# Crowsinc/LiveVisionKit

Hardware: AMD Instinct MI355X
Metric: stabilized frames/sec (one 4K YUV420 stream per GPU, steady state) (higher is better)
Workload: dtype f32

## Files before the change

include/lvk_hip.h:

```cpp
#ifndef LVK_HIP_H
#define LVK_HIP_H

#include <stdint.h>
#include <stddef.h>

#ifdef __cplusplus
extern "C" {
#endif

#define LVK_HIP_OK              0
#define LVK_HIP_ERR_ARG        -1
#define LVK_HIP_ERR_RUNTIME    -2
#define LVK_HIP_ERR_NO_DEVICE  -3

typedef struct lvk_hip_ctx lvk_hip_ctx;


int  lvk_hip_ctx_create(int device, lvk_hip_ctx** out);
int  lvk_hip_ctx_create_on_stream(int device, void* hip_stream, lvk_hip_ctx** out);
void lvk_hip_ctx_destroy(lvk_hip_ctx* ctx);
int  lvk_hip_sync(lvk_hip_ctx* ctx);
void* lvk_hip_stream(lvk_hip_ctx* ctx);
const char* lvk_hip_last_error(lvk_hip_ctx* ctx);
const char* lvk_hip_version(void);
// ... 6 lines not shown

int lvk_hip_malloc(lvk_hip_ctx* ctx, size_t bytes, void** d_ptr);
int lvk_hip_free(lvk_hip_ctx* ctx, void* d_ptr);
int lvk_hip_trim(lvk_hip_ctx* ctx);
int lvk_hip_upload(lvk_hip_ctx* ctx, void* d_dst, const void* h_src, size_t bytes);
int lvk_hip_download(lvk_hip_ctx* ctx, void* h_dst, const void* d_src, size_t bytes);

int  lvk_hip_host_malloc(lvk_hip_ctx* ctx, size_t bytes, void** h_ptr);
int  lvk_hip_host_free(lvk_hip_ctx* ctx, void* h_ptr);


int lvk_hip_remap_homography(lvk_hip_ctx* ctx,
                             const void* d_src, int src_step, int src_rows, int src_cols,
                             void* d_dst, int dst_step, int dst_rows, int dst_cols,
                             int off_x, int off_y, const float H[9], const uint8_t bg[3], int yuv);

int lvk_hip_remap_mesh(lvk_hip_ctx* ctx,
                       const void* d_src, int src_step, int src_rows, int src_cols,
                       void* d_dst, int dst_step,
                       const float* mesh, int mesh_rows, int mesh_cols, const uint8_t bg[3], int yuv);

int lvk_hip_remap_map(lvk_hip_ctx* ctx, const void* d_src, int src_step, int rows, int cols, void* d_dst, int dst_step,
                      const void* d_map, int map_step, const uint8_t bg[3], int yuv);

#define LVK_REMAP_EXACT 0
#define LVK_REMAP_1LSB  1
int lvk_hip_set_remap_precision(lvk_hip_ctx* ctx, int precision);
int lvk_hip_get_remap_precision(lvk_hip_ctx* ctx);

int lvk_hip_upscale(lvk_hip_ctx* ctx, const void* d_src, int src_step, int src_rows, int src_cols,
                    void* d_dst, int dst_step, int dst_rows, int dst_cols, int yuv);

int lvk_hip_sharpen(lvk_hip_ctx* ctx, const void* d_src, int src_step, int rows, int cols, void* d_dst, int dst_step, float sharpness);

typedef struct lvk_camera_params { double fx, fy, cx, cy, k1, k2, p1, p2, k3; } lvk_camera_params;
int lvk_hip_lens_map_create(lvk_hip_ctx* ctx, const lvk_camera_params* params, int rows, int cols, void** d_map, int view_xywh[4]);
int lvk_hip_lens_map_destroy(lvk_hip_ctx* ctx, void* d_map);
int lvk_hip_warpmesh_apply_lens(lvk_hip_ctx* ctx, const void* d_src, int src_step, int rows, int cols, void* d_dst, int dst_step,
                                const float* mesh, int mesh_rows, int mesh_cols, const uint8_t bg[3], int yuv, const lvk_camera_params* lens);
int lvk_hip_lens_undistort_points(lvk_hip_ctx* ctx, const lvk_camera_params* params, int rows, int cols, double sx, double sy,
                                  const float* pts, int n, float* out);

int lvk_hip_warpmesh_apply_yuv420(lvk_hip_ctx* ctx, const void* d_src, int src_step, int rows, int cols,
                                  void* o_y, int oy_step, void* o_u, int ou_step, void* o_v, int ov_step, int nv12,
                                  const float* mesh, int mesh_rows, int mesh_cols, const uint8_t bg[3]);

int lvk_hip_warpmesh_apply(lvk_hip_ctx* ctx,
                           const void* d_src, int src_step, int rows, int cols,
                           void* d_dst, int dst_step,
                           const float* mesh, int mesh_rows, int mesh_cols, const uint8_t bg[3], int yuv);

int lvk_hip_ingest_yuv420(lvk_hip_ctx* ctx, const void* d_y, int y_step, const void* d_u, int u_step, const void* d_v, int v_step, int nv12,
                          int rows, int cols, void* d_dst, int dst_step);
int lvk_hip_egress_yuv420(lvk_hip_ctx* ctx, const void* d_src, int src_step, int rows, int cols,
                          void* d_y, int y_step, void* d_u, int u_step, void* d_v, int v_step, int nv12);

#define LVK_VIDEO_FORMAT_I420 1
#define LVK_VIDEO_FORMAT_NV12 2
#define LVK_VIDEO_FORMAT_YVYU 3
#define LVK_VIDEO_FORMAT_YUY2 4
#define LVK_VIDEO_FORMAT_UYVY 5
#define LVK_VIDEO_FORMAT_RGBA 6
#define LVK_VIDEO_FORMAT_BGRA 7
#define LVK_VIDEO_FORMAT_BGRX 8
#define LVK_VIDEO_FORMAT_Y800 9
#define LVK_VIDEO_FORMAT_I444 10
#define LVK_VIDEO_FORMAT_BGR3 11
#define LVK_VIDEO_FORMAT_I422 12
#define LVK_VIDEO_FORMAT_I40A 13
#define LVK_VIDEO_FORMAT_I42A 14
#define LVK_VIDEO_FORMAT_YUVA 15
#define LVK_VIDEO_FORMAT_AYUV 16
int lvk_hip_ingest_obs(lvk_hip_ctx* ctx, int video_format, const void* const d_planes[3], const int steps[3], int rows, int cols, void* d_dst, int dst_step);
int lvk_hip_egress_obs(lvk_hip_ctx* ctx, int video_format, const void* d_src, int src_step, int rows, int cols, void* const d_planes[3], const int steps[3]);
int lvk_hip_obs_frame_format(int video_format);

typedef struct lvk_stab_settings
{
    int detection_width, detection_height;
    int detection_regions_x, detection_regions_y;
    int force_detection;
    float max_feature_density, min_feature_density, accumulation_rate;
    int track_local_motions;
    float temporal_smoothing, local_smoothing;
    int min_motion_samples;
    float acceptance_threshold, uniformity_threshold;
    int predictive_samples;
    float corrective_limit_x, corrective_limit_y;
    float smoothing_steps, response_rate;
    int motion_width, motion_height;
    float background[3];
    int crop_to_stable_region, stabilize_output;
    float min_scene_quality, min_tracking_quality;
} lvk_stab_settings;

typedef struct lvk_stab_stats
{
    float tracking_stability;
    float scene_quality, trust;
    float distribution;
    int n_detected, n_matched, n_tracked, frame_delay;
    double smoothing_factor;
    double homography[9];
} lvk_stab_stats;

#define LVK_FORMAT_BGR 0
#define LVK_FORMAT_BGRA 1
#define LVK_FORMAT_RGB 2
#define LVK_FORMAT_RGBA 3
#define LVK_FORMAT_YUV 4
#define LVK_FORMAT_GRAY 5

typedef struct lvk_hip_stab lvk_hip_stab;

void lvk_stab_default_settings(lvk_stab_settings* s);
int  lvk_hip_stab_create(lvk_hip_ctx* ctx, const lvk_stab_settings* settings, lvk_hip_stab** out);
void lvk_hip_stab_destroy(lvk_hip_stab* stab);
int  lvk_hip_stab_configure(lvk_hip_stab* stab, const lvk_stab_settings* settings);
int  lvk_hip_stab_restart(lvk_hip_stab* stab);
int  lvk_hip_stab_draw_trackers(lvk_hip_stab* stab);
int  lvk_hip_stab_draw_motion_mesh(lvk_hip_stab* stab);
int  lvk_hip_draw_grid(lvk_hip_ctx* ctx, void* d_dst, int dst_step, int rows, int cols, int grid_w, int grid_h, const uint8_t colour[3], int thickness);
int  lvk_hip_draw_crosses(lvk_hip_ctx* ctx, void* d_dst, int dst_step, int rows, int cols, const float* pts_xy, int n,
                          float scale_x, float scale_y, const uint8_t colour[3], int cross_size, int thickness);
int  lvk_hip_draw_points(lvk_hip_ctx* ctx, void* d_dst, int dst_step, int rows, int cols, const float* pts_xy, int n, float scale_x, float scale_y,
                         const uint8_t colour[3], int point_size);
int  lvk_hip_draw_rect(lvk_hip_ctx* ctx, void* d_dst, int dst_step, int rows, int cols, const int rect_xywh[4], const uint8_t colour[3], int thickness);
int  lvk_hip_draw_text(lvk_hip_ctx* ctx, void* d_dst, int dst_step, int rows, int cols, const char* text, int x, int y, const uint8_t colour[3],
                       int scale, int thickness);
int  lvk_hip_stab_set_lens(lvk_hip_stab* stab, const lvk_camera_params* params);
int  lvk_hip_stab_reset_context(lvk_hip_stab* stab);
int  lvk_hip_stab_ready(const lvk_hip_stab* stab);
int  lvk_hip_stab_frame_delay(const lvk_hip_stab* stab);
int  lvk_hip_stab_stable_region(const lvk_hip_stab* stab, int rows, int cols, int rect_xywh[4]);

typedef struct lvk_frame_info { int rows, cols, format; } lvk_frame_info;
int  lvk_hip_stab_next_output(const lvk_hip_stab* stab, int rows, int cols, int format, lvk_frame_info* out);
int  lvk_hip_stab_push(lvk_hip_stab* stab, const void* d_frame, int step, int rows, int cols, uint64_t timestamp, int format,
                       void* d_out, int out_step, int out_rows, int* produced, uint64_t* out_timestamp, const void** released,
                       lvk_frame_info* emitted);

int  lvk_hip_stab_push_yuv420(lvk_hip_stab* stab, const void* d_y, int y_step, const void* d_u, int u_step, const void* d_v, int v_step, int nv12,
                              int rows, int cols, uint64_t timestamp,
                              void* o_y, int oy_step, void* o_u, int ou_step, void* o_v, int ov_step, int o_rows,
                              int* produced, uint64_t* out_timestamp, lvk_frame_info* emitted);
int  lvk_hip_stab_push_obs(lvk_hip_stab* stab, int video_format, const void* const d_planes[3], const int steps[3], int rows, int cols, uint64_t timestamp,
                           void* const o_planes[3], const int o_steps[3], int o_rows, int* produced, uint64_t* out_timestamp, lvk_frame_info* emitted);

int  lvk_hip_stab_push_yuv420_host(lvk_hip_stab* stab, const void* h_y, int y_step, const void* h_u, int u_step, const void* h_v, int v_step, int nv12,
                                   int rows, int cols, uint64_t timestamp,
                                   void* oh_y, int oy_step, void* oh_u, int ou_step, void* oh_v, int ov_step, int o_rows,
                                   int* produced, uint64_t* out_timestamp, lvk_frame_info* emitted);
int  lvk_hip_stab_push_obs_host(lvk_hip_stab* stab, int video_format,
                                const void* const h_planes[3], const int steps[3], int rows, int cols, uint64_t timestamp,
                                void* const oh_planes[3], const int o_steps[3], int o_rows,
                                int* produced, uint64_t* out_timestamp, lvk_frame_info* emitted);
int  lvk_hip_stab_prefetch_yuv420_host(lvk_hip_stab* stab, const void* h_y, int y_step, const void* h_u, int u_step, const void* h_v, int v_step,
                                       int nv12, int rows, int cols);
int  lvk_hip_stab_prefetch_cancel(lvk_hip_stab* stab);
int  lvk_hip_stab_set_overlap(lvk_hip_stab* stab, int enable);
int  lvk_hip_stab_set_bulk_context(lvk_hip_stab* stab, lvk_hip_ctx* bulk);
void* lvk_hip_stab_output_stream(lvk_hip_stab* stab);
int  lvk_hip_stab_set_remap_precision(lvk_hip_stab* stab, int precision);
int  lvk_hip_stab_get_remap_precision(const lvk_hip_stab* stab);


typedef struct lvk_deblock_settings
{
    uint32_t detection_levels;
    uint32_t block_size;
    uint32_t filter_size;
    float filter_scaling;
} lvk_deblock_settings;

typedef struct lvk_hip_deblock lvk_hip_deblock;

void lvk_hip_deblock_default_settings(lvk_deblock_settings* s);
int  lvk_hip_deblock_create(lvk_hip_ctx* ctx, const lvk_deblock_settings* settings, lvk_hip_deblock** out);
int  lvk_hip_deblock_configure(lvk_hip_deblock* deb, const lvk_deblock_settings* settings);
void lvk_hip_deblock_destroy(lvk_hip_deblock* deb);
int  lvk_hip_deblock_apply(lvk_hip_deblock* deb, void* d_frame, int step, int rows, int cols, int format, int region_xywh[4]);
int  lvk_hip_deblock_draw_influence(const lvk_hip_deblock* deb, void* d_frame, int step, int rows, int cols, int format);
int  lvk_hip_deblock_filter_region(const lvk_hip_deblock* deb, int region_xywh[4]);

int  lvk_hip_cas(lvk_hip_ctx* ctx, const void* d_src, int src_step, int rows, int cols, int format, void* d_dst, int dst_step, float sharpness);

int  lvk_hip_reformat(lvk_hip_ctx* ctx, const void* d_src, int src_step, int rows, int cols, int src_format, void* d_dst, int dst_step,
                      int dst_format);

int  lvk_hip_fsr_easu(lvk_hip_ctx* ctx, const void* d_src, int src_step, int rows, int cols, int format, const int region_xywh[4], void* d_dst,
                      int dst_step, int out_rows, int out_cols);
int  lvk_hip_fsr_geometry(int rows, int cols, int out_rows, int out_cols, float multiplier, int maintain_aspect_ratio, const int crop_ltrb[4],
                          int region_xywh[4], int out_rows_cols[2], int* skip);
int  lvk_hip_text_size(const char* text, int scale, int thickness, int wh[2], int* baseline);



int  lvk_hip_stab_prefetch(lvk_hip_stab* stab, const void* d_frame, int step, int rows, int cols, int format);
int  lvk_hip_stab_prefetch_yuv420(lvk_hip_stab* stab, const void* d_y, int y_step, const void* d_u, int u_step, const void* d_v, int v_step,
                                  int nv12, int rows, int cols);
long long lvk_hip_stab_lookahead_frames(lvk_hip_stab* stab);

int lvk_hip_remap_homography_gray(lvk_hip_ctx* ctx, const void* d_src, int src_step, int src_rows, int src_cols,
                                  void* d_dst, int dst_step, int dst_rows, int dst_cols, int off_x, int off_y, const float H[9], uint8_t bg);
int lvk_hip_remap_mesh_gray(lvk_hip_ctx* ctx, const void* d_src, int src_step, int src_rows, int src_cols, void* d_dst, int dst_step,
                            const float* mesh, int mesh_rows, int mesh_cols, uint8_t bg);
int lvk_hip_remap_map_gray(lvk_hip_ctx* ctx, const void* d_src, int src_step, int rows, int cols, void* d_dst, int dst_step,
                           const void* d_map, int map_step, uint8_t bg);
int lvk_hip_warpmesh_apply_gray(lvk_hip_ctx* ctx, const void* d_src, int src_step, int rows, int cols, void* d_dst, int dst_step,
                                const float* mesh, int mesh_rows, int mesh_cols, uint8_t bg);
int lvk_hip_warpmesh_apply_lens_gray(lvk_hip_ctx* ctx, const void* d_src, int src_step, int rows, int cols, void* d_dst, int dst_step,
                                     const float* mesh, int mesh_rows, int mesh_cols, uint8_t bg, const lvk_camera_params* lens);
int  lvk_hip_stab_push_gray(lvk_hip_stab* stab, const void* d_frame, int step, int rows, int cols, uint64_t timestamp,
                            void* d_out, int out_step, int out_rows, int* produced, uint64_t* out_timestamp, const void** released,
                            lvk_frame_info* emitted);
int  lvk_hip_stab_push_gray_host(lvk_hip_stab* stab, const void* h_frame, int step, int rows, int cols, uint64_t timestamp,
                                 void* oh_out, int out_step, int out_rows, int* produced, uint64_t* out_timestamp, lvk_frame_info* emitted);

int lvk_hip_remap_homography_c4(lvk_hip_ctx* ctx, const void* d_src, int src_step, int src_rows, int src_cols,
                                void* d_dst, int dst_step, int dst_rows, int dst_cols, int off_x, int off_y, const float H[9], const uint8_t bg[4]);
int lvk_hip_remap_mesh_c4(lvk_hip_ctx* ctx, const void* d_src, int src_step, int src_rows, int src_cols, void* d_dst, int dst_step,
                          const float* mesh, int mesh_rows, int mesh_cols, const uint8_t bg[4]);
int lvk_hip_remap_map_c4(lvk_hip_ctx* ctx, const void* d_src, int src_step, int rows, int cols, void* d_dst, int dst_step,
                         const void* d_map, int map_step, const uint8_t bg[4]);
int lvk_hip_warpmesh_apply_c4(lvk_hip_ctx* ctx, const void* d_src, int src_step, int rows, int cols, void* d_dst, int dst_step,
                              const float* mesh, int mesh_rows, int mesh_cols, const uint8_t bg[4]);
int lvk_hip_warpmesh_apply_lens_c4(lvk_hip_ctx* ctx, const void* d_src, int src_step, int rows, int cols, void* d_dst, int dst_step,
                                   const float* mesh, int mesh_rows, int mesh_cols, const uint8_t bg[4], const lvk_camera_params* lens);
int  lvk_hip_stab_set_background_alpha(lvk_hip_stab* stab, int alpha);
int  lvk_hip_stab_push_c4(lvk_hip_stab* stab, const void* d_frame, int step, int rows, int cols, uint64_t timestamp, int format,
                          void* d_out, int out_step, int out_rows, int* produced, uint64_t* out_timestamp, const void** released,
                          lvk_frame_info* emitted);
int  lvk_hip_stab_push_c4_host(lvk_hip_stab* stab, const void* h_frame, int step, int rows, int cols, uint64_t timestamp, int format,
                               void* oh_out, int out_step, int out_rows, int* produced, uint64_t* out_timestamp, lvk_frame_info* emitted);

int lvk_hip_upscale_gray(lvk_hip_ctx* ctx, const void* d_src, int src_step, int src_rows, int src_cols, void* d_dst, int dst_step, int dst_rows, int dst_cols);
int lvk_hip_upscale_c4(lvk_hip_ctx* ctx, const void* d_src, int src_step, int src_rows, int src_cols, void* d_dst, int dst_step, int dst_rows, int dst_cols);
int lvk_hip_sharpen_gray(lvk_hip_ctx* ctx, const void* d_src, int src_step, int rows, int cols, void* d_dst, int dst_step, float sharpness);
int lvk_hip_sharpen_c4(lvk_hip_ctx* ctx, const void* d_src, int src_step, int rows, int cols, void* d_dst, int dst_step, float sharpness);

int lvk_hip_cas_gray(lvk_hip_ctx* ctx, const void* d_src, int src_step, int rows, int cols, void* d_dst, int dst_step, float sharpness);
int lvk_hip_fsr_easu_gray(lvk_hip_ctx* ctx, const void* d_src, int src_step, int rows, int cols, const int region_xywh[4],
                          void* d_dst, int dst_step, int out_rows, int out_cols);
int lvk_hip_fsr_easu_gray_path(int rw, int rh, int out_rows, int out_cols);


#define LVK_SCHED_PUSH_FREE_RUNNING   0
#define LVK_SCHED_PUSH_SYNCHRONISED   1
#define LVK_SCHED_INGEST_ON_TRACKER   2
#define LVK_SCHED_INGEST_ON_BULK      3
#define LVK_SCHED_INGEST_INLINE       4
#define LVK_SCHED_REMAP_PERSISTENT    5
#define LVK_SCHED_REMAP_FULL          6
#define LVK_SCHED_WAIT_SIGNAL_WORD    7
#define LVK_SCHED_WAIT_EVENT          8
#define LVK_SCHED_WAIT_WORD_TIMEOUT   9
#define LVK_SCHED_COUNT              10
int  lvk_hip_stab_schedule_counters(lvk_hip_stab* stab, long long out[LVK_SCHED_COUNT], int reset);

int  lvk_hip_stab_get_stats(const lvk_hip_stab* stab, lvk_stab_stats* out);
int  lvk_hip_stab_detector_frames(const lvk_hip_stab* stab, long long* on_device, long long* on_host);
int  lvk_hip_stab_get_meshes(const lvk_hip_stab* stab, float* motion, float* correction, int cap_floats);
int  lvk_hip_stab_get_features(const lvk_hip_stab* stab, float* xy_resp_age, int cap);


#define LVK_STAGE_DOWNSCALE 0
#define LVK_STAGE_PYRAMID   1
#define LVK_STAGE_FAST      2
#define LVK_STAGE_PYRLK     3
#define LVK_STAGE_MOTION    4
#define LVK_STAGE_REMAP     5
#define LVK_STAGE_INGEST    6
#define LVK_STAGE_EGRESS    7
#define LVK_STAGE_COUNT     8
int  lvk_hip_stab_set_profiling(lvk_hip_stab* stab, int enable);
int  lvk_hip_stab_get_profile(lvk_hip_stab* stab, double total_ms[LVK_STAGE_COUNT], long long launches[LVK_STAGE_COUNT]);

int lvk_hip_native_rcp(lvk_hip_ctx* ctx, const float* d_in, float* d_out, size_t n);

typedef struct lvk_hip_mesh_solver lvk_hip_mesh_solver;
int  lvk_hip_mesh_solver_create(lvk_hip_ctx* ctx, int cols, int rows, float gen_region_w, float gen_region_h,
                                float temporal_smoothing, float local_smoothing, int max_points, lvk_hip_mesh_solver** out);
void lvk_hip_mesh_solver_destroy(lvk_hip_mesh_solver* solver);
int  lvk_hip_mesh_solver_reset(lvk_hip_mesh_solver* solver);
int  lvk_hip_mesh_solver_solve(lvk_hip_mesh_solver* solver, const float* tracked, const float* matched, int n, float region_w, float region_h,
                               float temporal_now, float threshold, uint8_t* inliers, float* offsets);

int lvk_hip_luma_area_resize(lvk_hip_ctx* ctx, const void* d_src, int src_step, int pix_stride, int channel,
                             int srows, int scols, void* d_dst, int dst_step, int drows, int dcols);

int lvk_hip_pyr_down(lvk_hip_ctx* ctx, const void* d_src, int src_step, int rows, int cols, void* d_dst, int dst_step);
int lvk_hip_scharr(lvk_hip_ctx* ctx, const void* d_src, int src_step, int rows, int cols, void* d_dst);

int lvk_hip_build_pyramid(lvk_hip_ctx* ctx, const void* d_img, int step, int rows, int cols, int max_level, int win_w, int win_h,
                          uint8_t* levels, int16_t* derivs, int* level_rows, int* level_cols);

int lvk_hip_fast_detect(lvk_hip_ctx* ctx, const void* d_img, int step, int rows, int cols,
                        const int* regions, int nregions, uint32_t* out, int cap, int* counts);

int lvk_hip_pyrlk(lvk_hip_ctx* ctx, const void* d_prev, int prev_step, const void* d_next, int next_step, int rows, int cols,
                  const float* prev_pts, int n, float* next_pts, uint8_t* status,
                  int win_w, int win_h, int max_level, int max_count, double epsilon, double min_eig_threshold);

int lvk_hip_estimate_global_motion(lvk_hip_ctx* ctx, const float* pts1, const float* pts2, int n, double threshold,
                                   double region_w, double region_h, int full_homography, double H[9], uint8_t* mask);

int lvk_hip_estimate_global_motion_lo(lvk_hip_ctx* ctx, const float* pts1, const float* pts2, int n, double threshold,
                                      double region_w, double region_h, int full_homography, int lo_mode, double H[9], uint8_t* mask,
                                      int lo_info[2]);

int lvk_hip_fast_filter(lvk_hip_ctx* ctx, const float* prev, const float* matched, const uint8_t* status, int n, float* out_prev, float* out_matched);

#define LVK_TRACK_CHAIN_GUARD 64
#define LVK_TRACK_CHAIN_FILL  0xA5
typedef struct lvk_track_chain_desc
{
    const float* prev; const float* matched; const uint8_t* status; const float* und;
    const void* d_prev_img; int prev_step; const void* d_next_img; int next_step; int rows, cols;
    int win_w, win_h, max_level, max_count; double epsilon, min_eig;
    const lvk_camera_params* lens; int lens_rows, lens_cols; double lens_sx, lens_sy;
    int n_bound, count_on_device, n_word;
    int full, model_on_device, full_word;
    int separate_compact, host_signal;
    double threshold; int region_w, region_h;
} lvk_track_chain_desc;
typedef struct lvk_track_chain_result
{
    double H[9]; int rc, signalled, count_dev, count_host;
    uint8_t* mask; float* pairs_dev; float* mirror_matched; uint8_t* mirror_status;
    float* next_pts; uint8_t* flow_status; float* flow_und;
} lvk_track_chain_result;
int lvk_hip_track_chain(lvk_hip_ctx* ctx, const lvk_track_chain_desc* desc, lvk_track_chain_result* result);

int lvk_hip_deblock_get_grid(lvk_hip_deblock* deb, uint8_t* mean, uint8_t* grid, float* keep_block, int capacity, int extent_xy[2]);


int lvk_hip_cas_const(float sharpness, float* peak);

int lvk_hip_cvt_code_target(int code, int src_format, int dcn);

int lvk_hip_fsr_easu_const(int rw, int rh, int W, int H, int ow, int oh, float con[16]);

int lvk_hip_fsr_easu_path(int rw, int rh, int out_rows, int out_cols);

enum
{
    LVK_AREA_PATH_FAST_DW_8x8_C3_BGR = 0, LVK_AREA_PATH_FAST_DW_8x8_C3_RGB = 1, LVK_AREA_PATH_FAST_DW_4x4_C3_BGR = 2, LVK_AREA_PATH_FAST_DW_4x4_C3_RGB = 3,
    LVK_AREA_PATH_FAST_DW_8x8_C3 = 4, LVK_AREA_PATH_FAST_DW_4x4_C3 = 5, LVK_AREA_PATH_FAST_DW_8x8_C1 = 6, LVK_AREA_PATH_FAST_DW_4x4_C1 = 7,
    LVK_AREA_PATH_FAST = 8, LVK_AREA_PATH_TILE_4 = 9, LVK_AREA_PATH_TILE_8 = 10, LVK_AREA_PATH_TAPS_4 = 11, LVK_AREA_PATH_TAPS_8 = 12,
    LVK_AREA_PATH_GENERAL = 13, LVK_AREA_PATH_ENLARGE = 14, LVK_AREA_PATH_COUNT = 15
};
int lvk_hip_area_resize_path(lvk_hip_ctx* ctx, const void* d_src, int src_step, int pix_stride, int channel,
                             int srows, int scols, int drows, int dcols);

int lvk_hip_remap_map_yuv420(lvk_hip_ctx* ctx, const void* d_src, int src_step, int rows, int cols,
                             void* o_y, int oy_step, void* o_u, int ou_step, void* o_v, int ov_step, int nv12,
                             const void* d_map, int map_step, const uint8_t bg[3]);
typedef struct lvk_hip_lens lvk_hip_lens;
int  lvk_hip_lens_create(lvk_hip_ctx* ctx, const lvk_camera_params* profile , int test_mode, lvk_hip_lens** out);
int  lvk_hip_lens_configure(lvk_hip_lens* lens, const lvk_camera_params* profile, int test_mode);
void lvk_hip_lens_destroy(lvk_hip_lens* lens);
int  lvk_hip_lens_view(lvk_hip_lens* lens, int rows, int cols, int view_xywh[4]);
int  lvk_hip_lens_apply(lvk_hip_lens* lens, void* d_src, int src_step, int rows, int cols, int format, void* d_dst, int dst_step);
int  lvk_hip_lens_apply_gray(lvk_hip_lens* lens, const void* d_src, int src_step, int rows, int cols, void* d_dst, int dst_step);
int  lvk_hip_lens_apply_c4(lvk_hip_lens* lens, const void* d_src, int src_step, int rows, int cols, int format, void* d_dst, int dst_step);
int  lvk_hip_lens_apply_yuv420(lvk_hip_lens* lens, const void* d_y, int y_step, const void* d_u, int u_step, const void* d_v, int v_step,
                               void* o_y, int oy_step, void* o_u, int ou_step, void* o_v, int ov_step, int rows, int cols, int nv12);

int  lvk_hip_remap_map_obs(lvk_hip_ctx* ctx, int video_format, const void* d_src, int src_step, int rows, int cols,
                           void* const o_planes[3], const int o_steps[3], const void* d_map, int map_step, const uint8_t bg[3]);
int  lvk_hip_lens_apply_obs(lvk_hip_lens* lens, int video_format, const void* const d_planes[3], const int steps[3],
                            void* const o_planes[3], const int o_steps[3], int rows, int cols);

#ifdef __cplusplus
}
#endif

#include "lvk_hip_scaling_420.h"
#include "lvk_hip_deblock_420.h"
#include "lvk_hip_deblock_px.h"
#endif
```

livevisionkit_amd/_native.py:

```python
import ctypes
import os

_HERE = os.path.dirname(os.path.abspath(__file__))
LIB_PATH = os.environ.get("LVK_HIP_LIB") or os.path.join(_HERE, "liblvk_hip.so")

_c = ctypes
_P = _c.c_void_p
_SIG = {
    "lvk_hip_ctx_create": (_c.c_int, [_c.c_int, _c.POINTER(_P)]),
    "lvk_hip_ctx_create_on_stream": (_c.c_int, [_c.c_int, _P, _c.POINTER(_P)]),
    "lvk_hip_ctx_destroy": (None, [_P]),
    "lvk_hip_sync": (_c.c_int, [_P]),
    "lvk_hip_stream": (_P, [_P]),
    "lvk_hip_last_error": (_c.c_char_p, [_P]),
    "lvk_hip_version": (_c.c_char_p, []),
    "lvk_hip_abi_version": (_c.c_int, []),
    "lvk_hip_device_count": (_c.c_int, []),
    "lvk_hip_device_usable": (_c.c_int, [_c.c_int]),
    "lvk_hip_malloc": (_c.c_int, [_P, _c.c_size_t, _c.POINTER(_P)]),
    "lvk_hip_free": (_c.c_int, [_P, _P]),
    "lvk_hip_trim": (_c.c_int, [_P]),
    "lvk_hip_ctx_wait": (_c.c_int, [_P, _P]),
    "lvk_hip_upload": (_c.c_int, [_P, _P, _P, _c.c_size_t]),
    "lvk_hip_download": (_c.c_int, [_P, _P, _P, _c.c_size_t]),
    "lvk_hip_remap_homography": (_c.c_int, [_P, _P, _c.c_int, _c.c_int, _c.c_int, _P, _c.c_int, _c.c_int, _c.c_int,
                                            _c.c_int, _c.c_int, _c.POINTER(_c.c_float), _c.POINTER(_c.c_uint8), _c.c_int]),
    "lvk_hip_remap_mesh": (_c.c_int, [_P, _P, _c.c_int, _c.c_int, _c.c_int, _P, _c.c_int,
                                      _c.POINTER(_c.c_float), _c.c_int, _c.c_int, _c.POINTER(_c.c_uint8), _c.c_int]),
    "lvk_hip_remap_map": (_c.c_int, [_P, _P, _c.c_int, _c.c_int, _c.c_int, _P, _c.c_int, _P, _c.c_int, _c.POINTER(_c.c_uint8), _c.c_int]),
    "lvk_hip_remap_homography_gray": (_c.c_int, [_P, _P, _c.c_int, _c.c_int, _c.c_int, _P, _c.c_int, _c.c_int, _c.c_int,
                                                 _c.c_int, _c.c_int, _c.POINTER(_c.c_float), _c.c_uint8]),
    "lvk_hip_remap_mesh_gray": (_c.c_int, [_P, _P, _c.c_int, _c.c_int, _c.c_int, _P, _c.c_int, _c.POINTER(_c.c_float), _c.c_int, _c.c_int, _c.c_uint8]),
    "lvk_hip_remap_map_gray": (_c.c_int, [_P, _P, _c.c_int, _c.c_int, _c.c_int, _P, _c.c_int, _P, _c.c_int, _c.c_uint8]),
    "lvk_hip_warpmesh_apply_gray": (_c.c_int, [_P, _P, _c.c_int, _c.c_int, _c.c_int, _P, _c.c_int, _c.POINTER(_c.c_float), _c.c_int, _c.c_int, _c.c_uint8]),
    "lvk_hip_warpmesh_apply_lens_gray": (_c.c_int, [_P, _P, _c.c_int, _c.c_int, _c.c_int, _P, _c.c_int, _c.POINTER(_c.c_float), _c.c_int, _c.c_int, _c.c_uint8, _P]),
    "lvk_hip_stab_push_gray": (_c.c_int, [_P, _P, _c.c_int, _c.c_int, _c.c_int, _c.c_uint64, _P, _c.c_int, _c.c_int,
                                          _c.POINTER(_c.c_int), _c.POINTER(_c.c_uint64), _c.POINTER(_P), _P]),
    "lvk_hip_stab_push_gray_host": (_c.c_int, [_P, _P, _c.c_int, _c.c_int, _c.c_int, _c.c_uint64, _P, _c.c_int, _c.c_int,
                                               _c.POINTER(_c.c_int), _c.POINTER(_c.c_uint64), _P]),
    "lvk_hip_set_remap_precision": (_c.c_int, [_P, _c.c_int]),
    "lvk_hip_get_remap_precision": (_c.c_int, [_P]),
    "lvk_hip_stab_set_remap_precision": (_c.c_int, [_P, _c.c_int]),
    "lvk_hip_stab_get_remap_precision": (_c.c_int, [_P]),
    "lvk_hip_remap_homography_c4": (_c.c_int, [_P, _P, _c.c_int, _c.c_int, _c.c_int, _P, _c.c_int, _c.c_int, _c.c_int,
                                               _c.c_int, _c.c_int, _c.POINTER(_c.c_float), _c.POINTER(_c.c_uint8)]),
    "lvk_hip_remap_mesh_c4": (_c.c_int, [_P, _P, _c.c_int, _c.c_int, _c.c_int, _P, _c.c_int, _c.POINTER(_c.c_float), _c.c_int, _c.c_int, _c.POINTER(_c.c_uint8)]),
    "lvk_hip_remap_map_c4": (_c.c_int, [_P, _P, _c.c_int, _c.c_int, _c.c_int, _P, _c.c_int, _P, _c.c_int, _c.POINTER(_c.c_uint8)]),
    "lvk_hip_warpmesh_apply_c4": (_c.c_int, [_P, _P, _c.c_int, _c.c_int, _c.c_int, _P, _c.c_int, _c.POINTER(_c.c_float), _c.c_int, _c.c_int, _c.POINTER(_c.c_uint8)]),
    "lvk_hip_warpmesh_apply_lens_c4": (_c.c_int, [_P, _P, _c.c_int, _c.c_int, _c.c_int, _P, _c.c_int, _c.POINTER(_c.c_float), _c.c_int, _c.c_int, _c.POINTER(_c.c_uint8), _P]),
    "lvk_hip_stab_set_background_alpha": (_c.c_int, [_P, _c.c_int]),
    "lvk_hip_stab_push_c4": (_c.c_int, [_P, _P, _c.c_int, _c.c_int, _c.c_int, _c.c_uint64, _c.c_int, _P, _c.c_int, _c.c_int,
                                        _c.POINTER(_c.c_int), _c.POINTER(_c.c_uint64), _c.POINTER(_P), _P]),
    "lvk_hip_stab_push_c4_host": (_c.c_int, [_P, _P, _c.c_int, _c.c_int, _c.c_int, _c.c_uint64, _c.c_int, _P, _c.c_int, _c.c_int,
                                             _c.POINTER(_c.c_int), _c.POINTER(_c.c_uint64), _P]),
    "lvk_hip_upscale": (_c.c_int, [_P, _P, _c.c_int, _c.c_int, _c.c_int, _P, _c.c_int, _c.c_int, _c.c_int, _c.c_int]),
    "lvk_hip_sharpen": (_c.c_int, [_P, _P, _c.c_int, _c.c_int, _c.c_int, _P, _c.c_int, _c.c_float]),
    "lvk_hip_upscale_gray": (_c.c_int, [_P, _P, _c.c_int, _c.c_int, _c.c_int, _P, _c.c_int, _c.c_int, _c.c_int]),
    "lvk_hip_upscale_c4": (_c.c_int, [_P, _P, _c.c_int, _c.c_int, _c.c_int, _P, _c.c_int, _c.c_int, _c.c_int]),
    "lvk_hip_sharpen_gray": (_c.c_int, [_P, _P, _c.c_int, _c.c_int, _c.c_int, _P, _c.c_int, _c.c_float]),
    "lvk_hip_sharpen_c4": (_c.c_int, [_P, _P, _c.c_int, _c.c_int, _c.c_int, _P, _c.c_int, _c.c_float]),
    "lvk_hip_native_rcp": (_c.c_int, [_P, _P, _P, _c.c_size_t]),
    "lvk_hip_mesh_solver_create": (_c.c_int, [_P, _c.c_int, _c.c_int, _c.c_float, _c.c_float, _c.c_float, _c.c_float, _c.c_int, _c.POINTER(_P)]),
    "lvk_hip_mesh_solver_destroy": (None, [_P]),
    "lvk_hip_mesh_solver_reset": (_c.c_int, [_P]),
    "lvk_hip_mesh_solver_solve": (_c.c_int, [_P, _c.POINTER(_c.c_float), _c.POINTER(_c.c_float), _c.c_int, _c.c_float, _c.c_float, _c.c_float, _c.c_float,
                                             _c.POINTER(_c.c_uint8), _c.POINTER(_c.c_float)]),
    "lvk_hip_lens_map_create": (_c.c_int, [_P, _P, _c.c_int, _c.c_int, _c.POINTER(_P), _c.POINTER(_c.c_int)]),
    "lvk_hip_lens_map_destroy": (_c.c_int, [_P, _P]),
    "lvk_hip_warpmesh_apply_lens": (_c.c_int, [_P, _P, _c.c_int, _c.c_int, _c.c_int, _P, _c.c_int, _c.POINTER(_c.c_float), _c.c_int, _c.c_int, _c.POINTER(_c.c_uint8), _c.c_int, _P]),
    "lvk_hip_lens_undistort_points": (_c.c_int, [_P, _P, _c.c_int, _c.c_int, _c.c_double, _c.c_double, _c.POINTER(_c.c_float), _c.c_int, _c.POINTER(_c.c_float)]),
    "lvk_hip_stab_set_lens": (_c.c_int, [_P, _P]),
    "lvk_hip_stab_output_stream": (_P, [_P]),
    "lvk_hip_fast_filter": (_c.c_int, [_P, _c.POINTER(_c.c_float), _c.POINTER(_c.c_float), _c.POINTER(_c.c_uint8), _c.c_int, _c.POINTER(_c.c_float), _c.POINTER(_c.c_float)]),
    "lvk_hip_stab_draw_trackers": (_c.c_int, [_P]),
    "lvk_hip_stab_draw_motion_mesh": (_c.c_int, [_P]),
    "lvk_hip_draw_grid": (_c.c_int, [_P, _P, _c.c_int, _c.c_int, _c.c_int, _c.c_int, _c.c_int, _c.POINTER(_c.c_uint8), _c.c_int]),
    "lvk_hip_draw_crosses": (_c.c_int, [_P, _P, _c.c_int, _c.c_int, _c.c_int, _c.POINTER(_c.c_float), _c.c_int, _c.c_float, _c.c_float,
                                        _c.POINTER(_c.c_uint8), _c.c_int, _c.c_int]),
    "lvk_hip_draw_points": (_c.c_int, [_P, _P, _c.c_int, _c.c_int, _c.c_int, _c.POINTER(_c.c_float), _c.c_int, _c.c_float, _c.c_float,
                                       _c.POINTER(_c.c_uint8), _c.c_int]),
    "lvk_hip_draw_rect": (_c.c_int, [_P, _P, _c.c_int, _c.c_int, _c.c_int, _c.POINTER(_c.c_int), _c.POINTER(_c.c_uint8), _c.c_int]),
    "lvk_hip_draw_text": (_c.c_int, [_P, _P, _c.c_int, _c.c_int, _c.c_int, _c.c_char_p, _c.c_int, _c.c_int, _c.POINTER(_c.c_uint8), _c.c_int, _c.c_int]),
    "lvk_hip_text_size": (_c.c_int, [_c.c_char_p, _c.c_int, _c.c_int, _c.POINTER(_c.c_int), _c.POINTER(_c.c_int)]),
    "lvk_hip_warpmesh_apply_yuv420": (_c.c_int, [_P, _P, _c.c_int, _c.c_int, _c.c_int, _P, _c.c_int, _P, _c.c_int, _P, _c.c_int, _c.c_int,
                                                 _c.POINTER(_c.c_float), _c.c_int, _c.c_int, _c.POINTER(_c.c_uint8)]),
    "lvk_hip_warpmesh_apply": (_c.c_int, [_P, _P, _c.c_int, _c.c_int, _c.c_int, _P, _c.c_int,
                                          _c.POINTER(_c.c_float), _c.c_int, _c.c_int, _c.POINTER(_c.c_uint8), _c.c_int]),
    "lvk_hip_luma_area_resize": (_c.c_int, [_P, _P, _c.c_int, _c.c_int, _c.c_int, _c.c_int, _c.c_int, _P, _c.c_int, _c.c_int, _c.c_int]),
    "lvk_hip_pyr_down": (_c.c_int, [_P, _P, _c.c_int, _c.c_int, _c.c_int, _P, _c.c_int]),
    "lvk_hip_scharr": (_c.c_int, [_P, _P, _c.c_int, _c.c_int, _c.c_int, _P]),
    "lvk_hip_build_pyramid": (_c.c_int, [_P, _P, _c.c_int, _c.c_int, _c.c_int, _c.c_int, _c.c_int, _c.c_int,
                                         _c.POINTER(_c.c_uint8), _c.POINTER(_c.c_int16), _c.POINTER(_c.c_int), _c.POINTER(_c.c_int)]),
    "lvk_hip_fast_detect": (_c.c_int, [_P, _P, _c.c_int, _c.c_int, _c.c_int, _c.POINTER(_c.c_int), _c.c_int,
                                       _c.POINTER(_c.c_uint32), _c.c_int, _c.POINTER(_c.c_int)]),
    "lvk_hip_pyrlk": (_c.c_int, [_P, _P, _c.c_int, _P, _c.c_int, _c.c_int, _c.c_int, _c.POINTER(_c.c_float), _c.c_int,
                                 _c.POINTER(_c.c_float), _c.POINTER(_c.c_uint8), _c.c_int, _c.c_int, _c.c_int, _c.c_int,
                                 _c.c_double, _c.c_double]),
    "lvk_hip_ingest_yuv420": (_c.c_int, [_P, _P, _c.c_int, _P, _c.c_int, _P, _c.c_int, _c.c_int, _c.c_int, _c.c_int, _P, _c.c_int]),
    "lvk_hip_egress_yuv420": (_c.c_int, [_P, _P, _c.c_int, _c.c_int, _c.c_int, _P, _c.c_int, _P, _c.c_int, _P, _c.c_int, _c.c_int]),
    "lvk_hip_ingest_obs": (_c.c_int, [_P, _c.c_int, _P * 3, _c.c_int * 3, _c.c_int, _c.c_int, _P, _c.c_int]),
    "lvk_hip_egress_obs": (_c.c_int, [_P, _c.c_int, _P, _c.c_int, _c.c_int, _c.c_int, _P * 3, _c.c_int * 3]),
    "lvk_hip_obs_frame_format": (_c.c_int, [_c.c_int]),
    "lvk_hip_estimate_global_motion": (_c.c_int, [_P, _c.POINTER(_c.c_float), _c.POINTER(_c.c_float), _c.c_int, _c.c_double,
                                                  _c.c_double, _c.c_double, _c.c_int, _c.POINTER(_c.c_double), _c.POINTER(_c.c_uint8)]),
    "lvk_hip_estimate_global_motion_lo": (_c.c_int, [_P, _c.POINTER(_c.c_float), _c.POINTER(_c.c_float), _c.c_int, _c.c_double,
                                                     _c.c_double, _c.c_double, _c.c_int, _c.c_int, _c.POINTER(_c.c_double), _c.POINTER(_c.c_uint8),
                                                     _c.POINTER(_c.c_int)]),
    "lvk_hip_track_chain": (_c.c_int, [_P, _P, _P]),
    "lvk_stab_default_settings": (None, [_P]),
    "lvk_hip_stab_create": (_c.c_int, [_P, _P, _c.POINTER(_P)]),
    "lvk_hip_stab_destroy": (None, [_P]),
    "lvk_hip_stab_configure": (_c.c_int, [_P, _P]),
    "lvk_hip_stab_restart": (_c.c_int, [_P]),
    "lvk_hip_stab_reset_context": (_c.c_int, [_P]),
    "lvk_hip_stab_ready": (_c.c_int, [_P]),
    "lvk_hip_stab_frame_delay": (_c.c_int, [_P]),
    "lvk_hip_stab_stable_region": (_c.c_int, [_P, _c.c_int, _c.c_int, _c.POINTER(_c.c_int)]),
    "lvk_hip_stab_next_output": (_c.c_int, [_P, _c.c_int, _c.c_int, _c.c_int, _P]),
    "lvk_hip_stab_push": (_c.c_int, [_P, _P, _c.c_int, _c.c_int, _c.c_int, _c.c_uint64, _c.c_int, _P, _c.c_int, _c.c_int,
                                     _c.POINTER(_c.c_int), _c.POINTER(_c.c_uint64), _c.POINTER(_P), _P]),
    "lvk_hip_stab_push_yuv420": (_c.c_int, [_P, _P, _c.c_int, _P, _c.c_int, _P, _c.c_int, _c.c_int, _c.c_int, _c.c_int, _c.c_uint64,
                                            _P, _c.c_int, _P, _c.c_int, _P, _c.c_int, _c.c_int, _c.POINTER(_c.c_int), _c.POINTER(_c.c_uint64), _P]),
    "lvk_hip_stab_push_obs": (_c.c_int, [_P, _c.c_int, _P * 3, _c.c_int * 3, _c.c_int, _c.c_int, _c.c_uint64, _P * 3, _c.c_int * 3, _c.c_int,
                                         _c.POINTER(_c.c_int), _c.POINTER(_c.c_uint64), _P]),
    "lvk_hip_stab_push_yuv420_host": (_c.c_int, [_P, _P, _c.c_int, _P, _c.c_int, _P, _c.c_int, _c.c_int, _c.c_int, _c.c_int, _c.c_uint64,
                                            _P, _c.c_int, _P, _c.c_int, _P, _c.c_int, _c.c_int, _c.POINTER(_c.c_int), _c.POINTER(_c.c_uint64), _P]),
    "lvk_hip_stab_push_obs_host": (_c.c_int, [_P, _c.c_int, _P * 3, _c.c_int * 3, _c.c_int, _c.c_int, _c.c_uint64, _P * 3, _c.c_int * 3, _c.c_int,
                                              _c.POINTER(_c.c_int), _c.POINTER(_c.c_uint64), _P]),
    "lvk_hip_stab_prefetch_yuv420_host": (_c.c_int, [_P, _P, _c.c_int, _P, _c.c_int, _P, _c.c_int, _c.c_int, _c.c_int, _c.c_int]),
    "lvk_hip_stab_prefetch_cancel": (_c.c_int, [_P]),
    "lvk_hip_stab_prefetch": (_c.c_int, [_P, _P, _c.c_int, _c.c_int, _c.c_int, _c.c_int]),
    "lvk_hip_stab_prefetch_yuv420": (_c.c_int, [_P, _P, _c.c_int, _P, _c.c_int, _P, _c.c_int, _c.c_int, _c.c_int, _c.c_int]),
    "lvk_hip_stab_lookahead_frames": (_c.c_longlong, [_P]),
    "lvk_hip_stab_schedule_counters": (_c.c_int, [_P, _c.POINTER(_c.c_longlong), _c.c_int]),
    "lvk_hip_stab_detector_frames": (_c.c_int, [_P, _c.POINTER(_c.c_longlong), _c.POINTER(_c.c_longlong)]),
    "lvk_hip_host_malloc": (_c.c_int, [_P, _c.c_size_t, _c.POINTER(_P)]),
    "lvk_hip_host_free": (_c.c_int, [_P, _P]),
    "lvk_hip_stab_get_stats": (_c.c_int, [_P, _P]),
    "lvk_hip_stab_get_meshes": (_c.c_int, [_P, _c.POINTER(_c.c_float), _c.POINTER(_c.c_float), _c.c_int]),
    "lvk_hip_stab_get_features": (_c.c_int, [_P, _c.POINTER(_c.c_float), _c.c_int]),
    "lvk_hip_stab_set_overlap": (_c.c_int, [_P, _c.c_int]),
    "lvk_hip_stab_set_bulk_context": (_c.c_int, [_P, _P]),
    "lvk_hip_stab_set_profiling": (_c.c_int, [_P, _c.c_int]),
    "lvk_hip_stab_get_profile": (_c.c_int, [_P, _c.POINTER(_c.c_double), _c.POINTER(_c.c_longlong)]),
    "lvk_hip_deblock_default_settings": (None, [_P]),
    "lvk_hip_deblock_create": (_c.c_int, [_P, _P, _c.POINTER(_P)]),
    "lvk_hip_deblock_configure": (_c.c_int, [_P, _P]),
    "lvk_hip_deblock_destroy": (None, [_P]),
    "lvk_hip_deblock_apply": (_c.c_int, [_P, _P, _c.c_int, _c.c_int, _c.c_int, _c.c_int, _c.POINTER(_c.c_int)]),
    "lvk_hip_deblock_draw_influence": (_c.c_int, [_P, _P, _c.c_int, _c.c_int, _c.c_int, _c.c_int]),
    "lvk_hip_deblock_filter_region": (_c.c_int, [_P, _c.POINTER(_c.c_int)]),
    "lvk_hip_deblock_get_grid": (_c.c_int, [_P, _c.POINTER(_c.c_uint8), _c.POINTER(_c.c_uint8), _c.POINTER(_c.c_float), _c.c_int, _c.POINTER(_c.c_int)]),
    "lvk_hip_cas": (_c.c_int, [_P, _P, _c.c_int, _c.c_int, _c.c_int, _c.c_int, _P, _c.c_int, _c.c_float]),
    "lvk_hip_cas_const": (_c.c_int, [_c.c_float, _c.POINTER(_c.c_float)]),
    "lvk_hip_reformat": (_c.c_int, [_P, _P, _c.c_int, _c.c_int, _c.c_int, _c.c_int, _P, _c.c_int, _c.c_int]),
    "lvk_hip_cvt_code_target": (_c.c_int, [_c.c_int, _c.c_int, _c.c_int]),
    "lvk_hip_fsr_easu": (_c.c_int, [_P, _P, _c.c_int, _c.c_int, _c.c_int, _c.c_int, _c.POINTER(_c.c_int), _P, _c.c_int, _c.c_int, _c.c_int]),
    "lvk_hip_fsr_geometry": (_c.c_int, [_c.c_int, _c.c_int, _c.c_int, _c.c_int, _c.c_float, _c.c_int, _c.POINTER(_c.c_int), _c.POINTER(_c.c_int),
                                        _c.POINTER(_c.c_int), _c.POINTER(_c.c_int)]),
    "lvk_hip_fsr_easu_const": (_c.c_int, [_c.c_int, _c.c_int, _c.c_int, _c.c_int, _c.c_int, _c.c_int, _c.POINTER(_c.c_float)]),
    "lvk_hip_fsr_easu_path": (_c.c_int, [_c.c_int, _c.c_int, _c.c_int, _c.c_int]),
    "lvk_hip_cas_gray": (_c.c_int, [_P, _P, _c.c_int, _c.c_int, _c.c_int, _P, _c.c_int, _c.c_float]),
    "lvk_hip_fsr_easu_gray": (_c.c_int, [_P, _P, _c.c_int, _c.c_int, _c.c_int, _c.POINTER(_c.c_int), _P, _c.c_int, _c.c_int, _c.c_int]),
    "lvk_hip_fsr_easu_gray_path": (_c.c_int, [_c.c_int, _c.c_int, _c.c_int, _c.c_int]),
    "lvk_hip_area_resize_path": (_c.c_int, [_P, _P, _c.c_int, _c.c_int, _c.c_int, _c.c_int, _c.c_int, _c.c_int, _c.c_int]),
    "lvk_hip_remap_map_yuv420": (_c.c_int, [_P, _P, _c.c_int, _c.c_int, _c.c_int, _P, _c.c_int, _P, _c.c_int, _P, _c.c_int, _c.c_int,
                                            _P, _c.c_int, _c.POINTER(_c.c_uint8)]),
    "lvk_hip_lens_create": (_c.c_int, [_P, _P, _c.c_int, _c.POINTER(_P)]),
    "lvk_hip_lens_configure": (_c.c_int, [_P, _P, _c.c_int]),
    "lvk_hip_lens_destroy": (None, [_P]),
    "lvk_hip_lens_view": (_c.c_int, [_P, _c.c_int, _c.c_int, _c.POINTER(_c.c_int)]),
    "lvk_hip_lens_apply": (_c.c_int, [_P, _P, _c.c_int, _c.c_int, _c.c_int, _c.c_int, _P, _c.c_int]),
    "lvk_hip_lens_apply_gray": (_c.c_int, [_P, _P, _c.c_int, _c.c_int, _c.c_int, _P, _c.c_int]),
    "lvk_hip_lens_apply_c4": (_c.c_int, [_P, _P, _c.c_int, _c.c_int, _c.c_int, _c.c_int, _P, _c.c_int]),
    "lvk_hip_lens_apply_yuv420": (_c.c_int, [_P, _P, _c.c_int, _P, _c.c_int, _P, _c.c_int, _P, _c.c_int, _P, _c.c_int, _P, _c.c_int,
                                             _c.c_int, _c.c_int, _c.c_int]),
    "lvk_hip_remap_map_obs": (_c.c_int, [_P, _c.c_int, _P, _c.c_int, _c.c_int, _c.c_int, _P * 3, _c.c_int * 3, _P, _c.c_int, _c.POINTER(_c.c_uint8)]),
    "lvk_hip_lens_apply_obs": (_c.c_int, [_P, _c.c_int, _P * 3, _c.c_int * 3, _P * 3, _c.c_int * 3, _c.c_int, _c.c_int]),
}

_SIG_DEBLOCK_PX = {
    "lvk_hip_deblock_apply_gray": (_c.c_int, [_P, _P, _c.c_int, _c.c_int, _c.c_int, _c.POINTER(_c.c_int)]),
    "lvk_hip_deblock_apply_c4": (_c.c_int, [_P, _P, _c.c_int, _c.c_int, _c.c_int, _c.c_int, _c.POINTER(_c.c_int)]),
}

_SIG_DEBLOCK_420 = {
    "lvk_hip_deblock_apply_yuv420": (_c.c_int, [_P, _P, _c.c_int, _P, _c.c_int, _P, _c.c_int, _P, _c.c_int, _P, _c.c_int, _P, _c.c_int,
                                                _c.c_int, _c.c_int, _c.c_int, _c.POINTER(_c.c_int)]),
}

_SIG_SCALING_420 = {
    "lvk_hip_scale_yuv420": (_c.c_int, [_P, _P, _c.c_int, _P, _c.c_int, _P, _c.c_int, _c.c_int, _c.c_int,
                                        _P, _c.c_int, _P, _c.c_int, _P, _c.c_int, _c.c_int, _c.c_int, _c.c_int, _c.c_float]),
}

_lib = None


def symbols():
    return sorted(_SIG.keys())


def symbols_deblock_px():
    return sorted(_SIG_DEBLOCK_PX.keys())


def symbols_deblock_420():
    return sorted(_SIG_DEBLOCK_420.keys())


def symbols_scaling_420():
    return sorted(_SIG_SCALING_420.keys())


def load():
    global _lib
    if _lib is not None:
        return _lib
    if not os.path.exists(LIB_PATH):
        raise RuntimeError(
            f"{LIB_PATH} is missing: build it with `python -c 'import __graft_entry__ as g; g.build()'` "
            "(or `make -C livevisionkit_amd/csrc`). There is no CPU fallback.")
    import torch
    lib = ctypes.CDLL(LIB_PATH, mode=ctypes.RTLD_GLOBAL)
    for name, (res, args) in {**_SIG, **_SIG_DEBLOCK_PX, **_SIG_DEBLOCK_420, **_SIG_SCALING_420}.items():
        fn = getattr(lib, name)
        fn.restype = res
        fn.argtypes = args
    _lib = lib
    return lib
```

livevisionkit_amd/context.py:

```python
import ctypes

import numpy as np

from . import _native


class LvkHipError(RuntimeError):
    pass


def _f32(a):
    a = np.ascontiguousarray(a, dtype=np.float32)
    return a, a.ctypes.data_as(ctypes.POINTER(ctypes.c_float))


def _u8x3(bg):
    a = np.ascontiguousarray(bg, dtype=np.uint8).reshape(3)
    return a, a.ctypes.data_as(ctypes.POINTER(ctypes.c_uint8))


def _u8x4(bg):
    a = np.ascontiguousarray(bg, dtype=np.uint8).reshape(4)
    return a, a.ctypes.data_as(ctypes.POINTER(ctypes.c_uint8))


def _planes420_empty(rows, cols, nv12, device):
    import torch
    y = torch.empty((rows, cols), dtype=torch.uint8, device=device)
    u = torch.empty((rows // 2, cols // 2, 2) if nv12 else (rows // 2, cols // 2), dtype=torch.uint8, device=device)
    return (y, u) if nv12 else (y, u, torch.empty_like(u))


def _planes420_args(planes, nv12):
    a = []
    for p in planes[:2 if nv12 else 3]:
        a += [p.data_ptr(), p.stride(0)]
    return a + ([None, 0] if nv12 else [])


TRACK_CHAIN_GUARD = 64
TRACK_CHAIN_FILL = 0xA5


class TrackChainDesc(ctypes.Structure):
    _fields_ = [("prev", ctypes.POINTER(ctypes.c_float)), ("matched", ctypes.POINTER(ctypes.c_float)), ("status", ctypes.POINTER(ctypes.c_uint8)),
                ("und", ctypes.POINTER(ctypes.c_float)),
                ("d_prev_img", ctypes.c_void_p), ("prev_step", ctypes.c_int), ("d_next_img", ctypes.c_void_p), ("next_step", ctypes.c_int),
                ("rows", ctypes.c_int), ("cols", ctypes.c_int),
                ("win_w", ctypes.c_int), ("win_h", ctypes.c_int), ("max_level", ctypes.c_int), ("max_count", ctypes.c_int),
                ("epsilon", ctypes.c_double), ("min_eig", ctypes.c_double),
                ("lens", ctypes.c_void_p), ("lens_rows", ctypes.c_int), ("lens_cols", ctypes.c_int), ("lens_sx", ctypes.c_double), ("lens_sy", ctypes.c_double),
                ("n_bound", ctypes.c_int), ("count_on_device", ctypes.c_int), ("n_word", ctypes.c_int),
                ("full", ctypes.c_int), ("model_on_device", ctypes.c_int), ("full_word", ctypes.c_int),
                ("separate_compact", ctypes.c_int), ("host_signal", ctypes.c_int),
                ("threshold", ctypes.c_double), ("region_w", ctypes.c_int), ("region_h", ctypes.c_int)]


class TrackChainResult(ctypes.Structure):
    _fields_ = [("H", ctypes.c_double * 9), ("rc", ctypes.c_int), ("signalled", ctypes.c_int), ("count_dev", ctypes.c_int), ("count_host", ctypes.c_int),
                ("mask", ctypes.POINTER(ctypes.c_uint8)), ("pairs_dev", ctypes.POINTER(ctypes.c_float)), ("mirror_matched", ctypes.POINTER(ctypes.c_float)),
                ("mirror_status", ctypes.POINTER(ctypes.c_uint8)),
                ("next_pts", ctypes.POINTER(ctypes.c_float)), ("flow_status", ctypes.POINTER(ctypes.c_uint8)), ("flow_und", ctypes.POINTER(ctypes.c_float))]

REMAP_EXACT, REMAP_1LSB = 0, 1


def _remap_precision(precision):
    if isinstance(precision, str):
        return {"exact": REMAP_EXACT, "1lsb": REMAP_1LSB}.get(precision.lower(), -1)
    return int(precision)


class Context:

    def __init__(self, device=0, stream=None):
        import torch
        if not torch.cuda.is_available():
            raise LvkHipError("no GPU visible: the lvk HIP path has no CPU fallback")
        self.lib = _native.load()
        self.device = device
        torch.cuda.set_device(device)
        self._torch_stream = stream if stream is not None else torch.cuda.current_stream(device)
        handle = ctypes.c_void_p()
        rc = self.lib.lvk_hip_ctx_create_on_stream(device, ctypes.c_void_p(self._torch_stream.cuda_stream), ctypes.byref(handle))
        if rc != 0:
            raise LvkHipError(f"lvk_hip_ctx_create failed ({rc}): {self.lib.lvk_hip_last_error(None).decode()}")
        self.handle = handle

    def close(self):
        if getattr(self, "handle", None):
            self.lib.lvk_hip_ctx_destroy(self.handle)
            self.handle = None

    def __del__(self):
        try:
            self.close()
        except Exception:
            pass

    def _check(self, rc):
        if rc != 0:
            raise LvkHipError(f"lvk_hip call failed ({rc}): {self.lib.lvk_hip_last_error(self.handle).decode()}")

    def sync(self):
        self._check(self.lib.lvk_hip_sync(self.handle))

    def set_remap_precision(self, precision):
        self._check(self.lib.lvk_hip_set_remap_precision(self.handle, _remap_precision(precision)))

    @property
    def remap_precision(self):
        return self.lib.lvk_hip_get_remap_precision(self.handle)

    def remap_homography(self, src, H, bg=(255, 0, 255), yuv=True, out=None, dst_size=None, offset=(0, 0)):
        import torch
        rows, cols = src.shape[0], src.shape[1]
        drows, dcols = dst_size if dst_size is not None else (rows, cols)
        if out is None:
            out = torch.empty((drows, dcols, 3), dtype=torch.uint8, device=src.device)
        Ha, Hp = _f32(np.asarray(H, dtype=np.float32).reshape(9))
        bga, bgp = _u8x3(bg)
        self._check(self.lib.lvk_hip_remap_homography(
            self.handle, src.data_ptr(), src.stride(0), rows, cols, out.data_ptr(), out.stride(0), drows, dcols,
            offset[0], offset[1], Hp, bgp, 1 if yuv else 0))
        return out

    def remap_mesh(self, src, mesh, bg=(255, 0, 255), yuv=True, out=None):
        import torch
        rows, cols = src.shape[0], src.shape[1]
        if out is None:
            out = torch.empty((rows, cols, 3), dtype=torch.uint8, device=src.device)
        m = np.ascontiguousarray(mesh, dtype=np.float32)
        ma, mp = _f32(m)
        bga, bgp = _u8x3(bg)
        self._check(self.lib.lvk_hip_remap_mesh(
            self.handle, src.data_ptr(), src.stride(0), rows, cols, out.data_ptr(), out.stride(0),
            mp, m.shape[0], m.shape[1], bgp, 1 if yuv else 0))
        return out

    def warpmesh_apply(self, src, mesh, bg=(255, 0, 255), yuv=True, out=None):
        import torch
        rows, cols = src.shape[0], src.shape[1]
        if out is None:
            out = torch.empty((rows, cols, 3), dtype=torch.uint8, device=src.device)
        m = np.ascontiguousarray(mesh, dtype=np.float32)
        ma, mp = _f32(m)
        bga, bgp = _u8x3(bg)
        self._check(self.lib.lvk_hip_warpmesh_apply(
            self.handle, src.data_ptr(), src.stride(0), rows, cols, out.data_ptr(), out.stride(0),
            mp, m.shape[0], m.shape[1], bgp, 1 if yuv else 0))
        return out

    def _px_out(self, sfx, src, out, shape=None):
        import torch
        if sfx == "_gray" and src.dim() != 2:
            raise ValueError("a one-channel frame is a [rows, cols] uint8 tensor")
        if sfx == "_c4" and (src.dim() != 3 or src.shape[2] != 4):
            raise ValueError("a four-channel frame is a [rows, cols, 4] uint8 tensor")
        return out if out is not None else torch.empty(tuple(shape or src.shape[:2]) + tuple(src.shape[2:]), dtype=torch.uint8, device=src.device)

    def _px_call(self, name, sfx, src, out, bg, mid, tail=(), shape=None):
        out = self._px_out(sfx, src, out, shape)
        bga, bgp = (None, int(bg)) if sfx == "_gray" else _u8x4(bg)
        self._check(getattr(self.lib, "lvk_hip_" + name + sfx)(self.handle, src.data_ptr(), src.stride(0), src.shape[0], src.shape[1], out.data_ptr(), out.stride(0),
                                                               *mid, bgp, *tail))
        return out

    def _px_homography(self, sfx, src, H, bg, out, dst_size, offset):
        drows, dcols = dst_size if dst_size is not None else tuple(src.shape[:2])
        Ha, Hp = _f32(np.asarray(H, dtype=np.float32).reshape(9))
        return self._px_call("remap_homography", sfx, src, out, bg, (drows, dcols, offset[0], offset[1], Hp), shape=(drows, dcols))

    def _px_mesh(self, name, sfx, src, mesh, bg, out, lens=None):
        ma, mp = _f32(mesh)
        tail = () if lens is None else ((ctypes.c_double * 9)(*[float(v) for v in lens]),)
        return self._px_call(name, sfx, src, out, bg, (mp, ma.shape[0], ma.shape[1]), tail)

    def _px_map(self, sfx, src, offsets, bg, out):
        return self._px_call("remap_map", sfx, src, out, bg, (offsets.data_ptr(), offsets.stride(0) * 4))

    def remap_homography_gray(self, src, H, bg=0, out=None, dst_size=None, offset=(0, 0)):
        return self._px_homography("_gray", src, H, bg, out, dst_size, offset)

    def remap_mesh_gray(self, src, mesh, bg=0, out=None):
        return self._px_mesh("remap_mesh", "_gray", src, mesh, bg, out)

    def remap_map_gray(self, src, offsets, bg=0, out=None):
        return self._px_map("_gray", src, offsets, bg, out)

    def warpmesh_apply_gray(self, src, mesh, bg=0, out=None, lens=None):
        return self._px_mesh("warpmesh_apply" if lens is None else "warpmesh_apply_lens", "_gray", src, mesh, bg, out, lens)

    def remap_homography_c4(self, src, H, bg=(255, 0, 255, 255), out=None, dst_size=None, offset=(0, 0)):
        return self._px_homography("_c4", src, H, bg, out, dst_size, offset)

    def remap_mesh_c4(self, src, mesh, bg=(255, 0, 255, 255), out=None):
        return self._px_mesh("remap_mesh", "_c4", src, mesh, bg, out)

    def remap_map_c4(self, src, offsets, bg=(255, 0, 255, 255), out=None):
        return self._px_map("_c4", src, offsets, bg, out)

    def warpmesh_apply_c4(self, src, mesh, bg=(255, 0, 255, 255), out=None):
        return self._px_mesh("warpmesh_apply", "_c4", src, mesh, bg, out)

    def warpmesh_apply_lens_c4(self, src, mesh, lens, bg=(255, 0, 255, 255), out=None):
        return self._px_mesh("warpmesh_apply_lens", "_c4", src, mesh, bg, out, lens)

    def luma_area_resize(self, frame, drows, dcols, channel=0, out=None):
        import torch
        pix = frame.shape[2] if frame.dim() == 3 else 1
        if out is None:
            out = torch.empty((drows, dcols), dtype=torch.uint8, device=frame.device)
        self._check(self.lib.lvk_hip_luma_area_resize(self.handle, frame.data_ptr(), frame.stride(0), pix, channel,
                                                      frame.shape[0], frame.shape[1], out.data_ptr(), out.stride(0), drows, dcols))
        return out

    def area_resize_path(self, frame, drows, dcols, channel=0):
        pix = frame.shape[2] if frame.dim() == 3 else 1
        path = self.lib.lvk_hip_area_resize_path(self.handle, frame.data_ptr(), frame.stride(0), pix, channel, frame.shape[0], frame.shape[1], drows, dcols)
        self._check(min(path, 0))
        return path

    def pyr_down(self, img, out=None):
        import torch
        if out is None:
            out = torch.empty(((img.shape[0] + 1) // 2, (img.shape[1] + 1) // 2), dtype=torch.uint8, device=img.device)
        self._check(self.lib.lvk_hip_pyr_down(self.handle, img.data_ptr(), img.stride(0), img.shape[0], img.shape[1],
                                              out.data_ptr(), out.stride(0)))
        return out

    def scharr(self, img, out=None):
        import torch
        if out is None:
            out = torch.empty((img.shape[0], img.shape[1], 2), dtype=torch.int16, device=img.device)
        self._check(self.lib.lvk_hip_scharr(self.handle, img.data_ptr(), img.stride(0), img.shape[0], img.shape[1], out.data_ptr()))
        return out

    def build_pyramid(self, img, max_level=3, win=(11, 11)):
        rows, cols = img.shape
        lv = np.zeros(rows * cols * 2, np.uint8); dv = np.zeros(rows * cols * 4, np.int16)
        lr = np.zeros(8, np.int32); lc = np.zeros(8, np.int32)
        n = self.lib.lvk_hip_build_pyramid(self.handle, img.data_ptr(), img.stride(0), rows, cols, max_level, win[0], win[1],
                                           lv.ctypes.data_as(ctypes.POINTER(ctypes.c_uint8)), dv.ctypes.data_as(ctypes.POINTER(ctypes.c_int16)),
                                           lr.ctypes.data_as(ctypes.POINTER(ctypes.c_int)), lc.ctypes.data_as(ctypes.POINTER(ctypes.c_int)))
        self._check(min(n, 0))
        out, lo, do = [], 0, 0
        for i in range(n):
            r, c = int(lr[i]), int(lc[i])
            out.append((lv[lo:lo + r * c].reshape(r, c).copy(), dv[do:do + r * c * 2].reshape(r, c, 2).copy()))
            lo += r * c; do += r * c * 2
        return out

    def fast_detect(self, img, regions, cap=None):
        rg = np.ascontiguousarray(regions, dtype=np.int32).reshape(-1, 6)
        n = rg.shape[0]
        cap = cap or int(max(1, (rg[:, 2] * rg[:, 3]).max()))
        out = np.zeros((n, cap), np.uint32)
        counts = np.zeros(n, np.int32)
        self._check(self.lib.lvk_hip_fast_detect(self.handle, img.data_ptr(), img.stride(0), img.shape[0], img.shape[1],
                                                 rg.ctypes.data_as(ctypes.POINTER(ctypes.c_int)), n,
                                                 out.ctypes.data_as(ctypes.POINTER(ctypes.c_uint32)), cap,
                                                 counts.ctypes.data_as(ctypes.POINTER(ctypes.c_int))))
        res = []
        for i in range(n):
            e = out[i, :min(cap, counts[i])]
            res.append(np.stack([e & 0xFFF, (e >> 12) & 0xFFF, e >> 24], axis=1).astype(np.int32))
        return res, counts

    def pyrlk(self, prev, nxt, pts, win=(11, 11), max_level=3, max_count=5, epsilon=0.01, min_eig=1e-4):
        pts = np.ascontiguousarray(pts, np.float32).reshape(-1, 2)
        out = np.zeros_like(pts)
        st = np.zeros(len(pts), np.uint8)
        self._check(self.lib.lvk_hip_pyrlk(self.handle, prev.data_ptr(), prev.stride(0), nxt.data_ptr(), nxt.stride(0),
                                           prev.shape[0], prev.shape[1],
                                           pts.ctypes.data_as(ctypes.POINTER(ctypes.c_float)), len(pts),
                                           out.ctypes.data_as(ctypes.POINTER(ctypes.c_float)),
                                           st.ctypes.data_as(ctypes.POINTER(ctypes.c_uint8)),
                                           win[0], win[1], max_level, max_count, float(epsilon), float(min_eig)))
        return out, st

    def estimate_global_motion(self, p1, p2, threshold, region=(480, 270), full_homography=True):
        p1 = np.ascontiguousarray(p1, np.float32).reshape(-1, 2); p2 = np.ascontiguousarray(p2, np.float32).reshape(-1, 2)
        H = np.zeros(9, np.float64); mask = np.zeros(len(p1), np.uint8)
        rc = self.lib.lvk_hip_estimate_global_motion(self.handle, p1.ctypes.data_as(ctypes.POINTER(ctypes.c_float)),
                                                     p2.ctypes.data_as(ctypes.POINTER(ctypes.c_float)), len(p1), float(threshold),
                                                     float(region[0]), float(region[1]), 1 if full_homography else 0,
                                                     H.ctypes.data_as(ctypes.POINTER(ctypes.c_double)),
                                                     mask.ctypes.data_as(ctypes.POINTER(ctypes.c_uint8)))
        if rc in (-1, -2, -3):
            self._check(rc)
        return rc, H.reshape(3, 3), mask

    def estimate_global_motion_lo(self, p1, p2, threshold, lo_mode, region=(480, 270), full_homography=True):
        p1 = np.ascontiguousarray(p1, np.float32).reshape(-1, 2); p2 = np.ascontiguousarray(p2, np.float32).reshape(-1, 2)
        H = np.zeros(9, np.float64); mask = np.zeros(len(p1), np.uint8); info = (ctypes.c_int * 2)(-1, -1)
        rc = self.lib.lvk_hip_estimate_global_motion_lo(self.handle, p1.ctypes.data_as(ctypes.POINTER(ctypes.c_float)),
                                                        p2.ctypes.data_as(ctypes.POINTER(ctypes.c_float)), len(p1), float(threshold),
                                                        float(region[0]), float(region[1]), 1 if full_homography else 0, int(lo_mode),
                                                        H.ctypes.data_as(ctypes.POINTER(ctypes.c_double)),
                                                        mask.ctypes.data_as(ctypes.POINTER(ctypes.c_uint8)), info)
        if rc in (-1, -2, -3):
            self._check(rc)
        return rc, H.reshape(3, 3), mask, info[0], info[1]

    def ingest_yuv420(self, y, u, v=None, out=None):
        import torch
        rows, cols = y.shape
        if out is None:
            out = torch.empty((rows, cols, 3), dtype=torch.uint8, device=y.device)
        nv12 = v is None
        self._check(self.lib.lvk_hip_ingest_yuv420(self.handle, *_planes420_args((y, u, v), nv12), 1 if nv12 else 0, rows, cols, out.data_ptr(), out.stride(0)))
        return out

    def egress_yuv420(self, frame, nv12=False, out=None):
        rows, cols = frame.shape[:2]
        if out is None:
            out = _planes420_empty(rows, cols, nv12, frame.device)
        y, u, v = out if not nv12 else (out[0], out[1], None)
        self._check(self.lib.lvk_hip_egress_yuv420(self.handle, frame.data_ptr(), frame.stride(0), rows, cols, *_planes420_args((y, u, v), nv12), 1 if nv12 else 0))
        return (y, u) if nv12 else (y, u, v)

    VIDEO_FORMATS = {"I420": 1, "NV12": 2, "YVYU": 3, "YUY2": 4, "UYVY": 5, "RGBA": 6, "BGRA": 7, "BGRX": 8, "Y800": 9, "I444": 10, "BGR3": 11,
                     "I422": 12, "I40A": 13, "I42A": 14, "YUVA": 15, "AYUV": 16}

    def _obs_args(self, planes):
        import ctypes as c
        ptrs = (c.c_void_p * 3)(*[p.data_ptr() for p in planes] + [None] * (3 - len(planes)))
        steps = (c.c_int * 3)(*[p.stride(0) for p in planes] + [0] * (3 - len(planes)))
        return ptrs, steps

    def ingest_obs(self, fmt, planes, out=None):
        import torch
        rows, cols = planes[0].shape[:2]
        if out is None:
            out = torch.empty((rows, cols) if fmt == "Y800" else (rows, cols, 3), dtype=torch.uint8, device=planes[0].device)
        ptrs, steps = self._obs_args(planes)
        self._check(self.lib.lvk_hip_ingest_obs(self.handle, self.VIDEO_FORMATS[fmt], ptrs, steps, rows, cols, out.data_ptr(), out.stride(0)))
        return out

    def egress_obs(self, fmt, frame, planes):
        rows, cols = frame.shape[:2]
        ptrs, steps = self._obs_args(planes)
        self._check(self.lib.lvk_hip_egress_obs(self.handle, self.VIDEO_FORMATS[fmt], frame.data_ptr(), frame.stride(0), rows, cols, ptrs, steps))
        return planes

    def obs_frame_format(self, fmt):
        return self.lib.lvk_hip_obs_frame_format(self.VIDEO_FORMATS[fmt] if isinstance(fmt, str) else int(fmt))

    def remap_map(self, src, offsets, bg=(255, 0, 255), yuv=True, out=None):
        import torch
        rows, cols = src.shape[:2]
        if out is None:
            out = torch.empty_like(src)
        bga, bgp = _u8x3(bg)
        self._check(self.lib.lvk_hip_remap_map(self.handle, src.data_ptr(), src.stride(0), rows, cols, out.data_ptr(), out.stride(0),
                                               offsets.data_ptr(), offsets.stride(0) * 4, bgp, 1 if yuv else 0))
        return out

    def remap_map_yuv420(self, src, offsets, bg=(255, 0, 255), nv12=False, out=None):
        rows, cols = src.shape[0], src.shape[1]
        out = _planes420_empty(rows, cols, nv12, src.device) if out is None else tuple(out)
        bga, bgp = _u8x3(bg)
        self._check(self.lib.lvk_hip_remap_map_yuv420(self.handle, src.data_ptr(), src.stride(0), rows, cols, *_planes420_args(out, nv12), 1 if nv12 else 0,
                                                      offsets.data_ptr(), offsets.stride(0) * 4, bgp))
        return out

    def video_format(self, fmt):
        return self.VIDEO_FORMATS[fmt] if isinstance(fmt, str) else int(fmt)

    def remap_map_obs(self, fmt, src, offset_map, planes, bg=(0, 0, 0)):
        rows, cols = src.shape[0], src.shape[1]
        ptrs, steps = self._obs_args(planes)
        bga, bgp = _u8x3(bg)
        self._check(self.lib.lvk_hip_remap_map_obs(self.handle, self.video_format(fmt), src.data_ptr(), src.stride(0), rows, cols, ptrs, steps,
                                                   offset_map.data_ptr(), offset_map.stride(0) * 4, bgp))
        return planes

    def upscale(self, src, size, yuv=True, out=None):
        import torch
        rows, cols = src.shape[:2]
        if out is None:
            out = torch.empty((int(size[1]), int(size[0]), 3), dtype=torch.uint8, device=src.device)
        self._check(self.lib.lvk_hip_upscale(self.handle, src.data_ptr(), src.stride(0), rows, cols,
                                             out.data_ptr(), out.stride(0), out.shape[0], out.shape[1], 1 if yuv else 0))
        return out

    def sharpen(self, src, sharpness=0.7, out=None):
        import torch
        rows, cols = src.shape[:2]
        if out is None:
            out = torch.empty_like(src)
        self._check(self.lib.lvk_hip_sharpen(self.handle, src.data_ptr(), src.stride(0), rows, cols, out.data_ptr(), out.stride(0),
                                             float(sharpness)))
        return out

    def scale_yuv420(self, y, u, v=None, size=None, sharpness=0.8, out=None):
        rows, cols = y.shape
        w, h = (cols, rows) if size is None else (int(size[0]), int(size[1]))
        nv12 = v is None
        out = _planes420_empty(h, w, nv12, y.device) if out is None else tuple(out)
        self._check(self.lib.lvk_hip_scale_yuv420(self.handle, *_planes420_args((y, u, v), nv12), rows, cols, *_planes420_args(out, nv12),
                                                  h, w, 1 if nv12 else 0, float(sharpness)))
        return out

    def _px_upscale(self, sfx, src, size, out):
        out = self._px_out(sfx, src, out, (int(size[1]), int(size[0])))
        self._check(getattr(self.lib, "lvk_hip_upscale" + sfx)(self.handle, src.data_ptr(), src.stride(0), src.shape[0], src.shape[1],
                                                               out.data_ptr(), out.stride(0), out.shape[0], out.shape[1]))
        return out

    def _px_sharpen(self, sfx, src, sharpness, out):
        out = self._px_out(sfx, src, out)
        self._check(getattr(self.lib, "lvk_hip_sharpen" + sfx)(self.handle, src.data_ptr(), src.stride(0), src.shape[0], src.shape[1],
                                                               out.data_ptr(), out.stride(0), float(sharpness)))
        return out

    def upscale_gray(self, src, size, out=None):
        return self._px_upscale("_gray", src, size, out)

    def upscale_c4(self, src, size, out=None):
        return self._px_upscale("_c4", src, size, out)

    def sharpen_gray(self, src, sharpness=0.7, out=None):
        return self._px_sharpen("_gray", src, sharpness, out)

    def sharpen_c4(self, src, sharpness=0.7, out=None):
        return self._px_sharpen("_c4", src, sharpness, out)

    def mesh_solver(self, cols, rows, gen_region=(480, 270), temporal=1.0, local=20.0, max_points=4096):
        return MeshSolver(self, cols, rows, gen_region, temporal, local, max_points)

    def native_rcp(self, x):
        import torch
        x = x.contiguous()
        out = torch.empty_like(x)
        self._check(self.lib.lvk_hip_native_rcp(self.handle, x.data_ptr(), out.data_ptr(), x.numel()))
        return out

    def lens_map(self, params, rows, cols):
        import torch
        arr = (ctypes.c_double * 9)(*[float(v) for v in params])
        d = ctypes.c_void_p(); view = (ctypes.c_int * 4)()
        self._check(self.lib.lvk_hip_lens_map_create(self.handle, arr, rows, cols, ctypes.byref(d), view))
        tmp = np.zeros((rows, cols, 2), np.float32)
        self._check(self.lib.lvk_hip_download(self.handle, tmp.ctypes.data_as(ctypes.c_void_p), d, tmp.nbytes))
        self.sync()
        t = torch.from_numpy(tmp).to("cuda")
        self._check(self.lib.lvk_hip_lens_map_destroy(self.handle, d))
        return t, tuple(view)

    def warpmesh_apply_lens(self, src, mesh, params, bg=(255, 0, 255), yuv=True, out=None):
        import torch
        rows, cols = src.shape[0], src.shape[1]
        if out is None:
            out = torch.empty((rows, cols, 3), dtype=torch.uint8, device=src.device)
        m = np.ascontiguousarray(mesh, dtype=np.float32)
        ma, mp = _f32(m)
        bga, bgp = _u8x3(bg)
        arr = (ctypes.c_double * 9)(*[float(v) for v in params])
        self._check(self.lib.lvk_hip_warpmesh_apply_lens(self.handle, src.data_ptr(), src.stride(0), rows, cols, out.data_ptr(), out.stride(0),
                                                         mp, m.shape[0], m.shape[1], bgp, 1 if yuv else 0, arr))
        return out

    def lens_undistort_points(self, params, rows, cols, sx, sy, pts):
        p = np.ascontiguousarray(pts, np.float32).reshape(-1, 2)
        out = np.zeros_like(p)
        arr = (ctypes.c_double * 9)(*[float(v) for v in params])
        fp = ctypes.POINTER(ctypes.c_float)
        self._check(self.lib.lvk_hip_lens_undistort_points(self.handle, arr, rows, cols, float(sx), float(sy), p.ctypes.data_as(fp), len(p), out.ctypes.data_as(fp)))
        return out

    def draw_grid(self, frame, grid, colour, thickness=1):
        ca, cp = _u8x3(colour)
        self._check(self.lib.lvk_hip_draw_grid(self.handle, frame.data_ptr(), frame.stride(0), frame.shape[0], frame.shape[1], int(grid[0]), int(grid[1]), cp, thickness))
        return frame

    def draw_crosses(self, frame, points, colour, cross_size, thickness, scaling=(1.0, 1.0)):
        p = np.ascontiguousarray(points, np.float32).reshape(-1, 2)
        ca, cp = _u8x3(colour)
        self._check(self.lib.lvk_hip_draw_crosses(self.handle, frame.data_ptr(), frame.stride(0), frame.shape[0], frame.shape[1],
                                                  p.ctypes.data_as(ctypes.POINTER(ctypes.c_float)), len(p), float(scaling[0]), float(scaling[1]), cp,
                                                  int(cross_size), int(thickness)))
        return frame

    def fast_filter(self, prev, matched, status):
        a = np.ascontiguousarray(prev, np.float32).reshape(-1, 2); b = np.ascontiguousarray(matched, np.float32).reshape(-1, 2)
        st = np.ascontiguousarray(status, np.uint8).reshape(-1)
        oa = np.zeros_like(a); ob = np.zeros_like(b)
        fp = ctypes.POINTER(ctypes.c_float)
        m = self.lib.lvk_hip_fast_filter(self.handle, a.ctypes.data_as(fp), b.ctypes.data_as(fp), st.ctypes.data_as(ctypes.POINTER(ctypes.c_uint8)), len(a),
                                         oa.ctypes.data_as(fp), ob.ctypes.data_as(fp))
        if m < 0:
            self._check(m)
        return oa[:m], ob[:m]

    def track_chain(self, prev, matched=None, status=None, und=None, images=None, win=(11, 11), max_level=3, max_count=5, epsilon=0.01, min_eig=1e-4,
                    lens=None, threshold=3.0, region=(480, 270), full=True, full_word=None, n_word=None, separate_compact=False, host_signal=False):
        fp, bp = ctypes.POINTER(ctypes.c_float), ctypes.POINTER(ctypes.c_uint8)
        prev = np.ascontiguousarray(prev, np.float32).reshape(-1, 2)
        nb, G = len(prev), TRACK_CHAIN_GUARD
        d, r = TrackChainDesc(), TrackChainResult()
        keep = [prev]
        d.prev = prev.ctypes.data_as(fp)
        if images is None:
            matched = np.ascontiguousarray(matched, np.float32).reshape(nb, 2); status = np.ascontiguousarray(status, np.uint8).reshape(nb)
            keep += [matched, status]
            d.matched = matched.ctypes.data_as(fp); d.status = status.ctypes.data_as(bp)
            if und is not None:
                und = np.ascontiguousarray(und, np.float32).reshape(-1, 2)
                n_eff = nb if n_word is None else min(max(int(n_word), 0), nb)
                if len(und) != 2 * n_eff:
                    raise ValueError("und holds 2 x the effective count of positions (previous | matched)")
                keep.append(und)
                d.und = und.ctypes.data_as(fp)
        else:
            a, b = images
            keep += [a, b]
            d.d_prev_img = a.data_ptr(); d.prev_step = a.stride(0); d.d_next_img = b.data_ptr(); d.next_step = b.stride(0)
            d.rows, d.cols = a.shape[0], a.shape[1]
            d.win_w, d.win_h, d.max_level, d.max_count, d.epsilon, d.min_eig = win[0], win[1], max_level, max_count, float(epsilon), float(min_eig)
            if lens is not None:
                params, lrows, lcols, sx, sy = lens
                arr = (ctypes.c_double * 9)(*[float(v) for v in params])
                keep.append(arr)
                d.lens = ctypes.cast(arr, ctypes.c_void_p); d.lens_rows, d.lens_cols, d.lens_sx, d.lens_sy = int(lrows), int(lcols), float(sx), float(sy)
        d.n_bound = nb
        d.count_on_device, d.n_word = (0, 0) if n_word is None else (1, int(n_word))
        d.full = 1 if full else 0
        d.model_on_device, d.full_word = (0, 0) if full_word is None else (1, int(full_word))
        d.separate_compact = 1 if separate_compact else 0; d.host_signal = 1 if host_signal else 0
        d.threshold = float(threshold); d.region_w, d.region_h = int(region[0]), int(region[1])
        mask = np.zeros(nb, np.uint8); pairs = np.zeros((2, nb, 2), np.float32); mm = np.zeros((nb, 2), np.float32); ms = np.zeros(nb, np.uint8)
        r.mask = mask.ctypes.data_as(bp); r.pairs_dev = pairs.ctypes.data_as(fp); r.mirror_matched = mm.ctypes.data_as(fp); r.mirror_status = ms.ctypes.data_as(bp)
        out = {}
        if images is not None:
            nxt = np.zeros((nb + 2 * G, 2), np.float32); fst = np.zeros(nb + 2 * G, np.uint8); fund = np.zeros((2 * nb + 2 * G, 2), np.float32)
            r.next_pts = nxt.ctypes.data_as(fp); r.flow_status = fst.ctypes.data_as(bp); r.flow_und = fund.ctypes.data_as(fp)
            out.update(next_pts=nxt, flow_status=fst, flow_und=fund)
        self._check(self.lib.lvk_hip_track_chain(self.handle, ctypes.byref(d), ctypes.byref(r)))
        del keep
        out.update(H=np.array(r.H, np.float64).reshape(3, 3), rc=r.rc, signalled=r.signalled, count_dev=r.count_dev, count_host=r.count_host, mask=mask,
                   pairs_dev=pairs, mirror_matched=mm, mirror_status=ms)
        return out

    def warpmesh_apply_yuv420(self, src, mesh, bg=(255, 0, 255), nv12=False):
        rows, cols = src.shape[0], src.shape[1]
        out = _planes420_empty(rows, cols, nv12, src.device)
        m = np.ascontiguousarray(mesh, dtype=np.float32)
        ma, mp = _f32(m)
        bga, bgp = _u8x3(bg)
        self._check(self.lib.lvk_hip_warpmesh_apply_yuv420(self.handle, src.data_ptr(), src.stride(0), rows, cols, *_planes420_args(out, nv12), 1 if nv12 else 0,
                                                           mp, m.shape[0], m.shape[1], bgp))
        return out


class MeshSolver:

    def __init__(self, ctx, cols, rows, gen_region, temporal, local, max_points):
        self.ctx, self.cols, self.rows = ctx, cols, rows
        h = ctypes.c_void_p()
        ctx._check(ctx.lib.lvk_hip_mesh_solver_create(ctx.handle, cols, rows, float(gen_region[0]), float(gen_region[1]), float(temporal), float(local),
                                                      int(max_points), ctypes.byref(h)))
        self.handle = h

    def solve(self, tracked, matched, region=(480, 270), temporal=1.0, threshold=10.0):
        t = np.ascontiguousarray(tracked, np.float32).reshape(-1, 2); m = np.ascontiguousarray(matched, np.float32).reshape(-1, 2)
        inl = np.zeros(len(t), np.uint8); off = np.zeros((self.rows, self.cols, 2), np.float32)
        fp = ctypes.POINTER(ctypes.c_float)
        rc = self.ctx.lib.lvk_hip_mesh_solver_solve(self.handle, t.ctypes.data_as(fp), m.ctypes.data_as(fp), len(t), float(region[0]), float(region[1]),
                                                    float(temporal), float(threshold), inl.ctypes.data_as(ctypes.POINTER(ctypes.c_uint8)), off.ctypes.data_as(fp))
        if rc < 0:
            self.ctx._check(rc)
        return rc, inl, off

    def reset(self):
        self.ctx._check(self.ctx.lib.lvk_hip_mesh_solver_reset(self.handle))

    def close(self):
        if getattr(self, "handle", None):
            if getattr(self.ctx, "handle", None):
                self.ctx.lib.lvk_hip_mesh_solver_destroy(self.handle)
            self.handle = None
```

livevisionkit_amd/csrc/lvk_hip_internal.hpp:

```cpp
#pragma once

#include <hip/hip_runtime.h>
#include <cstdint>
#include <cstdio>
#include <string>
#include <vector>
#include <functional>
#include <map>
#include <set>
#include <mutex>
#include <utility>

#include "lvk_hip.h"
#include "planes420.hpp"

struct LinTabEntry { int s0, s1; float a0, a1; };
struct Lin8Entry { int s0, s1, a0, a1; };
struct AreaTabEntry { int si; float alpha; };
struct FastRegion { int x, y, w, h, threshold, active; };
constexpr int LVK_FAST_INLINE_REGIONS = 8;

constexpr int LVK_MAX_PYR_LEVELS = 8;
struct PyrLevel { const uint8_t* img; const short2* deriv; int rows, cols, step; };
struct PyrArgs { PyrLevel lv[LVK_MAX_PYR_LEVELS]; int nlevels; };

struct lvk_hip_ctx
{
    int remap_precision = LVK_REMAP_EXACT;
    int device = 0;
    int cu_count = 0;
    hipStream_t stream = nullptr;
    bool owns_stream = false;
    std::string last_error;

    static constexpr int kStageSlots = 16;
    static constexpr size_t kStageBytes = 64 * 1024;
    uint8_t* stage_host = nullptr;
    uint8_t* stage_dev = nullptr;
    hipEvent_t stage_done[kStageSlots] = {};
    int stage_next = 0;

    std::vector<hipStream_t> aux_streams;
    std::mutex aux_mutex;
    std::vector<std::pair<void*, std::function<int()>>> sync_hooks;

    std::mutex pool_mutex;
    std::multimap<size_t, void*> pool_free;
    std::map<void*, size_t> pool_sizes;
    std::set<void*> pool_cached;
    size_t pool_cached_bytes = 0;
    static constexpr size_t kPoolMaxCachedBytes = (size_t)4 << 30;

    std::vector<hipEvent_t> wait_events;

    std::map<std::tuple<int, int, int>, LinTabEntry*> lintabs;

    std::map<std::tuple<int, int, int>, Lin8Entry*> lin8tabs;

    struct AreaTabDev { int2* range = nullptr; AreaTabEntry* tab = nullptr; int max_taps = 0, span64 = 0, span4 = 0; };
    std::map<std::pair<int, int>, AreaTabDev> areatabs;
    std::map<std::pair<int, int>, int4*> enlargetabs;

    int fail(int code, const std::string& msg) { last_error = msg; if (code == LVK_HIP_ERR_RUNTIME) (void)hipGetLastError(); return code; }
};

struct lvk_device_guard
{
    int prev = -1; bool switched = false;
    explicit lvk_device_guard(const lvk_hip_ctx* ctx)
    {
        if (hipGetDevice(&prev) != hipSuccess) { (void)hipGetLastError(); prev = -1; }
        if (prev != ctx->device) switched = hipSetDevice(ctx->device) == hipSuccess;
    }
    ~lvk_device_guard() { if (switched && prev >= 0) (void)hipSetDevice(prev); }
    lvk_device_guard(const lvk_device_guard&) = delete;
    lvk_device_guard& operator=(const lvk_device_guard&) = delete;
};

#define LVK_HIP_ENTRY(ctx)                         \
    if (!(ctx)) return LVK_HIP_ERR_ARG;            \
    lvk_device_guard lvk_entry_device_guard(ctx)

#define LVK_HIP_CHECK(ctx, expr)                                                                      \
    do {                                                                                              \
        hipError_t _e = (expr);                                                                       \
        if (_e != hipSuccess)                                                                         \
        {                                                                                             \
            (void)hipGetLastError();    \
            return (ctx)->fail(LVK_HIP_ERR_RUNTIME, std::string(#expr) + ": " + hipGetErrorString(_e)); \
        }                                                                                             \
    } while (0)

#ifndef LVK_TRACKER_PRIO
#define LVK_TRACKER_PRIO 3
#endif
#define LVK_TRACKER_PRIORITY() __builtin_amdgcn_s_setprio(LVK_TRACKER_PRIO)

#if (defined(LVK_TIMELINE) || defined(LVK_RANSAC_TIMING) || defined(LVK_MESH_TIMING)) && !defined(LVK_PROBE_BUILD)
#error "instrumented build: pass -DLVK_PROBE_BUILD (scripts/variant_build.sh); never the library the tests and the bench load by default"
#endif

#ifdef LVK_TIMELINE
#define LVK_TL_SLOTS 4
#define LVK_TL_RING 8192
static __device__ unsigned lvk_tl_head[LVK_TL_SLOTS];
static __device__ unsigned long long lvk_tl_log[LVK_TL_SLOTS][LVK_TL_RING][2];
struct LvkTimelineScope
{
    int slot; bool sampled; unsigned long long t0;
    __device__ explicit LvkTimelineScope(int s) : slot(s), sampled(false), t0(0)
    {
        const unsigned total = gridDim.x * gridDim.y * gridDim.z;
        const unsigned b = (blockIdx.z * gridDim.y + blockIdx.y) * gridDim.x + blockIdx.x;
        sampled = threadIdx.x == 0 && threadIdx.y == 0 && ((b & 63u) == 63u || b == 0 || b == total - 1);
        if (sampled) t0 = (unsigned long long)wall_clock64();
    }
    __device__ ~LvkTimelineScope()
    {
        if (sampled)
        {
            const unsigned i = atomicAdd(&lvk_tl_head[slot], 1u) % LVK_TL_RING;
            lvk_tl_log[slot][i][0] = t0; lvk_tl_log[slot][i][1] = (unsigned long long)wall_clock64();
        }
    }
};
#define LVK_TL(slot) LvkTimelineScope lvk_tl_scope_(slot)
#define LVK_TL_EXPORT(unit)                                                                                     \
    extern "C" int lvk_tl_read_##unit(long long* out)                                                           \
    {                                                                                                           \
        unsigned idx[LVK_TL_SLOTS];                                                                             \
        if (hipDeviceSynchronize() != hipSuccess) return -1;                                                    \
        if (hipMemcpyFromSymbol(idx, HIP_SYMBOL(lvk_tl_head), sizeof(idx)) != hipSuccess) return -1;           \
        for (int s = 0; s < LVK_TL_SLOTS; s++) out[(size_t)s * (1 + 2 * LVK_TL_RING)] = idx[s];                 \
        for (int s = 0; s < LVK_TL_SLOTS; s++)                                                                  \
            if (hipMemcpyFromSymbol(out + (size_t)s * (1 + 2 * LVK_TL_RING) + 1, HIP_SYMBOL(lvk_tl_log), sizeof(long long) * 2 * LVK_TL_RING, \
                                    sizeof(long long) * 2 * LVK_TL_RING * s) != hipSuccess) return -1;         \
        return 0;                                                                                               \
    }
#else
#define LVK_TL(slot) do { } while (0)
#define LVK_TL_EXPORT(unit)
#endif

#define LVK_HIP_REQUIRE(ctx, cond)                                                                    \
    do { if (!(cond)) return (ctx)->fail(LVK_HIP_ERR_ARG, "pre-condition failed: " #cond); } while (0)

inline int lvk_format_channels(int format)
{
    switch (format)
    {
    case LVK_FORMAT_BGR: case LVK_FORMAT_RGB: case LVK_FORMAT_YUV: return 3;
    case LVK_FORMAT_BGRA: case LVK_FORMAT_RGBA: return 4;
    case LVK_FORMAT_GRAY: return 1;
    default: return 0;
    }
}

inline bool lvk_pitched_overlap(const void* a, int a_step, int a_rows, long long a_row_bytes, const void* b, int b_step, int b_rows, long long b_row_bytes)
{
    return yuv420::overlap(yuv420::span_of(a, a_step, a_rows, a_row_bytes), yuv420::span_of(b, b_step, b_rows, b_row_bytes));
}

int lvk_stage_params(lvk_hip_ctx* ctx, hipStream_t stream, const void* host, size_t bytes, void** d_out, int* slot = nullptr);
int lvk_stage_consumed(lvk_hip_ctx* ctx, int slot, hipStream_t stream);

int lvk_get_lintab(lvk_hip_ctx* ctx, int msize, int fsize, bool vertical, const LinTabEntry** d_out);

int lvk_get_areatab(lvk_hip_ctx* ctx, int ssize, int dsize, const int2** d_range, const AreaTabEntry** d_tab, int* max_taps = nullptr, int* span64 = nullptr, int* span4 = nullptr);

int lvk_launch_luma_area_resize(lvk_hip_ctx* ctx, const void* d_src, int src_step, int pix_stride, int channel,
                                int srows, int scols, void* d_dst, int dst_step, int drows, int dcols);
int lvk_launch_pyr_down(lvk_hip_ctx* ctx, const void* d_src, int src_step, int rows, int cols, void* d_dst, int dst_step);
int lvk_launch_scharr(lvk_hip_ctx* ctx, const void* d_src, int src_step, int rows, int cols, void* d_dst);
struct PyrArgs;
int lvk_launch_pyramid(lvk_hip_ctx* ctx, const PyrArgs& args, bool derivs = false);

int lvk_fast_workspace_bytes(int nregions, int max_rw, int max_rh, size_t* masks_bytes, size_t* scores_bytes);
int lvk_launch_fast(lvk_hip_ctx* ctx, const void* d_img, int step, int rows, int cols,
                    const FastRegion* d_regions, int nregions, int max_rw, int max_rh,
                    void* d_masks, void* d_scores, uint32_t* d_out, int cap, int* d_counts, const FastRegion* host_regions = nullptr);

struct FastInsertDesc
{
    const uint16_t* col_of; const uint32_t* row_base; const uint8_t* bucket;
    uint32_t* cell_first; void* cell_best ; int* region_count;
    const uint32_t* occ;
    const int* occ_bucket;
    int capacity; bool small_grid; int n_held, min_samples; float uniformity, homography_threshold;
    float2* pts; uint32_t* new_kp; int* result; int* d_n; int* d_full; int* counts;
};
int lvk_launch_fast_insert(lvk_hip_ctx* ctx, const void* d_img, int step, int rows, int cols, const FastRegion* host_regions, int nregions,
                           int max_rw, int max_rh, void* d_masks, void* d_scores, const FastInsertDesc& d);
bool lvk_fast_insert_fits(int cells, int nregions, int max_rw, int max_rh, int cols, int rows);
int lvk_fast_cells_reset(lvk_hip_ctx* ctx, uint32_t* d_first, void* d_best, int cells, int* d_region_count );

struct LensModel;
int lvk_pyramid_geometry(int rows, int cols, int max_level, int win_w, int win_h, int* lrows, int* lcols);
int lvk_launch_pyrlk(lvk_hip_ctx* ctx, const PyrArgs& prev, const PyrArgs& next, const float2* d_prev_pts, int n,
                     float2* d_next_pts, uint8_t* d_status, int win_w, int win_h, int max_count, double epsilon, double min_eig,
                     float2* d_prev_copy = nullptr,
                     const LensModel* lens = nullptr, double lens_sx = 0.0, double lens_sy = 0.0, float2* d_und = nullptr,
                     const int* d_n = nullptr);

struct DevicePyramid
{
    uint8_t* img_base = nullptr;
    uint8_t* deriv_base = nullptr;
    PyrArgs args{};
    int allocate(lvk_hip_ctx* ctx, int rows, int cols, int max_level, int win_w, int win_h);
    int build(lvk_hip_ctx* ctx, bool derivs = false);
    void release();
};

struct LvkHostSignal { unsigned* flag; unsigned seq; };

size_t lvk_ransac_workspace_bytes(int n);
int lvk_launch_ransac(lvk_hip_ctx* ctx, const float2* d_p1, const float2* d_p2, int n, double threshold, double region_w, double region_h,
                      bool full_homography, void* d_ws, double* d_H, int* d_ninl, uint8_t* d_mask, const int* d_n = nullptr,
                      const int* d_full = nullptr,
                      LvkHostSignal done = LvkHostSignal{nullptr, 0},
                      int lo_mode = 0);
int lvk_launch_match_compact(lvk_hip_ctx* ctx, const float2* d_prev, const float2* d_matched, const uint8_t* d_status, int n,
                             float2* d_p1, float2* d_p2, int* d_count, int* h_count, float2* h_matched, uint8_t* h_status,
                             const float2* d_und = nullptr, float region_w = 0.0f, float region_h = 0.0f,
                             const int* d_n_raw = nullptr);
constexpr int LVK_COMPACT_RANSAC_MAX = 2048;
int lvk_launch_compact_ransac(lvk_hip_ctx* ctx, const float2* d_prev, const float2* d_matched, const uint8_t* d_status, int n,
                              float2* d_p1, float2* d_p2, int* d_count, int* h_count, float2* h_matched, uint8_t* h_status,
                              const float2* d_und, float region_wf, float region_hf,
                              double threshold, double region_w, double region_h, bool full_homography, void* d_ws, double* d_H, int* d_ninl, uint8_t* d_mask,
                              const int* d_n_raw = nullptr, const int* d_full = nullptr, LvkHostSignal done = LvkHostSignal{nullptr, 0});

struct LvkTrackChain
{
    const PyrArgs* prev_pyr = nullptr; const PyrArgs* next_pyr = nullptr;
    const float2* h_pts = nullptr;
    int win_w = 0, win_h = 0, max_count = 0; double epsilon = 0.0, min_eig = 0.0;
    const LensModel* lens = nullptr; double lens_sx = 0.0, lens_sy = 0.0;
    int n = 0; const int* d_n = nullptr;
    bool full = false; const int* d_full = nullptr;
    float2* d_pts = nullptr; float2* d_matched = nullptr; uint8_t* d_status = nullptr;
    float2* d_und = nullptr;
    float2* d_p1 = nullptr; float2* d_p2 = nullptr; int* d_count = nullptr;
    int* h_count = nullptr; float2* h_matched = nullptr; uint8_t* h_status = nullptr;
    int region_w = 0, region_h = 0; double threshold = 0.0;
    bool separate_compact = false;
    bool estimate = true;
    void* d_ws = nullptr; double* h_H = nullptr; int* h_ninl = nullptr; uint8_t* h_mask = nullptr;
    LvkHostSignal done{nullptr, 0};
    void (*stage_boundary)(void* user) = nullptr; void* user = nullptr;
};
int lvk_launch_track_chain(lvk_hip_ctx* ctx, const LvkTrackChain& c);

struct LensArgs;
struct RemapLaunch
{
    hipStream_t stream = nullptr;
    int precision = LVK_REMAP_EXACT;
    const LensArgs* lens = nullptr;
    bool co_scheduled = false;
    int co_blocks_per_cu = 0;
};
int lvk_launch_remap_homography(lvk_hip_ctx* ctx, const void* d_src, int src_step, int src_rows, int src_cols,
                                void* d_dst, int dst_step, int dst_rows, int dst_cols, int off_x, int off_y,
                                const float H[9], const uint8_t bg[3], int yuv, const RemapLaunch& o);
int lvk_launch_remap_mesh(lvk_hip_ctx* ctx, const void* d_src, int src_step, int src_rows, int src_cols,
                          void* d_dst, int dst_step, const float* mesh, int mesh_rows, int mesh_cols, const uint8_t bg[3], int yuv, const RemapLaunch& o);

int lvk_launch_ingest_yuv420(lvk_hip_ctx* ctx, hipStream_t stream, const void* d_y, int y_step, const void* d_u, int u_step,
                             const void* d_v, int v_step, int nv12, int rows, int cols, void* d_dst, int dst_step);
int lvk_launch_egress_yuv420(lvk_hip_ctx* ctx, hipStream_t stream, const void* d_src, int src_step, int rows, int cols,
                             void* d_y, int y_step, void* d_u, int u_step, void* d_v, int v_step, int nv12);
int lvk_ingest_obs_check(lvk_hip_ctx* ctx, int video_format, const void* const d_planes[3], const int steps[3], int rows, int cols);
int lvk_launch_ingest_obs(lvk_hip_ctx* ctx, hipStream_t stream, int video_format, const void* const d_planes[3], const int steps[3],
                          int rows, int cols, void* d_dst, int dst_step);
int lvk_launch_egress_obs(lvk_hip_ctx* ctx, hipStream_t stream, int video_format, const void* d_src, int src_step, int rows, int cols,
                          void* const d_planes[3], const int steps[3]);


int lvk_launch_remap_map(lvk_hip_ctx* ctx, const void* d_src, int src_step, int rows, int cols,
                         void* d_dst, int dst_step, const void* d_map, int map_step, const uint8_t bg[3], int yuv, const RemapLaunch& o);

struct LensModel { double d[17]; float f[17]; int view[4]; };
struct LensModelD { double d[17]; };
__device__ __forceinline__ float2 lvk_lens_undistort_point(const LensModelD& M, double sx, double sy, float2 p)
{
    const double nfx = M.d[0], nfy = M.d[1], ncx = M.d[2], ncy = M.d[3], fx = M.d[4], fy = M.d[5], cx = M.d[6], cy = M.d[7];
    const double k1 = M.d[8], k2 = M.d[9], p1 = M.d[10], p2 = M.d[11], k3 = M.d[12];
    const double kxc = M.d[13], vxc = M.d[14], kyc = M.d[15], vyc = M.d[16];
    const double s = (double)p.x * sx, t = (double)p.y * sy;
    double u = s, v = t;
    for (int pass = 0; pass < 2; pass++)
    {
        const double s1 = s - (u * kxc + vxc), t1 = t - (v * kyc + vyc);
        const double x0 = (s1 - cx) / fx, y0 = (t1 - cy) / fy;
        double x = x0, y = y0;
        for (int j = 0; j < 5; j++)
        {
            const double r2 = x * x + y * y;
            const double icdist = 1.0 / (1 + ((k3 * r2 + k2) * r2 + k1) * r2);
            if (icdist < 0) { x = x0; y = y0; break; }
            const double dX = 2 * p1 * x * y + p2 * (r2 + 2 * x * x);
            const double dY = p1 * (r2 + 2 * y * y) + 2 * p2 * x * y;
            x = (x0 - dX) * icdist;
            y = (y0 - dY) * icdist;
        }
        u = x * nfx + ncx; v = y * nfy + ncy;
    }
    return make_float2((float)(u / sx), (float)(v / sy));
}
struct LensArgs { float f[17]; };
int lvk_lens_model_build(const lvk_camera_params& params, int rows, int cols, LensModel& out);
void lvk_lens_build_offsets(const lvk_camera_params& params, int rows, int cols, std::vector<float>& offsets, int view[4]);
int lvk_launch_lens_undistort(lvk_hip_ctx* ctx, hipStream_t stream, const LensModel& model, double sx, double sy,
                              const float2* a, int na, const float2* b, int nb, float2* out);
int lvk_launch_warpmesh_apply_lens(lvk_hip_ctx* ctx, const void* d_src, int src_step, int rows, int cols,
                                   void* d_dst, int dst_step, const float* mesh, int mesh_rows, int mesh_cols, const uint8_t bg[3], int yuv, const RemapLaunch& o);

int lvk_launch_remap_homography_gray(lvk_hip_ctx* ctx, const void* d_src, int src_step, int src_rows, int src_cols,
                                     void* d_dst, int dst_step, int dst_rows, int dst_cols, int off_x, int off_y, const float H[9], uint8_t bg, const RemapLaunch& o);
int lvk_launch_remap_mesh_gray(lvk_hip_ctx* ctx, const void* d_src, int src_step, int rows, int cols, void* d_dst, int dst_step,
                               const float* mesh, int mesh_rows, int mesh_cols, uint8_t bg, const RemapLaunch& o);
int lvk_launch_remap_map_gray(lvk_hip_ctx* ctx, const void* d_src, int src_step, int rows, int cols,
                              void* d_dst, int dst_step, const void* d_map, int map_step, uint8_t bg, const RemapLaunch& o);
int lvk_launch_warpmesh_apply_lens_gray(lvk_hip_ctx* ctx, const void* d_src, int src_step, int rows, int cols, void* d_dst, int dst_step,
                                        const float* mesh, int mesh_rows, int mesh_cols, uint8_t bg, const RemapLaunch& o);

int lvk_launch_remap_homography_c4(lvk_hip_ctx* ctx, const void* d_src, int src_step, int src_rows, int src_cols,
                                   void* d_dst, int dst_step, int dst_rows, int dst_cols, int off_x, int off_y, const float H[9], const uint8_t bg[4], const RemapLaunch& o);
int lvk_launch_remap_mesh_c4(lvk_hip_ctx* ctx, const void* d_src, int src_step, int rows, int cols, void* d_dst, int dst_step,
                             const float* mesh, int mesh_rows, int mesh_cols, const uint8_t bg[4], const RemapLaunch& o);
int lvk_launch_remap_map_c4(lvk_hip_ctx* ctx, const void* d_src, int src_step, int rows, int cols,
                            void* d_dst, int dst_step, const void* d_map, int map_step, const uint8_t bg[4], const RemapLaunch& o);
int lvk_launch_warpmesh_apply_lens_c4(lvk_hip_ctx* ctx, const void* d_src, int src_step, int rows, int cols, void* d_dst, int dst_step,
                                      const float* mesh, int mesh_rows, int mesh_cols, const uint8_t bg[4], const RemapLaunch& o);

int lvk_launch_draw_grid(lvk_hip_ctx* ctx, hipStream_t stream, void* d_dst, int dst_step, int rows, int cols, int grid_w, int grid_h,
                         const uint8_t colour[3], int thickness);
int lvk_launch_draw_crosses(lvk_hip_ctx* ctx, hipStream_t stream, void* d_dst, int dst_step, int rows, int cols, const float* pts, int n,
                            float scale_x, float scale_y, const uint8_t colour[3], int cross_size, int thickness);

int lvk_launch_upscale(lvk_hip_ctx* ctx, hipStream_t stream, const void* d_src, int src_step, int src_rows, int src_cols,
                       void* d_dst, int dst_step, int dst_rows, int dst_cols, int yuv);
int lvk_launch_sharpen(lvk_hip_ctx* ctx, hipStream_t stream, const void* d_src, int src_step, int rows, int cols,
                       void* d_dst, int dst_step, float sharpness);

struct lvk_mesh_solver_dev;
int lvk_mesh_solver_create(lvk_hip_ctx* ctx, int cols, int rows, float gen_w, float gen_h, float temporal, float local, lvk_mesh_solver_dev** out);
void lvk_mesh_solver_free(lvk_mesh_solver_dev* s);
int lvk_mesh_solver_reset(lvk_mesh_solver_dev* s, hipStream_t stream);
int lvk_mesh_solver_cols(const lvk_mesh_solver_dev* s);
int lvk_mesh_solver_rows(const lvk_mesh_solver_dev* s);
int lvk_launch_mesh_solve(lvk_mesh_solver_dev* s, hipStream_t stream, void* d_scratch , const float2* d_p1, const float2* d_p2, const int* d_count, int n_pts,
                          int min_samples, float region_w, float region_h, float temporal_now, float threshold,
                          float* h_offsets, uint8_t* h_mask, int* h_status);

int lvk_launch_warpmesh_apply_420(lvk_hip_ctx* ctx, const void* d_src, int src_step, int rows, int cols,
                                  void* o_y, int oy_step, void* o_u, int ou_step, void* o_v, int ov_step, int nv12,
                                  const float* mesh, int mesh_rows, int mesh_cols, const uint8_t bg[3], const RemapLaunch& o);
bool lvk_remap_obs_fusable(int video_format);
int lvk_launch_warpmesh_apply_obs(lvk_hip_ctx* ctx, int video_format, const void* d_src, int src_step, int rows, int cols,
                                  void* const planes[3], const int steps[3], const float* mesh, int mesh_rows, int mesh_cols, const uint8_t bg[3], const RemapLaunch& o);
int lvk_launch_remap_map_obs(lvk_hip_ctx* ctx, int video_format, const void* d_src, int src_step, int rows, int cols,
                             void* const planes[3], const int steps[3], const void* d_map, int map_step, const uint8_t bg[3], const RemapLaunch& o);
```

livevisionkit_amd/csrc/pyrlk.hip:

```cpp
#include "lvk_hip_internal.hpp"

#include <climits>

namespace {

__device__ __forceinline__ int reflect101(int p, int len)
{
    if (len == 1) return 0;
    while (p < 0 || p >= len) { p = (p < 0) ? -p : 2 * (len - 1) - p; }
    return p;
}

constexpr int LK_MARGIN = 8;

__host__ __device__ inline size_t lvk_pyrlk_part_offset(int win_w, int win_h)
{
    const size_t tarea = (size_t)(win_w + 1) * (win_h + 1), area = (size_t)win_w * win_h;
    const size_t earea = (size_t)(win_w + 3) * (win_h + 3);
    const size_t jarea = (size_t)(win_w + 1 + 2 * LK_MARGIN) * (win_h + 1 + 2 * LK_MARGIN);
    return ((tarea * 4 + area * 6 + earea + jarea) + 15) & ~(size_t)15;
}

__device__ __forceinline__ int descale(int x, int n) { return (x + (1 << (n - 1))) >> n; }

__device__ __forceinline__ long long wave_sum(long long v)
{
#pragma unroll
    for (int o = 32; o >= 1; o >>= 1) v += __shfl_xor(v, o);
    return v;
}

__device__ __forceinline__ int wave_sum_i32(int v)
{
    v += __builtin_amdgcn_update_dpp(0, v, 0x111, 0xf, 0xf, true);
    v += __builtin_amdgcn_update_dpp(0, v, 0x112, 0xf, 0xf, true);
    v += __builtin_amdgcn_update_dpp(0, v, 0x114, 0xf, 0xf, true);
    v += __builtin_amdgcn_update_dpp(0, v, 0x118, 0xf, 0xf, true);
    v += __builtin_amdgcn_update_dpp(0, v, 0x142, 0xa, 0xf, false);
    v += __builtin_amdgcn_update_dpp(0, v, 0x143, 0xc, 0xf, false);
    return __builtin_amdgcn_readlane(v, 63);
}

template <int K>
__device__ __forceinline__ void wave_sums(long long (&v)[K])
{
#pragma unroll
    for (int k = 0; k < K; k++)
    {
        const int lo = (int)(v[k] & 0xffff), hi = (int)(v[k] >> 16);
        v[k] = (long long)wave_sum_i32(hi) * 65536 + (long long)wave_sum_i32(lo);
    }
}

__device__ __forceinline__ int row_sum_i32(int v)
{
    v += __builtin_amdgcn_update_dpp(0, v, 0x111, 0xf, 0xf, true);
    v += __builtin_amdgcn_update_dpp(0, v, 0x112, 0xf, 0xf, true);
    v += __builtin_amdgcn_update_dpp(0, v, 0x114, 0xf, 0xf, true);
    v += __builtin_amdgcn_update_dpp(0, v, 0x118, 0xf, 0xf, true);
    return v;
}

__device__ __forceinline__ int cross_row_sum_i32(int v)
{
    v += __builtin_amdgcn_update_dpp(0, v, 0x142, 0xa, 0xf, false);
    v += __builtin_amdgcn_update_dpp(0, v, 0x143, 0xc, 0xf, false);
    return __builtin_amdgcn_readlane(v, 63);
}

__device__ __forceinline__ void wave_sums_row32(int a, int b, long long (&v)[2])
{
    const int ra = row_sum_i32(a), rb = row_sum_i32(b);
    v[0] = (long long)cross_row_sum_i32(ra >> 16) * 65536 + (long long)cross_row_sum_i32(ra & 0xffff);
    v[1] = (long long)cross_row_sum_i32(rb >> 16) * 65536 + (long long)cross_row_sum_i32(rb & 0xffff);
}

template <int WIN>
struct LkWalk
{
    static constexpr int TRIPS = WIN > 0 ? (WIN * WIN + 63) / 64 : 1;
    static constexpr bool ROW32 = WIN > 0 && WIN * WIN <= 128;
    static_assert(!ROW32 || (long long)TRIPS * 16 * 8160 * 4080 < (1ll << 31), "a DPP row's partial of diff * Ix must fit int32");
};

__device__ __forceinline__ void bilinear_weights(float a, float b, int& w00, int& w01, int& w10, int& w11)
{
    w00 = (int)__builtin_rintf((1.f - a) * (1.f - b) * 16384.0f);
    w01 = (int)__builtin_rintf(a * (1.f - b) * 16384.0f);
    w10 = (int)__builtin_rintf((1.f - a) * b * 16384.0f);
    w11 = 16384 - w00 - w01 - w10;
}

struct LevelState
{
    float A11, A12, A22, Dinv;
    int jx0, jy0;
    int skip;
    int pad;
};

__device__ __forceinline__ void wave_lds_sync()
{
    __builtin_amdgcn_fence(__ATOMIC_RELEASE, "wavefront");
    __builtin_amdgcn_wave_barrier();
    __builtin_amdgcn_fence(__ATOMIC_ACQUIRE, "wavefront");
}

__device__ __forceinline__ int reflect101_fast(int p, int len)
{
    if (len == 1) return 0;
    p = p < 0 ? -p : p;
    p = p >= len ? 2 * (len - 1) - p : p;
    while (p < 0 || p >= len) { p = (p < 0) ? -p : 2 * (len - 1) - p; }
    return p;
}

struct WindowSrc { const uint8_t* img; int rows, cols, step, x0, y0, w, h; };

template <int CHUNK>
__device__ __forceinline__ void window_loads(uint8_t (&v)[CHUNK], const WindowSrc& s, int base, int lane)
{
    const int total = s.w * s.h;
    const float rw = 1.0f / (float)s.w;
#pragma unroll
    for (int k = 0; k < CHUNK; k++)
    {
        const int idx = min(base + k * 64 + lane, total - 1);
        int ty = (int)(((float)idx + 0.5f) * rw), tx = idx - ty * s.w;
        if (tx < 0) { ty--; tx += s.w; }
        if (tx >= s.w) { ty++; tx -= s.w; }
        v[k] = s.img[(long)reflect101_fast(s.y0 + ty, s.rows) * s.step + reflect101_fast(s.x0 + tx, s.cols)];
    }
}

template <int CHUNK>
__device__ __forceinline__ void window_stores(uint8_t* __restrict__ tile, const uint8_t (&v)[CHUNK], int total, int base, int lane)
{
#pragma unroll
    for (int k = 0; k < CHUNK; k++)
    {
        const int idx = base + k * 64 + lane;
        if (idx < total) tile[idx] = v[k];
    }
}

template <int CHUNK>
__device__ __forceinline__ void stage_window(uint8_t* __restrict__ tile, const WindowSrc& s, int lane)
{
    const int total = s.w * s.h;
    for (int base = 0; base < total; base += 64 * CHUNK)
    {
        uint8_t v[CHUNK];
        window_loads<CHUNK>(v, s, base, lane);
        window_stores<CHUNK>(tile, v, total, base, lane);
    }
}

struct __attribute__((packed, aligned(1))) LkU4B { uint32_t w; };

__device__ __forceinline__ bool window_is_interior(const WindowSrc& s)
{
    const int dpr = (s.w + 3) >> 2;
    return s.x0 >= 0 && s.y0 >= 0 && s.x0 + 4 * dpr <= s.cols && s.y0 + s.h <= s.rows;
}

template <int CHUNK>
__device__ __forceinline__ void interior_loads(uint32_t (&v)[CHUNK], const WindowSrc& s, int lane)
{
    const int dpr = (s.w + 3) >> 2, total = s.h * dpr;
    const float rd = 1.0f / (float)dpr;
    const uint8_t* origin = s.img + (long)s.y0 * s.step + s.x0;
#pragma unroll
    for (int k = 0; k < CHUNK; k++)
    {
        const int q = min(k * 64 + lane, total - 1);
        int ty = (int)(((float)q + 0.5f) * rd), tq = q - ty * dpr;
        if (tq < 0) { ty--; tq += dpr; }
        if (tq >= dpr) { ty++; tq -= dpr; }
        v[k] = reinterpret_cast<const LkU4B*>(origin + ty * s.step + 4 * tq)->w;
    }
}

template <int CHUNK>
__device__ __forceinline__ void interior_stores(uint8_t* __restrict__ tile, const uint32_t (&v)[CHUNK], const WindowSrc& s, int lane)
{
    const int dpr = (s.w + 3) >> 2, total = s.h * dpr;
    const float rd = 1.0f / (float)dpr;
#pragma unroll
    for (int k = 0; k < CHUNK; k++)
    {
        const int q = k * 64 + lane;
        int ty = (int)(((float)q + 0.5f) * rd), tq = q - ty * dpr;
        if (tq < 0) { ty--; tq += dpr; }
        if (tq >= dpr) { ty++; tq -= dpr; }
        if (q < total)
        {
            uint8_t* d = tile + ty * s.w + 4 * tq;
            const int nb = min(4, s.w - 4 * tq);
            d[0] = (uint8_t)v[k];
            if (nb > 1) d[1] = (uint8_t)(v[k] >> 8);
            if (nb > 2) d[2] = (uint8_t)(v[k] >> 16);
            if (nb > 3) d[3] = (uint8_t)(v[k] >> 24);
        }
    }
}

template <int CA, int CB, int FA, int FB>
__device__ __forceinline__ void stage_two_windows(uint8_t* __restrict__ ta, const WindowSrc& a, uint8_t* __restrict__ tb, const WindowSrc& b, bool b_valid, int lane)
{
    const bool fa = window_is_interior(a) && a.h * ((a.w + 3) >> 2) <= 64 * FA;
    const bool fb = b_valid && window_is_interior(b) && b.h * ((b.w + 3) >> 2) <= 64 * FB;
    if (fa && fb)
    {
        uint32_t va[FA], vb[FB];
        interior_loads<FA>(va, a, lane);
        interior_loads<FB>(vb, b, lane);
        interior_stores<FA>(ta, va, a, lane);
        interior_stores<FB>(tb, vb, b, lane);
        return;
    }
    const int na = a.w * a.h, nb = b_valid ? b.w * b.h : 0;
    for (int t = 0; t * 64 * CA < na || t * 64 * CB < nb; t++)
    {
        const bool do_a = t * 64 * CA < na, do_b = t * 64 * CB < nb;
        uint8_t va[CA], vb[CB];
        if (do_a) window_loads<CA>(va, a, t * 64 * CA, lane);
        if (do_b) window_loads<CB>(vb, b, t * 64 * CB, lane);
        if (do_a) window_stores<CA>(ta, va, na, t * 64 * CA, lane);
        if (do_b) window_stores<CB>(tb, vb, nb, t * 64 * CB, lane);
    }
}

template <int CB, int FB>
__device__ __forceinline__ void stage_one_window(uint8_t* __restrict__ tb, const WindowSrc& b, int lane)
{
    if (window_is_interior(b) && b.h * ((b.w + 3) >> 2) <= 64 * FB)
    {
        uint32_t vb[FB];
        interior_loads<FB>(vb, b, lane);
        interior_stores<FB>(tb, vb, b, lane);
        return;
    }
    stage_window<CB>(tb, b, lane);
}

struct LensPointArgs { LensModelD model; double sx, sy; float2* und; const int* n_dev; };
template <int WIN, bool LENS>
__global__ __launch_bounds__(64 * LVK_MAX_PYR_LEVELS)
void k_pyrlk(PyrArgs prev, PyrArgs next, const float2* __restrict__ prev_pts, float2* __restrict__ prev_copy, int n,
             float2* __restrict__ next_pts, uint8_t* __restrict__ status,
             int win_w_arg, int win_h_arg, int max_count, double epsilon_sq, float min_eig_threshold, int level_bytes_arg, LensPointArgs la)
{
    LVK_TL(0);
    LVK_TRACKER_PRIORITY();
    const int win_w = WIN ? WIN : win_w_arg, win_h = WIN ? WIN : win_h_arg;
    const int level_bytes = WIN ? (int)lvk_pyrlk_part_offset(WIN, WIN) : level_bytes_arg;
    extern __shared__ __attribute__((aligned(16))) uint8_t smem[];
    const int pt = blockIdx.x;
    if (la.n_dev) { n = min(max(*la.n_dev, 0), n); if (pt >= n) return; }
    const int lane = threadIdx.x & 63, wave = threadIdx.x >> 6;
    const int tw = win_w + 1, th = win_h + 1, area = win_w * win_h, tarea = tw * th;
    const int jw = tw + 2 * LK_MARGIN, jh = th + 2 * LK_MARGIN;
    const int ew = tw + 2, eh = th + 2;
    LevelState* states = reinterpret_cast<LevelState*>(smem + (size_t)prev.nlevels * level_bytes);
    const int py0 = lane / win_w, px0 = lane - py0 * win_w, pdy_ = 64 / win_w, pdx_ = 64 - pdy_ * win_w;
    const int lx = lane & 15, ly = lane >> 4;

    const float2 p0 = prev_pts[pt];
    if (threadIdx.x == 0 && prev_copy) prev_copy[pt] = p0;
    const float halfx = (win_w - 1) * 0.5f, halfy = (win_h - 1) * 0.5f;
    const float FLT_SCALE = 1.f / (1 << 20);
    const int top = prev.nlevels - 1;

#ifdef LVK_LK_TIMING
    long long lt[8]; int ln = 0; int iters_total = 0;
    lt[ln++] = wall_clock64();
#endif
    {
        const int level = wave;
        uint8_t* base = smem + (size_t)level * level_bytes;
        short2* dtile = reinterpret_cast<short2*>(base);
        short* Iw = reinterpret_cast<short*>(base + (size_t)tarea * 4);
        short* Ixw = Iw + area;
        short* Iyw = Ixw + area;
        uint8_t* etile = reinterpret_cast<uint8_t*>(Iyw + area);
        uint8_t* jtile = etile + ew * eh;
        const PyrLevel I = prev.lv[level];
        const PyrLevel J = next.lv[level];
        float px = p0.x * (float)(1. / (1 << level));
        float py = p0.y * (float)(1. / (1 << level));
        const float nx = px, ny = py;
        LevelState st;
        st.A11 = st.A12 = st.A22 = st.Dinv = 0.f; st.jx0 = st.jy0 = INT_MIN / 2; st.skip = 0; st.pad = 0;
        px -= halfx; py -= halfy;
        const int ipx = (int)__builtin_floorf(px), ipy = (int)__builtin_floorf(py);
        if (ipx < -win_w || ipx >= I.cols || ipy < -win_h || ipy >= I.rows) st.skip = 1;
        else
        {
            const float a = px - ipx, b = py - ipy;
            int w00, w01, w10, w11;
            bilinear_weights(a, b, w00, w01, w10, w11);
            int jx0 = (int)__builtin_floorf(nx - halfx), jy0 = (int)__builtin_floorf(ny - halfy);
            const bool j_valid = !(jx0 < -win_w || jx0 >= J.cols || jy0 < -win_h || jy0 >= J.rows);
            jx0 = j_valid ? jx0 - LK_MARGIN : INT_MIN / 2; jy0 = j_valid ? jy0 - LK_MARGIN : INT_MIN / 2;
            stage_two_windows<4, 13, 1, 4>(etile, WindowSrc{I.img, I.rows, I.cols, I.step, ipx - 1, ipy - 1, ew, eh},
                                     jtile, WindowSrc{J.img, J.rows, J.cols, J.step, jx0, jy0, jw, jh}, j_valid, lane);
            wave_lds_sync();
            for (int ty = ly; ty < th; ty += 4)
                for (int tx = lx; tx < tw; tx += 16)
                {
                    const int xx = ipx + tx, yy = ipy + ty;
                    short2 d = make_short2(0, 0);
                    if (xx >= 0 && yy >= 0 && xx < I.cols && yy < I.rows)
                    {
                        const uint8_t* r0 = etile + ty * ew + tx; const uint8_t* r1 = r0 + ew; const uint8_t* r2 = r1 + ew;
                        const int t0m = (r0[0] + r2[0]) * 3 + r1[0] * 10, t0p = (r0[2] + r2[2]) * 3 + r1[2] * 10;
                        const int t1m = r2[0] - r0[0], t1c = r2[1] - r0[1], t1p = r2[2] - r0[2];
                        d = make_short2((short)(t0p - t0m), (short)((t1p + t1m) * 3 + t1c * 10));
                    }
                    dtile[ty * tw + tx] = d;
                }
            wave_lds_sync();
            const uint8_t* tile = etile + ew + 1;
            long long sA[3] = {0, 0, 0};
            for (int p = lane, y = py0, x = px0; p < area; p += 64)
            {
                const int i00 = y * tw + x, i01 = i00 + 1, i10 = i00 + tw, i11 = i10 + 1;
                const int e00 = y * ew + x, e01 = e00 + 1, e10 = e00 + ew, e11 = e10 + 1;
                const int ival = descale(__mul24(tile[e00], w00) + __mul24(tile[e01], w01) + __mul24(tile[e10], w10) + __mul24(tile[e11], w11), 14 - 5);
                const int ixval = descale(__mul24(dtile[i00].x, w00) + __mul24(dtile[i01].x, w01) + __mul24(dtile[i10].x, w10) + __mul24(dtile[i11].x, w11), 14);
                const int iyval = descale(__mul24(dtile[i00].y, w00) + __mul24(dtile[i01].y, w01) + __mul24(dtile[i10].y, w10) + __mul24(dtile[i11].y, w11), 14);
                Iw[p] = (short)ival; Ixw[p] = (short)ixval; Iyw[p] = (short)iyval;
                sA[0] += (long long)__mul24(ixval, ixval);
                sA[1] += (long long)__mul24(ixval, iyval);
                sA[2] += (long long)__mul24(iyval, iyval);
                y += pdy_; x += pdx_; if (x >= win_w) { x -= win_w; y++; }
            }
            wave_sums<3>(sA);
            const float A11 = (float)(double)sA[0] * FLT_SCALE, A12 = (float)(double)sA[1] * FLT_SCALE, A22 = (float)(double)sA[2] * FLT_SCALE;
            const float D = A11 * A22 - A12 * A12;
            const float minEig = (A22 + A11 - __builtin_sqrtf((A11 - A22) * (A11 - A22) + 4.f * A12 * A12)) / (float)(2 * win_w * win_h);
            if (minEig < min_eig_threshold || D < 1.1920928955078125e-07f) st.skip = 1;
            else { st.A11 = A11; st.A12 = A12; st.A22 = A22; st.Dinv = 1.f / D; st.jx0 = jx0; st.jy0 = jy0; }
        }
        if (lane == 0) states[level] = st;
    }
#ifdef LVK_LK_TIMING
    lt[ln++] = wall_clock64();
#endif
    __syncthreads();
    if (wave != 0) return;
#ifdef LVK_LK_TIMING
    lt[ln++] = wall_clock64();
#endif

    float outx = 0.f, outy = 0.f;
    bool ok = true;
    constexpr int TRIPS = LkWalk<WIN>::TRIPS;
    int joff[TRIPS];
    if constexpr (LkWalk<WIN>::ROW32)
    {
#pragma unroll
        for (int r = 0; r < TRIPS; r++)
        {
            const int p = lane + 64 * r;
            joff[r] = p < area ? (p / WIN) * jw + p % WIN : py0 * jw + px0;
        }
    }
    for (int level = top; level >= 0; level--)
    {
        const PyrLevel J = next.lv[level];
        const LevelState st = states[level];
        uint8_t* base = smem + (size_t)level * level_bytes;
        const short* Iw = reinterpret_cast<const short*>(base + (size_t)tarea * 4);
        const short* Ixw = Iw + area;
        const short* Iyw = Ixw + area;
        uint8_t* jtile = base + (size_t)tarea * 4 + (size_t)area * 6 + ew * eh;
        float nx, ny;
        if (level == top) { nx = p0.x * (float)(1. / (1 << level)); ny = p0.y * (float)(1. / (1 << level)); }
        else { nx = outx * 2.f; ny = outy * 2.f; }
        outx = nx; outy = ny;
        if (st.skip)
        {
            if (level == 0) ok = false;
            continue;
        }
        const float A11 = st.A11, A12 = st.A12, A22 = st.A22, D = st.Dinv;
        int jx0 = st.jx0, jy0 = st.jy0;
        nx -= halfx; ny -= halfy;
        float pdx = 0.f, pdy = 0.f;
        int Ip[TRIPS], Ixp[TRIPS], Iyp[TRIPS];
        if constexpr (LkWalk<WIN>::ROW32)
        {
#pragma unroll
            for (int r = 0; r < TRIPS; r++)
            {
                const bool in = lane + 64 * r < area;
                const int p = in ? lane + 64 * r : lane;
                const int iv = Iw[p], ixv = Ixw[p], iyv = Iyw[p];
                Ip[r] = in ? iv : 0; Ixp[r] = in ? ixv : 0; Iyp[r] = in ? iyv : 0;
            }
        }
        for (int j = 0; j < max_count; j++)
        {
            const int inx = (int)__builtin_floorf(nx), iny = (int)__builtin_floorf(ny);
            if (inx < -win_w || inx >= J.cols || iny < -win_h || iny >= J.rows)
            {
                if (level == 0) ok = false;
                break;
            }
            const float a = nx - inx, b = ny - iny;
            int w00, w01, w10, w11;
            bilinear_weights(a, b, w00, w01, w10, w11);
            if (inx < jx0 || iny < jy0 || inx + tw > jx0 + jw || iny + th > jy0 + jh)
            {
                jx0 = inx - LK_MARGIN; jy0 = iny - LK_MARGIN;
                wave_lds_sync();
                stage_one_window<13, 4>(jtile, WindowSrc{J.img, J.rows, J.cols, J.step, jx0, jy0, jw, jh}, lane);
                wave_lds_sync();
            }
            const uint8_t* jt = jtile + (iny - jy0) * jw + (inx - jx0);
            long long sb[2] = {0, 0};
            if constexpr (LkWalk<WIN>::ROW32)
            {
                int s0 = 0, s1 = 0;
#pragma unroll
                for (int r = 0; r < TRIPS; r++)
                {
                    const int i00 = joff[r], i01 = i00 + 1, i10 = i00 + jw, i11 = i10 + 1;
                    const int diff = descale(__mul24(jt[i00], w00) + __mul24(jt[i01], w01) + __mul24(jt[i10], w10) + __mul24(jt[i11], w11), 14 - 5) - Ip[r];
                    s0 += __mul24(diff, Ixp[r]);
                    s1 += __mul24(diff, Iyp[r]);
                }
                wave_sums_row32(s0, s1, sb);
            }
            else
            {
                for (int p = lane, y = py0, x = px0; p < area; p += 64)
                {
                    const int i00 = y * jw + x, i01 = i00 + 1, i10 = i00 + jw, i11 = i10 + 1;
                    const int diff = descale(__mul24(jt[i00], w00) + __mul24(jt[i01], w01) + __mul24(jt[i10], w10) + __mul24(jt[i11], w11), 14 - 5) - Iw[p];
                    sb[0] += (long long)__mul24(diff, Ixw[p]);
                    sb[1] += (long long)__mul24(diff, Iyw[p]);
                    y += pdy_; x += pdx_; if (x >= win_w) { x -= win_w; y++; }
                }
                wave_sums<2>(sb);
            }
            const float b1 = (float)(double)sb[0] * FLT_SCALE, b2 = (float)(double)sb[1] * FLT_SCALE;
            const float dx = (A12 * b2 - A22 * b1) * D;
            const float dy = (A12 * b1 - A11 * b2) * D;
            nx += dx; ny += dy;
            outx = nx + halfx; outy = ny + halfy;
            if ((double)dx * (double)dx + (double)dy * (double)dy <= epsilon_sq) break;
            if (j > 0 && (double)__builtin_fabsf(dx + pdx) < 0.01 && (double)__builtin_fabsf(dy + pdy) < 0.01)
            {
                outx -= dx * 0.5f; outy -= dy * 0.5f;
                break;
            }
            pdx = dx; pdy = dy;
#ifdef LVK_LK_TIMING
            iters_total++;
#endif
        }
#ifdef LVK_LK_TIMING
        if (ln < 8) lt[ln++] = wall_clock64();
#endif
    }
#ifdef LVK_LK_TIMING
    if (lane == 0 && (pt == 0 || pt == 300) && n > 400)
    {
        printf("pyrlk pt %d (100 MHz ticks): phase A %lld, barrier %lld, levels", pt, lt[1] - lt[0], lt[2] - lt[1]);
        for (int k = 3; k < ln; k++) printf(" %lld", lt[k] - lt[k - 1]);
        printf(" | full iterations %d\n", iters_total);
    }
#endif
    if (lane == 0)
    {
        next_pts[pt] = make_float2(outx, outy);
        status[pt] = ok ? 1 : 0;
    }
    if (LENS && lane < 2)
    {
        const float2 q = lvk_lens_undistort_point(la.model, la.sx, la.sy, lane == 0 ? p0 : make_float2(outx, outy));
        la.und[lane == 0 ? pt : n + pt] = q;
    }
}

}

size_t lvk_pyrlk_lds_bytes(int win_w, int win_h, int nlevels)
{
    return (size_t)nlevels * lvk_pyrlk_part_offset(win_w, win_h) + (size_t)nlevels * sizeof(LevelState);
}

int lvk_launch_pyrlk(lvk_hip_ctx* ctx, const PyrArgs& prev, const PyrArgs& next, const float2* d_prev_pts, int n,
                     float2* d_next_pts, uint8_t* d_status, int win_w, int win_h, int max_count, double epsilon, double min_eig, float2* d_prev_copy,
                     const LensModel* lens, double lens_sx, double lens_sy, float2* d_und, const int* d_n)
{
    LVK_HIP_REQUIRE(ctx, prev.nlevels >= 1 && prev.nlevels == next.nlevels && prev.nlevels <= LVK_MAX_PYR_LEVELS);
    LVK_HIP_REQUIRE(ctx, win_w >= 3 && win_h >= 3 && win_w <= 31 && win_h <= 31);
    if (n <= 0) return LVK_HIP_OK;
    max_count = std::min(std::max(max_count, 0), 100);
    epsilon = std::min(std::max(epsilon, 0.), 10.);
    epsilon *= epsilon;
    const size_t lds = lvk_pyrlk_lds_bytes(win_w, win_h, prev.nlevels);
    LensPointArgs la{};
    const bool with_lens = lens != nullptr && d_und != nullptr;
    if (with_lens) { for (int i = 0; i < 17; i++) la.model.d[i] = lens->d[i]; la.sx = lens_sx; la.sy = lens_sy; la.und = d_und; }
    la.n_dev = d_n;
    auto launch = [&](auto kernel) -> int {
        if (lds > 48 * 1024)
            LVK_HIP_CHECK(ctx, hipFuncSetAttribute(reinterpret_cast<const void*>(kernel), hipFuncAttributeMaxDynamicSharedMemorySize, (int)lds));
        hipLaunchKernelGGL(kernel, dim3(n), dim3(64 * prev.nlevels), lds, ctx->stream, prev, next, d_prev_pts, d_prev_copy, n,
                           d_next_pts, d_status, win_w, win_h, max_count, epsilon, (float)min_eig, (int)lvk_pyrlk_part_offset(win_w, win_h), la);
        return LVK_HIP_OK;
    };
    int lrc;
    if (win_w == 11 && win_h == 11) lrc = with_lens ? launch(k_pyrlk<11, true>) : launch(k_pyrlk<11, false>);
    else lrc = with_lens ? launch(k_pyrlk<0, true>) : launch(k_pyrlk<0, false>);
    if (lrc != LVK_HIP_OK) return lrc;
    LVK_HIP_CHECK(ctx, hipGetLastError());
    return LVK_HIP_OK;
}

int lvk_pyramid_geometry(int rows, int cols, int max_level, int win_w, int win_h, int* lrows, int* lcols)
{
    int n = 0;
    lrows[n] = rows; lcols[n] = cols; n++;
    for (int level = 1; level <= max_level && n < LVK_MAX_PYR_LEVELS; level++)
    {
        const int r = (lrows[n - 1] + 1) / 2, c = (lcols[n - 1] + 1) / 2;
        if (c <= win_w || r <= win_h) break;
        lrows[n] = r; lcols[n] = c; n++;
    }
    return n;
}

int DevicePyramid::allocate(lvk_hip_ctx* ctx, int rows, int cols, int max_level, int win_w, int win_h)
{
    release();
    int lr[LVK_MAX_PYR_LEVELS], lc[LVK_MAX_PYR_LEVELS];
    const int n = lvk_pyramid_geometry(rows, cols, max_level, win_w, win_h, lr, lc);
    size_t img_bytes = 0, der_bytes = 0;
    for (int i = 0; i < n; i++) { img_bytes += (size_t)lr[i] * ((lc[i] + 63) & ~63); der_bytes += (size_t)lr[i] * lc[i] * 4; }
    LVK_HIP_CHECK(ctx, hipMalloc((void**)&img_base, img_bytes));
    LVK_HIP_CHECK(ctx, hipMalloc((void**)&deriv_base, der_bytes));
    uint8_t* ip = img_base; uint8_t* dp = deriv_base;
    args.nlevels = n;
    for (int i = 0; i < n; i++)
    {
        const int step = (lc[i] + 63) & ~63;
        args.lv[i].img = ip; args.lv[i].deriv = reinterpret_cast<const short2*>(dp);
        args.lv[i].rows = lr[i]; args.lv[i].cols = lc[i]; args.lv[i].step = step;
        ip += (size_t)lr[i] * step; dp += (size_t)lr[i] * lc[i] * 4;
    }
    return LVK_HIP_OK;
}

void DevicePyramid::release()
{
    if (img_base) (void)hipFree(img_base);
    if (deriv_base) (void)hipFree(deriv_base);
    img_base = deriv_base = nullptr;
    args.nlevels = 0;
}

int DevicePyramid::build(lvk_hip_ctx* ctx, bool derivs) { return lvk_launch_pyramid(ctx, args, derivs); }

extern "C" {

int lvk_hip_pyrlk(lvk_hip_ctx* ctx, const void* d_prev, int prev_step, const void* d_next, int next_step, int rows, int cols,
                  const float* prev_pts, int n, float* next_pts, uint8_t* status,
                  int win_w, int win_h, int max_level, int max_count, double epsilon, double min_eig_threshold)
{
    LVK_HIP_ENTRY(ctx);
    LVK_HIP_REQUIRE(ctx, d_prev && d_next && rows > 0 && cols > 0 && n >= 0 && (n == 0 || (prev_pts && next_pts && status)));
    DevicePyramid P, N;
    int rc;
    if ((rc = P.allocate(ctx, rows, cols, max_level, win_w, win_h)) != LVK_HIP_OK) return rc;
    if ((rc = N.allocate(ctx, rows, cols, max_level, win_w, win_h)) != LVK_HIP_OK) { P.release(); return rc; }
    float2 *d_p = nullptr, *d_n = nullptr; uint8_t* d_s = nullptr;
    auto cleanup = [&]() { P.release(); N.release(); if (d_p) (void)hipFree(d_p); if (d_n) (void)hipFree(d_n); if (d_s) (void)hipFree(d_s); };
    hipError_t e;
    if ((e = hipMemcpy2DAsync(const_cast<uint8_t*>(P.args.lv[0].img), P.args.lv[0].step, d_prev, prev_step, cols, rows, hipMemcpyDeviceToDevice, ctx->stream)) != hipSuccess ||
        (e = hipMemcpy2DAsync(const_cast<uint8_t*>(N.args.lv[0].img), N.args.lv[0].step, d_next, next_step, cols, rows, hipMemcpyDeviceToDevice, ctx->stream)) != hipSuccess)
    { cleanup(); return ctx->fail(LVK_HIP_ERR_RUNTIME, hipGetErrorString(e)); }
    if ((rc = P.build(ctx)) != LVK_HIP_OK || (rc = N.build(ctx)) != LVK_HIP_OK) { cleanup(); return rc; }
    if (n > 0)
    {
        if ((e = hipMalloc((void**)&d_p, n * sizeof(float2))) != hipSuccess || (e = hipMalloc((void**)&d_n, n * sizeof(float2))) != hipSuccess ||
            (e = hipMalloc((void**)&d_s, n)) != hipSuccess ||
            (e = hipMemcpyAsync(d_p, prev_pts, n * sizeof(float2), hipMemcpyHostToDevice, ctx->stream)) != hipSuccess)
        { cleanup(); return ctx->fail(LVK_HIP_ERR_RUNTIME, hipGetErrorString(e)); }
        if ((rc = lvk_launch_pyrlk(ctx, P.args, N.args, d_p, n, d_n, d_s, win_w, win_h, max_count, epsilon, min_eig_threshold)) != LVK_HIP_OK) { cleanup(); return rc; }
        if ((e = hipMemcpyAsync(next_pts, d_n, n * sizeof(float2), hipMemcpyDeviceToHost, ctx->stream)) != hipSuccess ||
            (e = hipMemcpyAsync(status, d_s, n, hipMemcpyDeviceToHost, ctx->stream)) != hipSuccess)
        { cleanup(); return ctx->fail(LVK_HIP_ERR_RUNTIME, hipGetErrorString(e)); }
    }
    e = hipStreamSynchronize(ctx->stream);
    cleanup();
    if (e != hipSuccess) return ctx->fail(LVK_HIP_ERR_RUNTIME, hipGetErrorString(e));
    return P.args.nlevels >= 0 ? LVK_HIP_OK : LVK_HIP_ERR_RUNTIME;
}


int lvk_hip_build_pyramid(lvk_hip_ctx* ctx, const void* d_img, int step, int rows, int cols, int max_level, int win_w, int win_h,
                          uint8_t* levels, int16_t* derivs, int* level_rows, int* level_cols)
{
    LVK_HIP_ENTRY(ctx);
    LVK_HIP_REQUIRE(ctx, d_img && levels && derivs && level_rows && level_cols && rows > 0 && cols > 0 && step >= cols);
    DevicePyramid P;
    int rc;
    if ((rc = P.allocate(ctx, rows, cols, max_level, win_w, win_h)) != LVK_HIP_OK) return rc;
    hipError_t e = hipMemcpy2DAsync(const_cast<uint8_t*>(P.args.lv[0].img), P.args.lv[0].step, d_img, step, cols, rows, hipMemcpyDeviceToDevice, ctx->stream);
    if (e == hipSuccess && (rc = P.build(ctx, true)) == LVK_HIP_OK)
    {
        size_t lo = 0, dofs = 0;
        for (int i = 0; i < P.args.nlevels && e == hipSuccess; i++)
        {
            const PyrLevel& L = P.args.lv[i];
            level_rows[i] = L.rows; level_cols[i] = L.cols;
            e = hipMemcpy2DAsync(levels + lo, L.cols, L.img, L.step, L.cols, L.rows, hipMemcpyDeviceToHost, ctx->stream);
            if (e == hipSuccess) e = hipMemcpyAsync(derivs + dofs, L.deriv, (size_t)L.rows * L.cols * 4, hipMemcpyDeviceToHost, ctx->stream);
            lo += (size_t)L.rows * L.cols; dofs += (size_t)L.rows * L.cols * 2;
        }
        if (e == hipSuccess) e = hipStreamSynchronize(ctx->stream);
    }
    const int n = P.args.nlevels;
    P.release();
    if (e != hipSuccess) return ctx->fail(LVK_HIP_ERR_RUNTIME, hipGetErrorString(e));
    return rc == LVK_HIP_OK ? n : rc;
}

}

LVK_TL_EXPORT(pyrlk)
```

livevisionkit_amd/csrc/stabilizer.hip:

```cpp
#include "stab_state.hpp"

using namespace lvkstab;

int lvk_hip_stab::track(const QueuedFrame& f, const void* luma, int luma_step, int luma_pix, int luma_channel, WarpMeshF& motion, bool& have_motion)
{
    have_motion = false;
    tracking_stability = 0.0f;
    last_detected = last_matched = 0; last_distribution = 0.0f;
    hipStream_t st = ctx->stream;
    int rc;

    cur ^= 1;
    std::swap(prev_w, cur_w); std::swap(prev_h, cur_h);
    cur_w = s.detection_width; cur_h = s.detection_height;
    DevicePyramid& C = pyr[cur];
    DevicePyramid& P = pyr[cur ^ 1];
    int pe = 0;
    const bool built_ahead = ahead_built_for == push_seq && ahead_built.same(luma, luma_step, luma_pix, luma_channel, f.rows, f.cols) && pyr_w == cur_w && pyr_h == cur_h;
    ahead_built = LumaAhead(); ahead_built_for = 0;
    if (built_ahead) lookahead_frames++;
    else
    {
        pe = prof_begin(LVK_STAGE_DOWNSCALE);
        if ((rc = lvk_launch_luma_area_resize(ctx, luma, luma_step, luma_pix, luma_channel, f.rows, f.cols, const_cast<uint8_t*>(C.args.lv[0].img), C.args.lv[0].step, cur_h, cur_w)) != LVK_HIP_OK) return rc;
        prof_end(pe);
        pe = prof_begin(LVK_STAGE_PYRAMID);
        if ((rc = C.build(ctx)) != LVK_HIP_OK) return rc;
        prof_end(pe);
    }
    trace.mark(HostTrace::DOWN_PYR_LAUNCH);
    finish_post();
    if (post_error) { post_error = false; return fail(LVK_HIP_ERR_RUNTIME, "GPU-side fast_filter disagrees with the host's"); }
    auto leave_early = [&]() -> int { if (luma_pix != 3) LVK_HIP_CHECK(ctx, hipStreamSynchronize(st)); return LVK_HIP_OK; };
    if (!initialized || cur_w != prev_w || cur_h != prev_h) { initialized = true; return leave_early(); }

    grid.plan(plan);
    bool any = false;
    for (size_t i = 0; i < plan.size(); i++) { h_regions[i] = plan[i]; any = any || plan[i].active; }
    const size_t n_held = grid.held.size();
    const size_t n_bound = std::min(cap_features, n_held + (grid.capacity() - grid.used_cells()));
    const bool dev_insert = any && device_grid && grid.device_insert_ok() && (int)plan.size() <= LVK_FAST_INLINE_REGIONS &&
                            lvk_fast_insert_fits((int)grid.capacity(), (int)plan.size(), fast_max_rw, fast_max_rh, cur_w, cur_h) && n_bound >= 1 && n_bound <= 4096;
    float distribution = 0.0f;
    if (dev_insert)
    {
        for (size_t i = 0; i < n_held; i++) h_pts[i] = make_float2(grid.held[i].x, grid.held[i].y);
        int occ_bucket[16];
        grid.occupancy(h_occ, occ_bucket);
        const FastInsertDesc d{d_grid_col, d_grid_row, d_grid_bucket, d_cell_first, d_cell_best, d_region_count, h_occ, occ_bucket, (int)grid.capacity(), grid.grid_cols() <= 4 || grid.grid_rows() <= 4, (int)n_held,
                               s.min_motion_samples, s.uniformity_threshold, HOMOGRAPHY_DISTRIBUTION_THRESHOLD, h_pts, h_new_kp, h_insert, d_n_points, d_full, h_fast_counts};
        pe = prof_begin(LVK_STAGE_FAST);
        if ((rc = lvk_launch_fast_insert(ctx, C.args.lv[0].img, C.args.lv[0].step, cur_h, cur_w, h_regions, (int)plan.size(), fast_max_rw, fast_max_rh,
                                         d_fast_masks, d_fast_scores, d)) != LVK_HIP_OK) return rc;
        prof_end(pe);
        device_grid_frames++;
    }
    else
    {
    if (any)
    {
        pe = prof_begin(LVK_STAGE_FAST);
        if ((rc = lvk_launch_fast(ctx, C.args.lv[0].img, C.args.lv[0].step, cur_h, cur_w, h_regions, (int)plan.size(), fast_max_rw, fast_max_rh,
                                  d_fast_masks, d_fast_scores, h_fast_out, fast_cap, h_fast_counts, h_regions)) != LVK_HIP_OK) return rc;
        prof_end(pe);
        LVK_HIP_CHECK(ctx, hipStreamSynchronize(st));
        trace.mark(HostTrace::FAST_SYNC);
        host_grid_frames++;
    }
    for (size_t i = 0; i < plan.size(); i++)
        if (plan[i].active) grid.absorb(i, h_fast_out + i * (size_t)fast_cap, std::min(h_fast_counts[i], fast_cap));
    distribution = grid.finish(tracked);
    last_distribution = distribution; last_detected = (int)tracked.size();
    if (tracked.size() < (size_t)s.min_motion_samples || distribution < s.uniformity_threshold) { tracked.clear(); return leave_early(); }
    if (tracked.size() > cap_features) return fail(LVK_HIP_ERR_RUNTIME, "feature count exceeds the suppression grid capacity");
    }

    trace.mark(HostTrace::GRID);
    int n = dev_insert ? (int)n_bound : (int)tracked.size();
    if (!dev_insert) for (int i = 0; i < n; i++) h_pts[i] = make_float2(tracked[i].x, tracked[i].y);
    const int* dn = dev_insert ? d_n_points : nullptr;
    const int* dfull = dev_insert ? d_full : nullptr;
    const bool full = distribution > HOMOGRAPHY_DISTRIBUTION_THRESHOLD;
    const bool chained = n <= 4096;
    const bool field = s.track_local_motions != 0;
    LvkHostSignal done{nullptr, 0};
    if (chained && !field && !caller_runs_free)
    {
        if (!h_chain_flag) { LVK_HIP_CHECK(ctx, hipHostMalloc((void**)&h_chain_flag, 64, hipHostMallocCoherent)); *h_chain_flag = 0; }
        done = LvkHostSignal{h_chain_flag, ++chain_seq};
    }
    pe = prof_begin(LVK_STAGE_PYRLK);
    if (chained)
    {
        struct Stage { lvk_hip_stab* self; int* pe; } stage{this, &pe};
        LvkTrackChain c;
        c.prev_pyr = &P.args; c.next_pyr = &C.args; c.h_pts = h_pts;
        c.win_w = LK_WIN; c.win_h = LK_WIN; c.max_count = LK_ITERS; c.epsilon = LK_EPS; c.min_eig = LK_MIN_EIG;
        c.lens = lens ? &lens_model : nullptr; c.lens_sx = (double)f.cols / (double)cur_w; c.lens_sy = (double)f.rows / (double)cur_h;
        c.n = n; c.d_n = dn; c.full = full; c.d_full = dfull;
        c.d_pts = d_pts; c.d_matched = d_matched; c.d_status = d_status; c.d_und = lens ? d_und : nullptr;
        c.d_p1 = d_p1; c.d_p2 = d_p1 + cap_features; c.d_count = d_count; c.h_count = h_count; c.h_matched = h_matched; c.h_status = h_status;
        c.region_w = cur_w; c.region_h = cur_h; c.threshold = s.acceptance_threshold;
        c.separate_compact = field; c.estimate = !field;
        c.d_ws = d_ransac_ws; c.h_H = h_H; c.h_ninl = h_ninl; c.h_mask = h_mask; c.done = done;
        c.stage_boundary = [](void* u) { Stage* g = (Stage*)u; g->self->prof_end(*g->pe); *g->pe = g->self->prof_begin(LVK_STAGE_MOTION); };
        c.user = &stage;
        if ((rc = lvk_launch_track_chain(ctx, c)) != LVK_HIP_OK) return rc;
        if (field)
        {
            if ((rc = lvk_launch_mesh_solve(mesh_dev, st, d_mesh_scratch, d_p1, d_p1 + cap_features, d_count, n, s.min_motion_samples, (float)cur_w, (float)cur_h,
                                            s.temporal_smoothing, s.acceptance_threshold, h_offsets, h_mask, h_mesh_status)) != LVK_HIP_OK) return rc;
        }
        prof_end(pe);
    }
    else
    {
        LVK_HIP_CHECK(ctx, hipMemcpyAsync(d_pts, h_pts, n * sizeof(float2), hipMemcpyHostToDevice, st));
        if ((rc = lvk_launch_pyrlk(ctx, P.args, C.args, d_pts, n, h_matched, h_status, LK_WIN, LK_WIN, LK_ITERS, LK_EPS, LK_MIN_EIG)) != LVK_HIP_OK) return rc;
        prof_end(pe);
    }
    trace.mark(HostTrace::LK_LAUNCH);
    bool chain_event_armed = false;
    if (deferred_ingest && tracker_ingest_capable)
    {
        const hipError_t q = hipStreamQuery(remap_stream);
        if (q != hipSuccess) (void)hipGetLastError();
        ingest_on_tracker = ingest_placement == 1 || (ingest_placement == 0 && ((q == hipErrorNotReady && !host_direct_now) || ingest_wait[0] != nullptr));
    }
    const bool build_ahead = chained && ahead_announced.luma != nullptr && pyr_w == cur_w && pyr_h == cur_h;
    if (chained && ((deferred_ingest && tracker_ingest_capable && ingest_on_tracker) || build_ahead))
    {
        if (!chain_done) LVK_HIP_CHECK(ctx, hipEventCreateWithFlags(&chain_done, hipEventDisableTiming));
        LVK_HIP_CHECK(ctx, hipEventRecord(chain_done, st)); chain_event_armed = true;
    }
    if (deferred_ingest && (rc = run_deferred_ingest()) != LVK_HIP_OK) return rc;
    if (build_ahead && (rc = launch_build_ahead(P, cur_w, cur_h)) != LVK_HIP_OK) return rc;
    if (lens && !chained)
    {
        if ((rc = lvk_launch_lens_undistort(ctx, st, lens_model, (double)f.cols / (double)cur_w, (double)f.rows / (double)cur_h,
                                            d_pts, n, h_matched, n, h_und)) != LVK_HIP_OK) return rc;
    }
    bool have_results = false;
    if (done.flag)
    {
        const unsigned expect = signal_test_lose ? done.seq + 0x40000000u : done.seq;
        const auto t0 = std::chrono::steady_clock::now();
        const auto budget = std::chrono::microseconds(signal_spin_us);
        for (unsigned spins = 0;; spins++)
        {
            if (__atomic_load_n(done.flag, __ATOMIC_ACQUIRE) == expect) { have_results = true; break; }
            if ((spins & 63u) == 63u && std::chrono::steady_clock::now() - t0 > budget) break;
            lvk_cpu_relax();
        }
        sched[have_results ? LVK_SCHED_WAIT_SIGNAL_WORD : LVK_SCHED_WAIT_WORD_TIMEOUT]++;
    }
    if (!have_results)
    {
        if (chain_event_armed) LVK_HIP_CHECK(ctx, hipEventSynchronize(chain_done));
        else LVK_HIP_CHECK(ctx, hipStreamSynchronize(st));
        sched[LVK_SCHED_WAIT_EVENT]++;
    }
    trace.mark(HostTrace::LK_SYNC);

    if (dev_insert)
    {
        const int n_new = h_insert[0];
        float q_dev; std::memcpy(&q_dev, &h_insert[2], sizeof(float));
        if (n_new < 0 || (size_t)n_new > grid.capacity()) return fail(LVK_HIP_ERR_RUNTIME, "device suppression grid returned an impossible count");
        distribution = grid.finish_device(tracked, h_new_kp, n_new, h_fast_counts, fast_cap);
        last_distribution = distribution; last_detected = (int)tracked.size();
        if (distribution != q_dev || tracked.size() != n_held + (size_t)n_new)
            return fail(LVK_HIP_ERR_RUNTIME, "device suppression grid disagrees with the host's bookkeeping");
        if (tracked.size() < (size_t)s.min_motion_samples || distribution < s.uniformity_threshold) { tracked.clear(); return LVK_HIP_OK; }
        if (tracked.size() > cap_features) return fail(LVK_HIP_ERR_RUNTIME, "feature count exceeds the suppression grid capacity");
        n = (int)tracked.size();
    }
    if (chained)
    {
        const int m = *h_count;
        last_matched = m;
        if (m < 0 || m > n) return fail(LVK_HIP_ERR_RUNTIME, "GPU-side fast_filter returned an impossible count");
        if ((size_t)m < (size_t)s.min_motion_samples) { tracked.clear(); return LVK_HIP_OK; }
        motion = WarpMeshF(s.motion_height, s.motion_width);
        if (field)
        {
            if (*h_mesh_status != 0) { tracked.clear(); return LVK_HIP_OK; }
            std::memcpy(motion.off.data(), h_offsets, motion.off.size() * sizeof(float));
        }
        else
        {
            std::memcpy(last_H, h_H, sizeof(last_H));
            motion.from_homography(last_H, (float)cur_w, (float)cur_h);
        }
        size_t inliers = 0;
        for (int i = 0; i < m; i++) inliers += h_mask[i] ? 1 : 0;
        tracking_stability = (float)inliers / (float)m;
        have_motion = true;
        post_n = n; post_m = m;
        trace.mark(HostTrace::POST);
        return LVK_HIP_OK;
    }

    if (lens && !chained)
    {
        const float w = (float)cur_w, h = (float)cur_h;
        auto inside = [&](const float2& p) { return p.x >= 0.0f && p.x < w && p.y >= 0.0f && p.y < h; };
        for (int k = 0; k < n; k++)
            if (!(inside(h_und[k]) && inside(h_und[n + k]))) h_status[k] = 0;
    }
    int m = n;
    for (int k = n - 1; k >= 0; k--)
        if (!h_status[k])
        {
            m--;
            std::swap(tracked[k], tracked[m]);
            std::swap(h_pts[k], h_pts[m]);
            std::swap(h_matched[k], h_matched[m]);
            if (lens && !chained) { std::swap(h_und[k], h_und[m]); std::swap(h_und[n + k], h_und[n + m]); }
        }
    tracked.resize(m);
    last_matched = m;
    if (chained && *h_count != m) return fail(LVK_HIP_ERR_RUNTIME, "GPU-side fast_filter disagrees with the host's");
    if ((size_t)m < (size_t)s.min_motion_samples) { tracked.clear(); return LVK_HIP_OK; }

    trace.mark(HostTrace::FILTER);
    motion = WarpMeshF(s.motion_height, s.motion_width);
    const float2* e1 = lens ? h_und : h_pts;
    const float2* e2 = lens ? h_und + n : h_matched;
    if (s.track_local_motions)
    {
        std::memcpy(h_p1, e1, m * sizeof(float2));
        std::memcpy(h_p1 + m, e2, m * sizeof(float2));
        LVK_HIP_CHECK(ctx, hipMemcpyAsync(d_p1, h_p1, 2 * (size_t)m * sizeof(float2), hipMemcpyHostToDevice, st));
        if ((rc = lvk_launch_mesh_solve(mesh_dev, st, d_mesh_scratch, d_p1, d_p1 + m, nullptr, m, 0, (float)cur_w, (float)cur_h,
                                        s.temporal_smoothing, s.acceptance_threshold, h_offsets, h_mask, h_mesh_status)) != LVK_HIP_OK) return rc;
        LVK_HIP_CHECK(ctx, hipStreamSynchronize(st));
        if (*h_mesh_status != 0)
        {
            tracked.clear();
            return LVK_HIP_OK;
        }
        std::memcpy(motion.off.data(), h_offsets, motion.off.size() * sizeof(float));
        size_t inl = 0;
        for (int i = 0; i < m; i++) inl += h_mask[i] ? 1 : 0;
        tracking_stability = (float)inl / (float)m;
        for (int i = m - 1; i >= 0; i--)
        {
            if (h_mask[i]) { tracked[i].age++; tracked[i].x = h_matched[i].x; tracked[i].y = h_matched[i].y; }
            else { std::swap(tracked[i], tracked.back()); tracked.pop_back(); }
        }
        grid.propagate(tracked);
        have_motion = true;
        return LVK_HIP_OK;
    }
    if (!chained)
    {
        std::memcpy(h_p1, e1, m * sizeof(float2));
        std::memcpy(h_p1 + m, e2, m * sizeof(float2));
        LVK_HIP_CHECK(ctx, hipMemcpyAsync(d_p1, h_p1, 2 * (size_t)m * sizeof(float2), hipMemcpyHostToDevice, st));
        pe = prof_begin(LVK_STAGE_MOTION);
        if ((rc = lvk_launch_ransac(ctx, d_p1, d_p1 + m, m, s.acceptance_threshold, (double)cur_w, (double)cur_h, full, d_ransac_ws, h_H, h_ninl, h_mask)) != LVK_HIP_OK) return rc;
        prof_end(pe);
        trace.mark(HostTrace::RANSAC_LAUNCH);
        LVK_HIP_CHECK(ctx, hipStreamSynchronize(st));
        trace.mark(HostTrace::RANSAC_SYNC);
    }
    std::memcpy(last_H, h_H, sizeof(last_H));
    motion.from_homography(last_H, (float)cur_w, (float)cur_h);

    size_t inliers = 0;
    for (int i = 0; i < m; i++) inliers += h_mask[i] ? 1 : 0;
    tracking_stability = (float)inliers / (float)m;

    for (int i = m - 1; i >= 0; i--)
    {
        if (h_mask[i]) { tracked[i].age++; tracked[i].x = h_matched[i].x; tracked[i].y = h_matched[i].y; }
        else { std::swap(tracked[i], tracked.back()); tracked.pop_back(); }
    }
    grid.propagate(tracked);
    have_motion = true;
    trace.mark(HostTrace::POST);
    return LVK_HIP_OK;
}

static const char* lvk_frame_format_name(int f);
static std::string lvk_stab_pixel_class_clash(const lvk_hip_stab* st, int bpp, int format);


int lvk_stab_push_impl(lvk_hip_stab* st, const void* d_frame, int step, int rows, int cols, uint64_t timestamp, int format,
                     const void* luma, int luma_step, int luma_pix,
                     void* d_out, int out_step, int out_rows, int* produced, uint64_t* out_timestamp, const void** released, OutPlanes420* o420,
                     lvk_frame_info* emitted, int bpp)
{
    lvk_hip_ctx* ctx = st->ctx;
    if (produced) *produced = 0;
    if (released) *released = nullptr;
    LVK_HIP_REQUIRE(ctx, bpp == 1 || bpp == 3 || bpp == 4);
    const bool gray_entry = bpp == 1, c4_entry = bpp == 4;
    if (gray_entry) LVK_HIP_REQUIRE(ctx, d_frame && rows > 0 && cols > 0 && step >= cols && format == LVK_FORMAT_GRAY && luma_pix == 1);
    else if (c4_entry) LVK_HIP_REQUIRE(ctx, d_frame && rows > 0 && cols > 0 && step >= 4 * cols && (format == LVK_FORMAT_BGRA || format == LVK_FORMAT_RGBA) && luma_pix == 4);
    else LVK_HIP_REQUIRE(ctx, d_frame && rows > 0 && cols > 0 && step >= 3 * cols);
    if (!st->buffers_ok) return ctx->fail(LVK_HIP_ERR_RUNTIME, "the last configure() failed while allocating the tracker's buffers: configure again");
    if (bpp == 3) LVK_HIP_REQUIRE(ctx, format == LVK_FORMAT_YUV || format == LVK_FORMAT_BGR || format == LVK_FORMAT_RGB);
    const int luma_channel = (gray_entry || format == LVK_FORMAT_YUV) ? 0 : ((format == LVK_FORMAT_BGR || format == LVK_FORMAT_BGRA) ? -1 : -2);
    if (bpp == 3) LVK_HIP_REQUIRE(ctx, luma_pix == 3 || format == LVK_FORMAT_YUV);
    { const std::string why = lvk_stab_pixel_class_clash(st, bpp, format); if (!why.empty()) return ctx->fail(LVK_HIP_ERR_ARG, why); }
    const QueuedFrame in{d_frame, step, rows, cols, timestamp, format};
    {
        QueuedFrame due;
        if (st->next_output(in, &due))
        {
            const bool to_planes = o420 && o420->y && (st->s.stabilize_output || st->s.crop_to_stable_region || st->lens);
            const bool planes_fit = !o420 || o420->vf != 0 ||
                                    (o420->y && o420->y_step >= due.cols && o420->u_step >= (o420->nv12 ? due.cols : due.cols / 2) &&
                                     (o420->nv12 || o420->v_step >= due.cols / 2) && o420->rows_cap >= due.rows);
            const bool fits = planes_fit && (to_planes || (d_out != nullptr && out_step >= bpp * due.cols && out_rows >= due.rows));
            if (!fits)
                return ctx->fail(LVK_HIP_ERR_ARG, "the output buffer does not hold the frame this push emits: " + std::to_string(due.cols) + " x " + std::to_string(due.rows) +
                                                      " (the DELAYED frame's own size -- lvk_hip_stab_next_output); nothing was queued");
        }
    }
    st->caller_runs_free = st->caller_free_running_now() || st->host_free_running_hint;
    if (st->caller_runs_free) { st->free_streak++; st->sync_streak = 0; }
    else
    {
        const bool grace = st->free_streak >= 8 && st->sync_streak == 0;
        st->sync_streak++;
        if (grace) st->caller_runs_free = true; else st->free_streak = 0;
    }
    st->sched[st->caller_runs_free ? LVK_SCHED_PUSH_FREE_RUNNING : LVK_SCHED_PUSH_SYNCHRONISED]++;
    { const int lrc = st->ensure_lens(rows, cols); if (lrc != LVK_HIP_OK) return lrc; }
    static const WarpMeshF identity_mesh(2, 2);
    const uint8_t bg[4] = {(uint8_t)st->s.background[0], (uint8_t)st->s.background[1], (uint8_t)st->s.background[2], st->background_alpha};

    auto enqueue = [&]() {
        if (st->queue.size() == st->queue_capacity) { if (released) *released = st->queue.front().d_ptr; st->queue.pop_front(); }
        st->queue.push_back(in);
    };
    auto emit = [&](const WarpMeshF* mesh) -> int {
        const QueuedFrame f = st->queue.front();
        st->queue.pop_front();
        int rc = LVK_HIP_OK;
        const bool side = st->overlap && mesh && st->s.stabilize_output;
        hipStream_t rs = side ? st->remap_stream : ctx->stream;
        const bool persistent = side && st->caller_runs_free;
        if (mesh) st->sched[persistent ? LVK_SCHED_REMAP_PERSISTENT : LVK_SCHED_REMAP_FULL]++;
        const int co_blocks_per_cu = (persistent && st->host_direct_now) ? 1 : 0;
        if (side && (rc = st->bulk_stream_sees_caller_work()) != LVK_HIP_OK) return rc;
        if (st->remap_wait) { const hipEvent_t e = st->remap_wait; st->remap_wait = nullptr; LVK_HIP_CHECK(ctx, hipStreamWaitEvent(rs, e, 0)); }
        st->trace.mark(HostTrace::EMIT_WAITS);
        const int pe = st->prof_begin(LVK_STAGE_REMAP, rs);
        LensArgs lens_other; const LensArgs* lens_args = nullptr;
        if (st->lens)
        {
            lens_args = &st->lens_args;
            if (f.rows != st->lens_rows || f.cols != st->lens_cols)
            {
                LensModel m;
                if (lvk_lens_model_build(st->lens_params, f.rows, f.cols, m) != LVK_HIP_OK) return ctx->fail(LVK_HIP_ERR_ARG, "invalid camera profile for the delayed frame's size");
                std::memcpy(lens_other.f, m.f, sizeof(lens_other.f)); lens_args = &lens_other;
            }
        }
        const RemapLaunch how{rs, st->remap_precision, lens_args, persistent, co_blocks_per_cu};
        if (mesh && o420 && o420->y && o420->vf != 0)
        {
            rc = lvk_launch_warpmesh_apply_obs(ctx, o420->vf, f.d_ptr, f.step, f.rows, f.cols, o420->p, o420->s, mesh->off.data(), mesh->rows, mesh->cols, bg, how);
            o420->used = true;
        }
        else if (mesh && o420 && o420->y)
        {
            rc = lvk_launch_warpmesh_apply_420(ctx, f.d_ptr, f.step, f.rows, f.cols, o420->y, o420->y_step, o420->u, o420->u_step, o420->v, o420->v_step,
                                               o420->nv12, mesh->off.data(), mesh->rows, mesh->cols, bg, how);
            o420->used = true;
        }
        else if (mesh && gray_entry) rc = lvk_launch_warpmesh_apply_lens_gray(ctx, f.d_ptr, f.step, f.rows, f.cols, d_out, out_step, mesh->off.data(), mesh->rows, mesh->cols, bg[0], how);
        else if (mesh && c4_entry) rc = lvk_launch_warpmesh_apply_lens_c4(ctx, f.d_ptr, f.step, f.rows, f.cols, d_out, out_step, mesh->off.data(), mesh->rows, mesh->cols, bg, how);
        else if (mesh) rc = lvk_launch_warpmesh_apply_lens(ctx, f.d_ptr, f.step, f.rows, f.cols, d_out, out_step, mesh->off.data(), mesh->rows, mesh->cols, bg,
                                                      f.format == LVK_FORMAT_YUV ? 1 : 0, how);
        else
        {
            hipError_t e = hipMemcpy2DAsync(d_out, out_step, f.d_ptr, f.step, (size_t)f.cols * bpp, f.rows, hipMemcpyDeviceToDevice, ctx->stream);
            if (e != hipSuccess) rc = ctx->fail(LVK_HIP_ERR_RUNTIME, hipGetErrorString(e));
        }
        st->prof_end(pe, rs);
        st->trace.mark(HostTrace::EMIT_KERNEL);
        if (rc != LVK_HIP_OK) return rc;
        if (produced) *produced = 1;
        if (out_timestamp) *out_timestamp = f.ts;
        if (emitted) *emitted = lvk_frame_info{f.rows, f.cols, f.format};
        if (side && st->pool_frames)
        {
            if (st->tracker_ingest_capable)
            {
                const int si = st->slot_index(f.d_ptr);
                if (si >= 0)
                {
                    if (!st->slot_read_done[(size_t)si]) { hipError_t e = hipEventCreateWithFlags(&st->slot_read_done[(size_t)si], hipEventDisableTiming); if (e != hipSuccess) return ctx->fail(LVK_HIP_ERR_RUNTIME, hipGetErrorString(e)); }
                    hipError_t e = hipEventRecord(st->slot_read_done[(size_t)si], rs);
                    if (e != hipSuccess) return ctx->fail(LVK_HIP_ERR_RUNTIME, hipGetErrorString(e));
                    st->slot_read_armed[(size_t)si] = 1;
                }
// ... 453 lines not shown
```

livevisionkit_amd/csrc/track_chain.hip:

```cpp
#include "lvk_hip_internal.hpp"

#include <algorithm>
#include <chrono>
#include <cstring>

int lvk_launch_track_chain(lvk_hip_ctx* ctx, const LvkTrackChain& c)
{
    int rc;
    const int n = c.n;
    if (c.prev_pyr &&
        (rc = lvk_launch_pyrlk(ctx, *c.prev_pyr, *c.next_pyr, c.h_pts, n, c.d_matched, c.d_status, c.win_w, c.win_h, c.max_count, c.epsilon, c.min_eig, c.d_pts,
                               c.d_und ? c.lens : nullptr, c.lens_sx, c.lens_sy, c.d_und, c.d_n)) != LVK_HIP_OK) return rc;
    const bool fused_compact = c.estimate && !c.separate_compact && n <= LVK_COMPACT_RANSAC_MAX;
    if (!fused_compact && (rc = lvk_launch_match_compact(ctx, c.d_pts, c.d_matched, c.d_status, n, c.d_p1, c.d_p2, c.d_count, c.h_count, c.h_matched, c.h_status,
                                                         c.d_und, (float)c.region_w, (float)c.region_h, c.d_n)) != LVK_HIP_OK) return rc;
    if (c.stage_boundary) c.stage_boundary(c.user);
    if (!c.estimate) return LVK_HIP_OK;
    if (fused_compact)
        return lvk_launch_compact_ransac(ctx, c.d_pts, c.d_matched, c.d_status, n, c.d_p1, c.d_p2, c.d_count, c.h_count, c.h_matched, c.h_status,
                                         c.d_und, (float)c.region_w, (float)c.region_h,
                                         c.threshold, (double)c.region_w, (double)c.region_h, c.full, c.d_ws, c.h_H, c.h_ninl, c.h_mask, c.d_n, c.d_full, c.done);
    return lvk_launch_ransac(ctx, c.d_p1, c.d_p2, n, c.threshold, (double)c.region_w, (double)c.region_h, c.full, c.d_ws, c.h_H, c.h_ninl, c.h_mask, c.d_count, c.d_full, c.done);
}

namespace {

struct ChainBuffers
{
    std::vector<void*> dev, host;
    DevicePyramid P, N;
    template <class T> hipError_t device(T** p, size_t count) { hipError_t e = hipMalloc((void**)p, std::max<size_t>(count, 1) * sizeof(T)); if (e == hipSuccess) dev.push_back(*p); return e; }
    template <class T> hipError_t pinned(T** p, size_t count) { hipError_t e = hipHostMalloc((void**)p, std::max<size_t>(count, 1) * sizeof(T), hipHostMallocCoherent); if (e == hipSuccess) host.push_back(*p); return e; }
    ~ChainBuffers() { for (void* p : dev) (void)hipFree(p); for (void* p : host) (void)hipHostFree(p); P.release(); N.release(); }
};

}

extern "C" int lvk_hip_track_chain(lvk_hip_ctx* ctx, const lvk_track_chain_desc* d, lvk_track_chain_result* r)
{
    LVK_HIP_ENTRY(ctx);
    LVK_HIP_REQUIRE(ctx, d && r && d->prev && d->n_bound >= 1 && d->n_bound <= 4096 && d->region_w > 0 && d->region_h > 0);
    const bool flow = d->d_prev_img != nullptr;
    LVK_HIP_REQUIRE(ctx, flow ? (d->d_next_img && d->rows > 0 && d->cols > 0 && r->next_pts && r->flow_status && (!d->lens || r->flow_und))
                              : (d->matched && d->status && !d->lens));
    LVK_HIP_REQUIRE(ctx, r->mask && r->pairs_dev && r->mirror_matched && r->mirror_status);
    const int nb = d->n_bound, G = LVK_TRACK_CHAIN_GUARD;
    const int n_eff = d->count_on_device ? std::min(std::max(d->n_word, 0), nb) : nb;
    const bool with_und = flow ? d->lens != nullptr : d->und != nullptr;
    constexpr int FILL = LVK_TRACK_CHAIN_FILL;

    ChainBuffers b;
    hipStream_t st = ctx->stream;
    float2 *h_pts, *h_matched, *d_pts, *d_matched, *d_und, *d_p; uint8_t *h_status, *h_mask, *d_status; int *h_count, *h_ninl, *d_count, *d_words; double* h_H; unsigned* h_flag; void* d_ws;
    hipError_t e;
    if ((e = b.pinned(&h_pts, nb)) != hipSuccess || (e = b.pinned(&h_matched, nb)) != hipSuccess || (e = b.pinned(&h_status, nb)) != hipSuccess ||
        (e = b.pinned(&h_mask, nb)) != hipSuccess || (e = b.pinned(&h_count, 1)) != hipSuccess || (e = b.pinned(&h_ninl, 1)) != hipSuccess ||
        (e = b.pinned(&h_H, 9)) != hipSuccess || (e = b.pinned(&h_flag, 16)) != hipSuccess ||
        (e = b.device(&d_pts, nb)) != hipSuccess || (e = b.device(&d_matched, nb + 2 * G)) != hipSuccess || (e = b.device(&d_status, nb + 2 * G)) != hipSuccess ||
        (e = b.device(&d_und, 2 * nb + 2 * G)) != hipSuccess || (e = b.device(&d_p, 2 * nb)) != hipSuccess || (e = b.device(&d_count, 1)) != hipSuccess ||
        (e = b.device(&d_words, 2)) != hipSuccess || (e = hipMalloc(&d_ws, lvk_ransac_workspace_bytes(nb))) != hipSuccess)
        return ctx->fail(LVK_HIP_ERR_RUNTIME, hipGetErrorString(e));
    b.dev.push_back(d_ws);
    std::memcpy(h_pts, d->prev, (size_t)nb * sizeof(float2));
    std::memset(h_matched, FILL, (size_t)nb * sizeof(float2)); std::memset(h_status, FILL, nb); std::memset(h_mask, FILL, nb);
    *h_count = -1; *h_ninl = -1; *h_flag = 0;
    for (int q = 0; q < 9; q++) h_H[q] = 0.0;
    const int words[2] = {d->n_word, d->full_word};
    if ((e = hipMemsetAsync(d_pts, FILL, (size_t)nb * sizeof(float2), st)) != hipSuccess ||
        (e = hipMemsetAsync(d_matched, FILL, (size_t)(nb + 2 * G) * sizeof(float2), st)) != hipSuccess ||
        (e = hipMemsetAsync(d_status, FILL, (size_t)(nb + 2 * G), st)) != hipSuccess ||
        (e = hipMemsetAsync(d_und, FILL, (size_t)(2 * nb + 2 * G) * sizeof(float2), st)) != hipSuccess ||
        (e = hipMemsetAsync(d_p, FILL, (size_t)2 * nb * sizeof(float2), st)) != hipSuccess ||
        (e = hipMemsetAsync(d_count, FILL, sizeof(int), st)) != hipSuccess ||
        (e = hipMemcpyAsync(d_words, words, sizeof(words), hipMemcpyHostToDevice, st)) != hipSuccess)
        return ctx->fail(LVK_HIP_ERR_RUNTIME, hipGetErrorString(e));

    LvkTrackChain c;
    LensModel lens_model;
    if (flow)
    {
        int rc;
        if ((rc = b.P.allocate(ctx, d->rows, d->cols, d->max_level, d->win_w, d->win_h)) != LVK_HIP_OK || (rc = b.N.allocate(ctx, d->rows, d->cols, d->max_level, d->win_w, d->win_h)) != LVK_HIP_OK) return rc;
        if ((e = hipMemcpy2DAsync(const_cast<uint8_t*>(b.P.args.lv[0].img), b.P.args.lv[0].step, d->d_prev_img, d->prev_step, d->cols, d->rows, hipMemcpyDeviceToDevice, st)) != hipSuccess ||
            (e = hipMemcpy2DAsync(const_cast<uint8_t*>(b.N.args.lv[0].img), b.N.args.lv[0].step, d->d_next_img, d->next_step, d->cols, d->rows, hipMemcpyDeviceToDevice, st)) != hipSuccess)
            return ctx->fail(LVK_HIP_ERR_RUNTIME, hipGetErrorString(e));
        if ((rc = b.P.build(ctx)) != LVK_HIP_OK || (rc = b.N.build(ctx)) != LVK_HIP_OK) return rc;
        if (d->lens)
        {
            if (lvk_lens_model_build(*d->lens, d->lens_rows, d->lens_cols, lens_model) != LVK_HIP_OK) return ctx->fail(LVK_HIP_ERR_ARG, "invalid camera profile");
            c.lens = &lens_model; c.lens_sx = d->lens_sx; c.lens_sy = d->lens_sy;
        }
        c.prev_pyr = &b.P.args; c.next_pyr = &b.N.args; c.h_pts = h_pts;
        c.win_w = d->win_w; c.win_h = d->win_h; c.max_count = d->max_count; c.epsilon = d->epsilon; c.min_eig = d->min_eig;
    }
    else
    {
        if ((e = hipMemcpyAsync(d_pts, d->prev, (size_t)nb * sizeof(float2), hipMemcpyHostToDevice, st)) != hipSuccess ||
            (e = hipMemcpyAsync(d_matched + G, d->matched, (size_t)nb * sizeof(float2), hipMemcpyHostToDevice, st)) != hipSuccess ||
            (e = hipMemcpyAsync(d_status + G, d->status, (size_t)nb, hipMemcpyHostToDevice, st)) != hipSuccess ||
            (d->und && n_eff > 0 && (e = hipMemcpyAsync(d_und + G, d->und, (size_t)2 * n_eff * sizeof(float2), hipMemcpyHostToDevice, st)) != hipSuccess))
            return ctx->fail(LVK_HIP_ERR_RUNTIME, hipGetErrorString(e));
    }
    c.n = nb; c.d_n = d->count_on_device ? d_words : nullptr;
    c.full = d->full != 0; c.d_full = d->model_on_device ? d_words + 1 : nullptr;
    c.d_pts = d_pts; c.d_matched = d_matched + G; c.d_status = d_status + G; c.d_und = with_und ? d_und + G : nullptr;
    c.d_p1 = d_p; c.d_p2 = d_p + nb; c.d_count = d_count; c.h_count = h_count; c.h_matched = h_matched; c.h_status = h_status;
    c.region_w = d->region_w; c.region_h = d->region_h; c.threshold = d->threshold;
    c.separate_compact = d->separate_compact != 0;
    c.d_ws = d_ws; c.h_H = h_H; c.h_ninl = h_ninl; c.h_mask = h_mask;
    if (d->host_signal) c.done = LvkHostSignal{h_flag, 0x5EED0001u};
    int rc = lvk_launch_track_chain(ctx, c);
    if (rc != LVK_HIP_OK) { (void)hipStreamSynchronize(st); return rc; }

    r->signalled = 0;
    if (c.done.flag)
    {
        const auto t0 = std::chrono::steady_clock::now();
        for (unsigned spins = 0;; spins++)
        {
            if (__atomic_load_n(c.done.flag, __ATOMIC_ACQUIRE) == c.done.seq) { r->signalled = 1; break; }
            if ((spins & 63u) == 63u && std::chrono::steady_clock::now() - t0 > std::chrono::seconds(2)) break;
        }
    }
    if (!r->signalled)
    {
        if ((e = hipStreamSynchronize(st)) != hipSuccess) return ctx->fail(LVK_HIP_ERR_RUNTIME, hipGetErrorString(e));
        if (c.done.flag && __atomic_load_n(c.done.flag, __ATOMIC_ACQUIRE) == c.done.seq) r->signalled = 1;
    }
    std::memcpy(r->H, h_H, 9 * sizeof(double));
    const int ninl = *h_ninl;
    r->count_host = *h_count;
    std::memcpy(r->mask, h_mask, nb);
    std::memcpy(r->mirror_matched, h_matched, (size_t)nb * sizeof(float2));
    std::memcpy(r->mirror_status, h_status, nb);
    r->count_dev = -1;
    if ((e = hipMemcpyAsync(&r->count_dev, d_count, sizeof(int), hipMemcpyDeviceToHost, st)) != hipSuccess ||
        (e = hipMemcpyAsync(r->pairs_dev, d_p, (size_t)2 * nb * sizeof(float2), hipMemcpyDeviceToHost, st)) != hipSuccess ||
        (flow && ((e = hipMemcpyAsync(r->next_pts, d_matched, (size_t)(nb + 2 * G) * sizeof(float2), hipMemcpyDeviceToHost, st)) != hipSuccess ||
                  (e = hipMemcpyAsync(r->flow_status, d_status, (size_t)(nb + 2 * G), hipMemcpyDeviceToHost, st)) != hipSuccess)) ||
        (flow && r->flow_und && (e = hipMemcpyAsync(r->flow_und, d_und, (size_t)(2 * nb + 2 * G) * sizeof(float2), hipMemcpyDeviceToHost, st)) != hipSuccess) ||
        (e = hipStreamSynchronize(st)) != hipSuccess)
        return ctx->fail(LVK_HIP_ERR_RUNTIME, hipGetErrorString(e));
    if (d->host_signal && !r->signalled) return ctx->fail(LVK_HIP_ERR_RUNTIME, "the chain completed without storing its host signal word");
    r->rc = ninl >= 0 ? ninl : -10 + ninl;
    return LVK_HIP_OK;
}
```

Measured before the change: 9839.

## Let pyramidal LK use fewer waves per feature, chosen by occupancy model

The PyrLK kernel used to launch one wave per pyramid level per feature. It now loops levels over a variable number of waves (1, 2 or 4), and the host picks that count from CU count, feature count and available wave slots, with fewer slots assumed when flow overlaps the remap. This aims to fit more feature blocks at once and to stop the flow stage crowding out the concurrent warp kernel. The cost is serialized level setup inside a block and cost constants hardcoded from profiling. Probe-only timeline logging and a forced-waves build option are also added.

```diff
diff --git a/include/lvk_hip.h b/include/lvk_hip.h
--- a/include/lvk_hip.h
+++ b/include/lvk_hip.h
@@ -332,6 +332,10 @@
                   const float* prev_pts, int n, float* next_pts, uint8_t* status,
                   int win_w, int win_h, int max_level, int max_count, double epsilon, double min_eig_threshold);
 
+int lvk_hip_pyrlk_waves(lvk_hip_ctx* ctx, const void* d_prev, int prev_step, const void* d_next, int next_step, int rows, int cols,
+                        const float* prev_pts, int n, float* next_pts, uint8_t* status,
+                        int win_w, int win_h, int max_level, int max_count, double epsilon, double min_eig_threshold, int waves_per_feature);
+
 int lvk_hip_estimate_global_motion(lvk_hip_ctx* ctx, const float* pts1, const float* pts2, int n, double threshold,
                                    double region_w, double region_h, int full_homography, double H[9], uint8_t* mask);
 
@@ -353,6 +357,7 @@
     int full, model_on_device, full_word;
     int separate_compact, host_signal;
     double threshold; int region_w, region_h;
+    int flow_waves;
 } lvk_track_chain_desc;
 typedef struct lvk_track_chain_result
 {
diff --git a/livevisionkit_amd/_native.py b/livevisionkit_amd/_native.py
--- a/livevisionkit_amd/_native.py
+++ b/livevisionkit_amd/_native.py
@@ -96,6 +96,9 @@
     "lvk_hip_pyrlk": (_c.c_int, [_P, _P, _c.c_int, _P, _c.c_int, _c.c_int, _c.c_int, _c.POINTER(_c.c_float), _c.c_int,
                                  _c.POINTER(_c.c_float), _c.POINTER(_c.c_uint8), _c.c_int, _c.c_int, _c.c_int, _c.c_int,
                                  _c.c_double, _c.c_double]),
+    "lvk_hip_pyrlk_waves": (_c.c_int, [_P, _P, _c.c_int, _P, _c.c_int, _c.c_int, _c.c_int, _c.POINTER(_c.c_float), _c.c_int,
+                                       _c.POINTER(_c.c_float), _c.POINTER(_c.c_uint8), _c.c_int, _c.c_int, _c.c_int, _c.c_int,
+                                       _c.c_double, _c.c_double, _c.c_int]),
     "lvk_hip_ingest_yuv420": (_c.c_int, [_P, _P, _c.c_int, _P, _c.c_int, _P, _c.c_int, _c.c_int, _c.c_int, _c.c_int, _P, _c.c_int]),
     "lvk_hip_egress_yuv420": (_c.c_int, [_P, _P, _c.c_int, _c.c_int, _c.c_int, _P, _c.c_int, _P, _c.c_int, _P, _c.c_int, _c.c_int]),
     "lvk_hip_ingest_obs": (_c.c_int, [_P, _c.c_int, _P * 3, _c.c_int * 3, _c.c_int, _c.c_int, _P, _c.c_int]),
diff --git a/livevisionkit_amd/context.py b/livevisionkit_amd/context.py
--- a/livevisionkit_amd/context.py
+++ b/livevisionkit_amd/context.py
@@ -53,7 +53,7 @@
                 ("n_bound", ctypes.c_int), ("count_on_device", ctypes.c_int), ("n_word", ctypes.c_int),
                 ("full", ctypes.c_int), ("model_on_device", ctypes.c_int), ("full_word", ctypes.c_int),
                 ("separate_compact", ctypes.c_int), ("host_signal", ctypes.c_int),
-                ("threshold", ctypes.c_double), ("region_w", ctypes.c_int), ("region_h", ctypes.c_int)]
+                ("threshold", ctypes.c_double), ("region_w", ctypes.c_int), ("region_h", ctypes.c_int), ("flow_waves", ctypes.c_int)]
 
 
 class TrackChainResult(ctypes.Structure):
@@ -279,6 +279,18 @@
                                            win[0], win[1], max_level, max_count, float(epsilon), float(min_eig)))
         return out, st
 
+    def pyrlk_waves(self, prev, nxt, pts, waves, win=(11, 11), max_level=3, max_count=5, epsilon=0.01, min_eig=1e-4):
+        pts = np.ascontiguousarray(pts, np.float32).reshape(-1, 2)
+        out = np.zeros_like(pts)
+        st = np.zeros(len(pts), np.uint8)
+        self._check(self.lib.lvk_hip_pyrlk_waves(self.handle, prev.data_ptr(), prev.stride(0), nxt.data_ptr(), nxt.stride(0),
+                                                 prev.shape[0], prev.shape[1],
+                                                 pts.ctypes.data_as(ctypes.POINTER(ctypes.c_float)), len(pts),
+                                                 out.ctypes.data_as(ctypes.POINTER(ctypes.c_float)),
+                                                 st.ctypes.data_as(ctypes.POINTER(ctypes.c_uint8)),
+                                                 win[0], win[1], max_level, max_count, float(epsilon), float(min_eig), int(waves)))
+        return out, st
+
     def estimate_global_motion(self, p1, p2, threshold, region=(480, 270), full_homography=True):
         p1 = np.ascontiguousarray(p1, np.float32).reshape(-1, 2); p2 = np.ascontiguousarray(p2, np.float32).reshape(-1, 2)
         H = np.zeros(9, np.float64); mask = np.zeros(len(p1), np.uint8)
@@ -495,7 +507,7 @@
         return oa[:m], ob[:m]
 
     def track_chain(self, prev, matched=None, status=None, und=None, images=None, win=(11, 11), max_level=3, max_count=5, epsilon=0.01, min_eig=1e-4,
-                    lens=None, threshold=3.0, region=(480, 270), full=True, full_word=None, n_word=None, separate_compact=False, host_signal=False):
+                    lens=None, threshold=3.0, region=(480, 270), full=True, full_word=None, n_word=None, separate_compact=False, host_signal=False, flow_waves=0):
         fp, bp = ctypes.POINTER(ctypes.c_float), ctypes.POINTER(ctypes.c_uint8)
         prev = np.ascontiguousarray(prev, np.float32).reshape(-1, 2)
         nb, G = len(prev), TRACK_CHAIN_GUARD
@@ -519,6 +531,7 @@
             d.d_prev_img = a.data_ptr(); d.prev_step = a.stride(0); d.d_next_img = b.data_ptr(); d.next_step = b.stride(0)
             d.rows, d.cols = a.shape[0], a.shape[1]
             d.win_w, d.win_h, d.max_level, d.max_count, d.epsilon, d.min_eig = win[0], win[1], max_level, max_count, float(epsilon), float(min_eig)
+            d.flow_waves = int(flow_waves)
             if lens is not None:
                 params, lrows, lcols, sx, sy = lens
                 arr = (ctypes.c_double * 9)(*[float(v) for v in params])
diff --git a/livevisionkit_amd/csrc/lvk_hip_internal.hpp b/livevisionkit_amd/csrc/lvk_hip_internal.hpp
--- a/livevisionkit_amd/csrc/lvk_hip_internal.hpp
+++ b/livevisionkit_amd/csrc/lvk_hip_internal.hpp
@@ -200,7 +200,14 @@
                      float2* d_next_pts, uint8_t* d_status, int win_w, int win_h, int max_count, double epsilon, double min_eig,
                      float2* d_prev_copy = nullptr,
                      const LensModel* lens = nullptr, double lens_sx = 0.0, double lens_sy = 0.0, float2* d_und = nullptr,
-                     const int* d_n = nullptr);
+                     const int* d_n = nullptr,
+                     int wave_slots = 0,
+                     int waves = 0);
+#ifndef LVK_FLOW_SLOTS_BESIDE_REMAP
+#define LVK_FLOW_SLOTS_BESIDE_REMAP 4
+#endif
+constexpr int LVK_FLOW_SLOTS_ALONE = 20;
+int lvk_pyrlk_choose_waves(int nlevels, int n, int cu_count, int wave_slots);
 
 struct DevicePyramid
 {
@@ -237,6 +244,7 @@
     const float2* h_pts = nullptr;
     int win_w = 0, win_h = 0, max_count = 0; double epsilon = 0.0, min_eig = 0.0;
     const LensModel* lens = nullptr; double lens_sx = 0.0, lens_sy = 0.0;
+    int flow_wave_slots = 0, flow_waves = 0;
     int n = 0; const int* d_n = nullptr;
     bool full = false; const int* d_full = nullptr;
     float2* d_pts = nullptr; float2* d_matched = nullptr; uint8_t* d_status = nullptr;
diff --git a/livevisionkit_amd/csrc/pyrlk.hip b/livevisionkit_amd/csrc/pyrlk.hip
--- a/livevisionkit_amd/csrc/pyrlk.hip
+++ b/livevisionkit_amd/csrc/pyrlk.hip
@@ -1,6 +1,10 @@
 #include "lvk_hip_internal.hpp"
 
 #include <climits>
+
+#if defined(LVK_PYRLK_FORCE_WAVES) && !defined(LVK_PROBE_BUILD)
+#error "LVK_PYRLK_FORCE_WAVES is for probe builds (scripts/variant_build.sh): the product library chooses the waves per feature per launch"
+#endif
 
 namespace {
 
@@ -20,6 +24,8 @@
     const size_t jarea = (size_t)(win_w + 1 + 2 * LK_MARGIN) * (win_h + 1 + 2 * LK_MARGIN);
     return ((tarea * 4 + area * 6 + earea + jarea) + 15) & ~(size_t)15;
 }
+
+__device__ __forceinline__ int opaque_vgpr(int v) { asm volatile("" : "+v"(v)); return v; }
 
 __device__ __forceinline__ int descale(int x, int n) { return (x + (1 << (n - 1))) >> n; }
 
@@ -245,6 +251,28 @@
 }
 
 struct LensPointArgs { LensModelD model; double sx, sy; float2* und; const int* n_dev; };
+
+#ifdef LVK_TIMELINE
+#define LVK_LK_BLOCK_RING 131072
+static __device__ unsigned lvk_lk_block_head;
+static __device__ unsigned long long lvk_lk_block_log[LVK_LK_BLOCK_RING][2];
+struct LkBlockScope
+{
+    unsigned long long t0;
+    __device__ LkBlockScope() : t0(threadIdx.x == 0 ? (unsigned long long)wall_clock64() : 0ull) {}
+    __device__ ~LkBlockScope()
+    {
+        if (threadIdx.x == 0)
+        {
+            const unsigned i = atomicAdd(&lvk_lk_block_head, 1u) % LVK_LK_BLOCK_RING;
+            lvk_lk_block_log[i][0] = t0; lvk_lk_block_log[i][1] = (unsigned long long)wall_clock64();
+        }
+    }
+};
+#define LVK_LK_BLOCK_LOG() LkBlockScope lvk_lk_block_scope_
+#else
+#define LVK_LK_BLOCK_LOG() do { } while (0)
+#endif
 template <int WIN, bool LENS>
 __global__ __launch_bounds__(64 * LVK_MAX_PYR_LEVELS)
 void k_pyrlk(PyrArgs prev, PyrArgs next, const float2* __restrict__ prev_pts, float2* __restrict__ prev_copy, int n,
@@ -258,13 +286,13 @@
     extern __shared__ __attribute__((aligned(16))) uint8_t smem[];
     const int pt = blockIdx.x;
     if (la.n_dev) { n = min(max(*la.n_dev, 0), n); if (pt >= n) return; }
-    const int lane = threadIdx.x & 63, wave = threadIdx.x >> 6;
+    LVK_LK_BLOCK_LOG();
+    const int lane = threadIdx.x & 63, wave = __builtin_amdgcn_readfirstlane(threadIdx.x >> 6), waves = blockDim.x >> 6;
     const int tw = win_w + 1, th = win_h + 1, area = win_w * win_h, tarea = tw * th;
     const int jw = tw + 2 * LK_MARGIN, jh = th + 2 * LK_MARGIN;
     const int ew = tw + 2, eh = th + 2;
     LevelState* states = reinterpret_cast<LevelState*>(smem + (size_t)prev.nlevels * level_bytes);
     const int py0 = lane / win_w, px0 = lane - py0 * win_w, pdy_ = 64 / win_w, pdx_ = 64 - pdy_ * win_w;
-    const int lx = lane & 15, ly = lane >> 4;
 
     const float2 p0 = prev_pts[pt];
     if (threadIdx.x == 0 && prev_copy) prev_copy[pt] = p0;
@@ -276,8 +304,9 @@
     long long lt[8]; int ln = 0; int iters_total = 0;
     lt[ln++] = wall_clock64();
 #endif
-    {
-        const int level = wave;
+    for (int level = wave; level < prev.nlevels; level += waves)
+    {
+        const int lane_a = opaque_vgpr(lane), py0_a = opaque_vgpr(py0), px0_a = opaque_vgpr(px0), lx_a = lane_a & 15, ly_a = lane_a >> 4;
         uint8_t* base = smem + (size_t)level * level_bytes;
         short2* dtile = reinterpret_cast<short2*>(base);
         short* Iw = reinterpret_cast<short*>(base + (size_t)tarea * 4);
@@ -304,10 +333,10 @@
             const bool j_valid = !(jx0 < -win_w || jx0 >= J.cols || jy0 < -win_h || jy0 >= J.rows);
             jx0 = j_valid ? jx0 - LK_MARGIN : INT_MIN / 2; jy0 = j_valid ? jy0 - LK_MARGIN : INT_MIN / 2;
             stage_two_windows<4, 13, 1, 4>(etile, WindowSrc{I.img, I.rows, I.cols, I.step, ipx - 1, ipy - 1, ew, eh},
-                                     jtile, WindowSrc{J.img, J.rows, J.cols, J.step, jx0, jy0, jw, jh}, j_valid, lane);
+                                     jtile, WindowSrc{J.img, J.rows, J.cols, J.step, jx0, jy0, jw, jh}, j_valid, lane_a);
             wave_lds_sync();
-            for (int ty = ly; ty < th; ty += 4)
-                for (int tx = lx; tx < tw; tx += 16)
+            for (int ty = ly_a; ty < th; ty += 4)
+                for (int tx = lx_a; tx < tw; tx += 16)
                 {
                     const int xx = ipx + tx, yy = ipy + ty;
                     short2 d = make_short2(0, 0);
@@ -323,7 +352,7 @@
             wave_lds_sync();
             const uint8_t* tile = etile + ew + 1;
             long long sA[3] = {0, 0, 0};
-            for (int p = lane, y = py0, x = px0; p < area; p += 64)
+            for (int p = lane_a, y = py0_a, x = px0_a; p < area; p += 64)
             {
                 const int i00 = y * tw + x, i01 = i00 + 1, i10 = i00 + tw, i11 = i10 + 1;
                 const int e00 = y * ew + x, e01 = e00 + 1, e10 = e00 + ew, e11 = e10 + 1;
@@ -343,7 +372,7 @@
             if (minEig < min_eig_threshold || D < 1.1920928955078125e-07f) st.skip = 1;
             else { st.A11 = A11; st.A12 = A12; st.A22 = A22; st.Dinv = 1.f / D; st.jx0 = jx0; st.jy0 = jy0; }
         }
-        if (lane == 0) states[level] = st;
+        if (lane_a == 0) states[level] = st;
     }
 #ifdef LVK_LK_TIMING
     lt[ln++] = wall_clock64();
@@ -493,13 +522,37 @@
     return (size_t)nlevels * lvk_pyrlk_part_offset(win_w, win_h) + (size_t)nlevels * sizeof(LevelState);
 }
 
+static const int LVK_PYRLK_BLOCK_TICKS[2] = {1704, 2276};
+
+int lvk_pyrlk_choose_waves(int nlevels, int n, int cu_count, int wave_slots)
+{
+    const int cus = cu_count > 0 ? cu_count : 256;
+    if (wave_slots <= 0) wave_slots = LVK_FLOW_SLOTS_ALONE;
+    int best = 0; long long best_cost = 0;
+    for (int k = 0, W = 4; k < 2; k++, W >>= 1)
+    {
+        const int w = std::min(W, nlevels);
+        const long long at_once = (long long)cus * (wave_slots / w);
+        if (at_once <= 0) continue;
+        if (n <= at_once) return w;
+        const long long cost = ((n + at_once - 1) / at_once) * LVK_PYRLK_BLOCK_TICKS[k];
+        if (!best || cost < best_cost) { best = w; best_cost = cost; }
+    }
+    return best ? best : std::min(2, nlevels);
+}
+
 int lvk_launch_pyrlk(lvk_hip_ctx* ctx, const PyrArgs& prev, const PyrArgs& next, const float2* d_prev_pts, int n,
                      float2* d_next_pts, uint8_t* d_status, int win_w, int win_h, int max_count, double epsilon, double min_eig, float2* d_prev_copy,
-                     const LensModel* lens, double lens_sx, double lens_sy, float2* d_und, const int* d_n)
+                     const LensModel* lens, double lens_sx, double lens_sy, float2* d_und, const int* d_n, int wave_slots, int waves)
 {
     LVK_HIP_REQUIRE(ctx, prev.nlevels >= 1 && prev.nlevels == next.nlevels && prev.nlevels <= LVK_MAX_PYR_LEVELS);
     LVK_HIP_REQUIRE(ctx, win_w >= 3 && win_h >= 3 && win_w <= 31 && win_h <= 31);
+    LVK_HIP_REQUIRE(ctx, waves == 0 || waves == 1 || waves == 2 || waves == 4);
     if (n <= 0) return LVK_HIP_OK;
+    waves = waves ? std::min(waves, prev.nlevels) : lvk_pyrlk_choose_waves(prev.nlevels, n, ctx->cu_count, wave_slots);
+#ifdef LVK_PYRLK_FORCE_WAVES
+    waves = std::min((int)LVK_PYRLK_FORCE_WAVES, prev.nlevels);
+#endif
     max_count = std::min(std::max(max_count, 0), 100);
     epsilon = std::min(std::max(epsilon, 0.), 10.);
     epsilon *= epsilon;
@@ -511,7 +564,7 @@
     auto launch = [&](auto kernel) -> int {
         if (lds > 48 * 1024)
             LVK_HIP_CHECK(ctx, hipFuncSetAttribute(reinterpret_cast<const void*>(kernel), hipFuncAttributeMaxDynamicSharedMemorySize, (int)lds));
-        hipLaunchKernelGGL(kernel, dim3(n), dim3(64 * prev.nlevels), lds, ctx->stream, prev, next, d_prev_pts, d_prev_copy, n,
+        hipLaunchKernelGGL(kernel, dim3(n), dim3(64 * waves), lds, ctx->stream, prev, next, d_prev_pts, d_prev_copy, n,
                            d_next_pts, d_status, win_w, win_h, max_count, epsilon, (float)min_eig, (int)lvk_pyrlk_part_offset(win_w, win_h), la);
         return LVK_HIP_OK;
     };
@@ -573,8 +626,17 @@
                   const float* prev_pts, int n, float* next_pts, uint8_t* status,
                   int win_w, int win_h, int max_level, int max_count, double epsilon, double min_eig_threshold)
 {
+    return lvk_hip_pyrlk_waves(ctx, d_prev, prev_step, d_next, next_step, rows, cols, prev_pts, n, next_pts, status, win_w, win_h, max_level, max_count,
+                               epsilon, min_eig_threshold, 0);
+}
+
+int lvk_hip_pyrlk_waves(lvk_hip_ctx* ctx, const void* d_prev, int prev_step, const void* d_next, int next_step, int rows, int cols,
+                        const float* prev_pts, int n, float* next_pts, uint8_t* status,
+                        int win_w, int win_h, int max_level, int max_count, double epsilon, double min_eig_threshold, int waves_per_feature)
+{
     LVK_HIP_ENTRY(ctx);
     LVK_HIP_REQUIRE(ctx, d_prev && d_next && rows > 0 && cols > 0 && n >= 0 && (n == 0 || (prev_pts && next_pts && status)));
+    LVK_HIP_REQUIRE(ctx, waves_per_feature == 0 || waves_per_feature == 1 || waves_per_feature == 2 || waves_per_feature == 4);
     DevicePyramid P, N;
     int rc;
     if ((rc = P.allocate(ctx, rows, cols, max_level, win_w, win_h)) != LVK_HIP_OK) return rc;
@@ -592,7 +654,8 @@
             (e = hipMalloc((void**)&d_s, n)) != hipSuccess ||
             (e = hipMemcpyAsync(d_p, prev_pts, n * sizeof(float2), hipMemcpyHostToDevice, ctx->stream)) != hipSuccess)
         { cleanup(); return ctx->fail(LVK_HIP_ERR_RUNTIME, hipGetErrorString(e)); }
-        if ((rc = lvk_launch_pyrlk(ctx, P.args, N.args, d_p, n, d_n, d_s, win_w, win_h, max_count, epsilon, min_eig_threshold)) != LVK_HIP_OK) { cleanup(); return rc; }
+        if ((rc = lvk_launch_pyrlk(ctx, P.args, N.args, d_p, n, d_n, d_s, win_w, win_h, max_count, epsilon, min_eig_threshold, nullptr, nullptr, 0.0, 0.0, nullptr,
+                                   nullptr, 0, waves_per_feature)) != LVK_HIP_OK) { cleanup(); return rc; }
         if ((e = hipMemcpyAsync(next_pts, d_n, n * sizeof(float2), hipMemcpyDeviceToHost, ctx->stream)) != hipSuccess ||
             (e = hipMemcpyAsync(status, d_s, n, hipMemcpyDeviceToHost, ctx->stream)) != hipSuccess)
         { cleanup(); return ctx->fail(LVK_HIP_ERR_RUNTIME, hipGetErrorString(e)); }
@@ -635,3 +698,16 @@
 }
 
 LVK_TL_EXPORT(pyrlk)
+
+#ifdef LVK_TIMELINE
+extern "C" int lvk_tl_read_pyrlk_blocks(long long* out, int capacity)
+{
+    if (!out || capacity < 1 + 2 * LVK_LK_BLOCK_RING) return -1;
+    unsigned head = 0;
+    if (hipDeviceSynchronize() != hipSuccess) return -1;
+    if (hipMemcpyFromSymbol(&head, HIP_SYMBOL(lvk_lk_block_head), sizeof(head)) != hipSuccess) return -1;
+    out[0] = head;
+    if (hipMemcpyFromSymbol(out + 1, HIP_SYMBOL(lvk_lk_block_log), sizeof(long long) * 2 * LVK_LK_BLOCK_RING) != hipSuccess) return -1;
+    return LVK_LK_BLOCK_RING;
+}
+#endif
diff --git a/livevisionkit_amd/csrc/stabilizer.hip b/livevisionkit_amd/csrc/stabilizer.hip
--- a/livevisionkit_amd/csrc/stabilizer.hip
+++ b/livevisionkit_amd/csrc/stabilizer.hip
@@ -97,6 +97,7 @@
         c.prev_pyr = &P.args; c.next_pyr = &C.args; c.h_pts = h_pts;
         c.win_w = LK_WIN; c.win_h = LK_WIN; c.max_count = LK_ITERS; c.epsilon = LK_EPS; c.min_eig = LK_MIN_EIG;
         c.lens = lens ? &lens_model : nullptr; c.lens_sx = (double)f.cols / (double)cur_w; c.lens_sy = (double)f.rows / (double)cur_h;
+        c.flow_wave_slots = (overlap && caller_runs_free) ? LVK_FLOW_SLOTS_BESIDE_REMAP : LVK_FLOW_SLOTS_ALONE;
         c.n = n; c.d_n = dn; c.full = full; c.d_full = dfull;
         c.d_pts = d_pts; c.d_matched = d_matched; c.d_status = d_status; c.d_und = lens ? d_und : nullptr;
         c.d_p1 = d_p1; c.d_p2 = d_p1 + cap_features; c.d_count = d_count; c.h_count = h_count; c.h_matched = h_matched; c.h_status = h_status;
diff --git a/livevisionkit_amd/csrc/track_chain.hip b/livevisionkit_amd/csrc/track_chain.hip
--- a/livevisionkit_amd/csrc/track_chain.hip
+++ b/livevisionkit_amd/csrc/track_chain.hip
@@ -10,7 +10,7 @@
     const int n = c.n;
     if (c.prev_pyr &&
         (rc = lvk_launch_pyrlk(ctx, *c.prev_pyr, *c.next_pyr, c.h_pts, n, c.d_matched, c.d_status, c.win_w, c.win_h, c.max_count, c.epsilon, c.min_eig, c.d_pts,
-                               c.d_und ? c.lens : nullptr, c.lens_sx, c.lens_sy, c.d_und, c.d_n)) != LVK_HIP_OK) return rc;
+                               c.d_und ? c.lens : nullptr, c.lens_sx, c.lens_sy, c.d_und, c.d_n, c.flow_wave_slots, c.flow_waves)) != LVK_HIP_OK) return rc;
     const bool fused_compact = c.estimate && !c.separate_compact && n <= LVK_COMPACT_RANSAC_MAX;
     if (!fused_compact && (rc = lvk_launch_match_compact(ctx, c.d_pts, c.d_matched, c.d_status, n, c.d_p1, c.d_p2, c.d_count, c.h_count, c.h_matched, c.h_status,
                                                          c.d_und, (float)c.region_w, (float)c.region_h, c.d_n)) != LVK_HIP_OK) return rc;
@@ -92,6 +92,7 @@
         }
         c.prev_pyr = &b.P.args; c.next_pyr = &b.N.args; c.h_pts = h_pts;
         c.win_w = d->win_w; c.win_h = d->win_h; c.max_count = d->max_count; c.epsilon = d->epsilon; c.min_eig = d->min_eig;
+        c.flow_waves = d->flow_waves;
     }
     else
     {
```

New measurement: 9815, median of 2. About the same (-0.2%).
